# Roy-Shubhajit/FIT-GNN

Hardware: AMD Instinct MI355X
Metric: edges aggregated/sec (GCN fwd+bwd) on coarsened subgraphs (higher is better)
Workload: dtype f32

## Files before the change

fit-gnn_amd/csrc/gemm_f32.hip:

```cpp
#include <algorithm>
#include <cmath>

#include "common.h"
#include "fitgnn_hip.h"

namespace {

typedef float f32x16 __attribute__((ext_vector_type(16)));

constexpr int kBK = 32;
constexpr int kPitch = 36;

template <int WM, int WN, int MI, int NJ, bool AKM, bool BKM>
struct Geo {
    static constexpr int TI = 32 * MI * WM, TJ = 32 * NJ * WN, THREADS = 64 * WM * WN;
    static constexpr int A_DW = AKM ? kBK * TI : TI * kPitch;
    static constexpr int B_DW = BKM ? kBK * TJ : TJ * kPitch;
    static constexpr int STAGE_DW = A_DW + B_DW;
    static constexpr int LDS_BYTES = 2 * STAGE_DW * 4;
    static constexpr int NA = TI * 8 / THREADS, NB = TJ * 8 / THREADS;
    static_assert(LDS_BYTES <= 160 * 1024, "tile does not fit the CU's LDS");
    static_assert(TI * 8 % THREADS == 0 && TJ * 8 % THREADS == 0, "stage not divisible over the threads");
};

template <bool KM, int T, int NV, int THREADS>
__device__ __forceinline__ void load_slab(float4 (&r)[NV], const float *__restrict__ P, long ld, long t0, long lim, long k0, long klim) {
    const int tid = threadIdx.x;
#pragma unroll
    for (int p = 0; p < NV; ++p) {
        const int v = tid + p * THREADS;
        if (!KM) {
            const int row = v >> 3, k4 = v & 7;
            long i = t0 + row;
            i = i < lim ? i : lim - 1;
            const long k = k0 + 4 * k4;
            r[p] = k < klim ? *reinterpret_cast<const float4 *>(P + i * ld + k) : make_float4(0.f, 0.f, 0.f, 0.f);
        } else {
            constexpr int Q = T / 4;
            const int kr = v / Q, c4 = v % Q;
            long i = t0 + 4 * c4;
            i = i + 4 <= lim ? i : lim - 4;
            const long k = k0 + kr;
            r[p] = k < klim ? *reinterpret_cast<const float4 *>(P + k * ld + i) : make_float4(0.f, 0.f, 0.f, 0.f);
        }
    }
}

template <bool KM, int T, int NV, int THREADS>
__device__ __forceinline__ void store_slab(const float4 (&r)[NV], float *lds) {
    const int tid = threadIdx.x;
#pragma unroll
    for (int p = 0; p < NV; ++p) {
        const int v = tid + p * THREADS;
        if (!KM) {
            const int row = v >> 3, k4 = v & 7;
            *reinterpret_cast<float4 *>(lds + row * kPitch + 4 * k4) = r[p];
        } else {
            constexpr int Q = T / 4;
            const int kr = v / Q, c4 = v % Q;
            *reinterpret_cast<float4 *>(lds + kr * T + 4 * c4) = r[p];
        }
    }
}

template <bool KM, int T>
__device__ __forceinline__ void frag(float (&f)[4], const float *lds, int o, int kk, int lane) {
    if (!KM) {
        const float4 v = *reinterpret_cast<const float4 *>(lds + (o + (lane & 31)) * kPitch + 8 * kk + 4 * (lane >> 5));
        f[0] = v.x; f[1] = v.y; f[2] = v.z; f[3] = v.w;
    } else {
        const float *p = lds + (8 * kk + 4 * (lane >> 5)) * T + o + (lane & 31);
#pragma unroll
        for (int s = 0; s < 4; ++s) f[s] = p[s * T];
    }
}

struct StoreEpi {
    const int64_t *rows;
    const float *bias;
    const uint8_t *mask;
    uint64_t seed;
    long row0;
    uint32_t epi;
    float p_drop;
};

template <int WM, int WN, int MI, int NJ, bool AKM, bool BKM, bool EPI>
__global__ __launch_bounds__(64 * WM * WN) void gemm_f32_kernel(const float *__restrict__ A, long lda, const float *__restrict__ B, long ldb,
                                                                   long I, int J, long K, float *__restrict__ C, long ldc, int tiles_i,
                                                                   int tiles_j, int nchunks, long chunk_k, StoreEpi se) {
    using G = Geo<WM, WN, MI, NJ, AKM, BKM>;
    extern __shared__ __attribute__((aligned(16))) float lds_f[];
    const int lane = threadIdx.x & 63, wave = __builtin_amdgcn_readfirstlane(threadIdx.x >> 6);
    const int wm = wave / WN, wn = wave % WN;
    const int xcd = blockIdx.x & 7, slot = blockIdx.x >> 3;
    int ti, tj, chunk = 0;
    if (nchunks > 1) {
        const int ntile = tiles_i * tiles_j;
        const int tile = slot % ntile;
        chunk = xcd + 8 * (slot / ntile);
        ti = tile / tiles_j, tj = tile % tiles_j;
        if (chunk >= nchunks) return;
    } else {
        tj = slot % tiles_j;
        ti = xcd + 8 * (slot / tiles_j);
        if (ti >= tiles_i) return;
    }
    const long i0 = (long)ti * G::TI, j0 = (long)tj * G::TJ;
    const long k_begin = (long)chunk * chunk_k;
    const long k_end = nchunks > 1 ? (k_begin + chunk_k < K ? k_begin + chunk_k : K) : K;
    const int nstage = k_end > k_begin ? (int)((k_end - k_begin + kBK - 1) / kBK) : 0;

    f32x16 acc[MI][NJ];
#pragma unroll
    for (int i = 0; i < MI; ++i)
#pragma unroll
        for (int j = 0; j < NJ; ++j)
#pragma unroll
            for (int r = 0; r < 16; ++r) acc[i][j][r] = 0.f;

    float4 ra[G::NA], rb[G::NB];
    if (nstage > 0) {
        load_slab<AKM, G::TI, G::NA, G::THREADS>(ra, A, lda, i0, I, k_begin, k_end);
        load_slab<BKM, G::TJ, G::NB, G::THREADS>(rb, B, ldb, j0, (long)J, k_begin, k_end);
        store_slab<AKM, G::TI, G::NA, G::THREADS>(ra, lds_f);
        store_slab<BKM, G::TJ, G::NB, G::THREADS>(rb, lds_f + G::A_DW);
    }
    __syncthreads();
    auto read_frags = [&](float (&fa)[MI][4], float (&fb)[NJ][4], const float *sa, const float *sb, int kk) {
#pragma unroll
        for (int i = 0; i < MI; ++i) frag<AKM, G::TI>(fa[i], sa, wm * (32 * MI) + i * 32, kk, lane);
#pragma unroll
        for (int j = 0; j < NJ; ++j) frag<BKM, G::TJ>(fb[j], sb, wn * (32 * NJ) + j * 32, kk, lane);
    };
    auto multiply = [&](const float (&fa)[MI][4], const float (&fb)[NJ][4]) {
#pragma unroll
        for (int st = 0; st < 4; ++st)
#pragma unroll
            for (int i = 0; i < MI; ++i)
#pragma unroll
                for (int j = 0; j < NJ; ++j)
                    acc[i][j] = __builtin_amdgcn_mfma_f32_32x32x2f32(fa[i][st], fb[j][st], acc[i][j], 0, 0, 0);
    };
    constexpr int NKK = kBK / 8;
    auto products = [&](int s) {
        const float *sa = lds_f + (s & 1) * G::STAGE_DW;
        const float *sb = sa + G::A_DW;
#pragma unroll
        for (int kk = 0; kk < NKK; ++kk) {
            float fa[MI][4], fb[NJ][4];
            read_frags(fa, fb, sa, sb, kk);
            multiply(fa, fb);
        }
    };
    for (int s = 0; s < nstage; ++s) {
        const bool more = s + 1 < nstage;
        if (more) {
            const long k0 = k_begin + (long)(s + 1) * kBK;
            load_slab<AKM, G::TI, G::NA, G::THREADS>(ra, A, lda, i0, I, k0, k_end);
            load_slab<BKM, G::TJ, G::NB, G::THREADS>(rb, B, ldb, j0, (long)J, k0, k_end);
        }
        products(s);
        if (more) {
            float *na = lds_f + ((s + 1) & 1) * G::STAGE_DW;
            store_slab<AKM, G::TI, G::NA, G::THREADS>(ra, na);
            store_slab<BKM, G::TJ, G::NB, G::THREADS>(rb, na + G::A_DW);
        }
        __syncthreads();
    }

    float *out = nchunks > 1 ? C + (long)chunk * I * J : C;
    const long ldo = nchunks > 1 ? (long)J : ldc;
    if constexpr (EPI) {
        const uint64_t seed = fitgnn::resolve_seed(se.seed, se.epi);
        const float keep_scale = (se.epi & FITGNN_EPI_DROPOUT) ? 1.0f / (1.0f - se.p_drop) : 1.0f;
        const uint32_t thresh = fitgnn::dropout_threshold(se.p_drop);
#pragma unroll
        for (int i = 0; i < MI; ++i) {
            const long row0 = i0 + wm * (32 * MI) + i * 32 + 4 * (lane >> 5);
            long orow[16];
#pragma unroll
            for (int r = 0; r < 16; ++r) {
                const long row = row0 + (r & 3) + 8 * (r >> 2);
                orow[r] = row < I ? (se.rows ? (long)se.rows[row] : se.row0 + row) : 0;
            }
#pragma unroll
            for (int j = 0; j < NJ; ++j) {
                const long col = j0 + wn * (32 * NJ) + j * 32 + (lane & 31);
                const float bias = ((se.epi & FITGNN_EPI_BIAS) && col < J) ? se.bias[col] : 0.f;
#pragma unroll
                for (int r = 0; r < 16; ++r) {
                    const long row = row0 + (r & 3) + 8 * (r >> 2);
                    if (row < I && col < J)
                        out[row * ldo + col] = fitgnn::finish_elem(acc[i][j][r], bias, se.epi, keep_scale, thresh, seed, se.mask,
                                                                   (uint64_t)orow[r] * (uint64_t)J + (uint64_t)col);
                }
            }
        }
        return;
    }
#pragma unroll
    for (int i = 0; i < MI; ++i) {
#pragma unroll
        for (int j = 0; j < NJ; ++j) {
            const long col = j0 + wn * (32 * NJ) + j * 32 + (lane & 31);
            const long row0 = i0 + wm * (32 * MI) + i * 32 + 4 * (lane >> 5);
#pragma unroll
            for (int r = 0; r < 16; ++r) {
                const long row = row0 + (r & 3) + 8 * (r >> 2);
                if (row < I && col < J) out[row * ldo + col] = acc[i][j][r];
            }
        }
    }
}

template <bool EPI>
__global__ __launch_bounds__(256) void sum_chunks_kernel(const float *__restrict__ partial, int nchunks, long IJ, float *__restrict__ out, int J,
                                                         long ldc, StoreEpi se) {
    const long q = (long)blockIdx.x * blockDim.x + threadIdx.x;
    if (q >= IJ) return;
    float part[8];
#pragma unroll
    for (int u = 0; u < 8; ++u) part[u] = 0.f;
    int c = 0;
    for (; c + 8 <= nchunks; c += 8) {
#pragma unroll
        for (int u = 0; u < 8; ++u) part[u] += partial[(long)(c + u) * IJ + q];
    }
#pragma unroll
    for (int u = 0; u < 8; ++u)
        if (c + u < nchunks) part[u] += partial[(long)(c + u) * IJ + q];
    float acc = part[0];
#pragma unroll
    for (int u = 1; u < 8; ++u) acc += part[u];
    const long row = q / J, col = q % J;
    if constexpr (EPI) {
        const uint64_t seed = fitgnn::resolve_seed(se.seed, se.epi);
        const float keep_scale = (se.epi & FITGNN_EPI_DROPOUT) ? 1.0f / (1.0f - se.p_drop) : 1.0f;
        const long orow = se.rows ? (long)se.rows[row] : se.row0 + row;
        acc = fitgnn::finish_elem(acc, (se.epi & FITGNN_EPI_BIAS) ? se.bias[col] : 0.f, se.epi, keep_scale, fitgnn::dropout_threshold(se.p_drop),
                                  seed, se.mask, (uint64_t)orow * (uint64_t)J + (uint64_t)col);
    }
    out[row * ldc + col] = acc;
}

enum Shape { S256 = 0, S256x128, S64x512, S128, S64x128, S128x64, S64x64 };
struct ShapeDim { int ti, tj, per_cu; };
constexpr ShapeDim kShape[] = {{256, 256, 1}, {256, 128, 1}, {64, 512, 1}, {128, 128, 2}, {64, 128, 2}, {128, 64, 2}, {64, 64, 4}};

struct Plan {
    int shape;
    int tiles_i, tiles_j, nchunks;
    long chunk_k;
    long main_rows;
    int rem_tiles_i, rem_chunks;
    long rem_chunk_k;
};

Plan make_plan(long I, int J, long K, bool akm, bool bkm) {
    Plan p;
    const bool tn = akm && bkm;
    auto tiles_of = [&](int sh) { return ((I + kShape[sh].ti - 1) / kShape[sh].ti) * ((J + kShape[sh].tj - 1) / kShape[sh].tj); };
    if (tn) {
        if (I <= 64) p.shape = S64x512;
        else if (J <= 128 || K < 65536) p.shape = S128;
        else p.shape = S256;
    } else if (J <= 64) {
        p.shape = S128x64;
    } else {
        const int cand[4] = {J <= 128 ? S256x128 : S256, S128, S64x128, S64x64};
        const double eff[4] = {1.0, K <= 256 ? 1.0 : 0.85, 0.94, 0.85};
        double best_cost = 0;
        for (int q = 0; q < 4; ++q) {
            const int sh = cand[q];
            const long t = tiles_of(sh);
            double rounds = (double)((t + 255) / 256);
            if (q == 0 && !akm && t / 256 >= 1 && t % 256 > 0 && t % 256 <= 96 && K >= 8 * 2 * kBK) rounds = (double)(t / 256) + 0.15;
            const double cost = rounds * kShape[sh].ti * kShape[sh].tj / eff[q];
            if (q == 0 || cost < best_cost) { best_cost = cost; p.shape = sh; }
        }
        if (K >= 4096 && tiles_of(S256) <= 512 && J > 128) p.shape = S128;
    }
    const int TI = kShape[p.shape].ti, TJ = kShape[p.shape].tj;
    const double slots = 256.0 * kShape[p.shape].per_cu;
    p.tiles_i = (int)((I + TI - 1) / TI);
    p.tiles_j = (J + TJ - 1) / TJ;
    p.nchunks = 1;
    p.chunk_k = K;
    const double ntile = (double)p.tiles_i * p.tiles_j;
    const double t_tile = 2.0 * TI * TJ * (double)K / (0.45e12 / kShape[p.shape].per_cu);
    const long most = K / (4 * kBK);
    double best = ceil(ntile / slots) * t_tile;
    for (long c = 8; c <= most && c <= 256; c += 8) {
        const double t = ceil(ntile * (double)c / slots) * t_tile / (double)c + (double)(c + 1) * (double)I * (double)J * 4.0 / 3.0e12 + 4e-6;
        if (t < 0.92 * best) { best = t; p.nchunks = (int)c; }
    }
    if (p.nchunks > 1) {
        const long per = (K + p.nchunks - 1) / p.nchunks;
        p.chunk_k = (per + kBK - 1) / kBK * kBK;
    }
    p.main_rows = 0; p.rem_tiles_i = 0; p.rem_chunks = 1; p.rem_chunk_k = K;
    const long T = (long)p.tiles_i * p.tiles_j;
    const long full = T / 256, rem = T % 256;
    if (!akm && kShape[p.shape].per_cu == 1 && p.nchunks == 1 && full >= 1 && rem > 0 && rem <= 96 && K >= 8 * 2 * kBK) {
        const long main_tiles_i = full * 256 / p.tiles_j;
        if (main_tiles_i >= 1 && main_tiles_i < p.tiles_i) {
            p.main_rows = main_tiles_i * TI;
            p.rem_tiles_i = (int)(p.tiles_i - main_tiles_i);
            p.rem_chunks = 8;
            p.rem_chunk_k = ((K + 7) / 8 + kBK - 1) / kBK * kBK;
        }
    }
    return p;
}

template <int WM, int WN, int MI, int NJ, bool AKM, bool BKM, bool EPI>
int launch(const Plan &p, const float *a, long lda, const float *b, long ldb, long I, int J, long K, float *c, long ldc, hipStream_t s,
           const StoreEpi &se) {
    using G = Geo<WM, WN, MI, NJ, AKM, BKM>;
    static std::atomic<uint64_t> lds_done{0};
    if (const int rc = fitgnn_lds_limit_once((const void *)gemm_f32_kernel<WM, WN, MI, NJ, AKM, BKM, EPI>, G::LDS_BYTES, lds_done)) return rc;
    unsigned grid;
    if (p.nchunks > 1) grid = (unsigned)(p.tiles_i * p.tiles_j * ((p.nchunks + 7) / 8 * 8));
    else grid = (unsigned)((p.tiles_i + 7) / 8 * 8 * p.tiles_j);
    hipLaunchKernelGGL((gemm_f32_kernel<WM, WN, MI, NJ, AKM, BKM, EPI>), dim3(grid), dim3(G::THREADS), G::LDS_BYTES, s, a, lda, b, ldb, I, J,
                       K, c, ldc, p.tiles_i, p.tiles_j, p.nchunks, p.chunk_k, se);
    return (int)hipGetLastError();
}

template <bool AKM, bool BKM, bool EPI = false>
int launch_shape(const Plan &p, const float *a, long lda, const float *b, long ldb, long I, int J, long K, float *c, long ldc, hipStream_t s,
                 const StoreEpi &se = StoreEpi{}) {
    if constexpr (AKM && BKM) {
        if (p.shape == S64x512) return launch<1, 4, 2, 4, AKM, BKM, EPI>(p, a, lda, b, ldb, I, J, K, c, ldc, s, se);
    }
    switch (p.shape) {
        case S256x128: return launch<4, 1, 2, 4, AKM, BKM, EPI>(p, a, lda, b, ldb, I, J, K, c, ldc, s, se);
        case S128: return launch<2, 2, 2, 2, AKM, BKM, EPI>(p, a, lda, b, ldb, I, J, K, c, ldc, s, se);
        case S64x128: return launch<2, 2, 1, 2, AKM, BKM, EPI>(p, a, lda, b, ldb, I, J, K, c, ldc, s, se);
        case S128x64: return launch<4, 1, 1, 2, AKM, BKM, EPI>(p, a, lda, b, ldb, I, J, K, c, ldc, s, se);
        case S64x64: return launch<2, 2, 1, 1, AKM, BKM, EPI>(p, a, lda, b, ldb, I, J, K, c, ldc, s, se);
        default: return launch<4, 2, 2, 4, AKM, BKM, EPI>(p, a, lda, b, ldb, I, J, K, c, ldc, s, se);
    }
}

}

extern "C" size_t fitgnn_gemm_exact_workspace_bytes(int64_t I, int32_t J, int64_t K, int32_t a_kmajor, int32_t b_kmajor) {
    if (I <= 0 || J <= 0 || K <= 0) return 0;
    const Plan p = make_plan((long)I, J, (long)K, a_kmajor != 0, b_kmajor != 0);
    if (p.main_rows > 0) return (size_t)p.rem_chunks * (size_t)(I - p.main_rows) * (size_t)J * sizeof(float);
    return p.nchunks > 1 ? (size_t)p.nchunks * (size_t)I * (size_t)J * sizeof(float) : 0;
}

extern "C" int fitgnn_gemm_exact_plan(int64_t I, int32_t J, int64_t K, int32_t a_kmajor, int32_t b_kmajor, int32_t *shape, int32_t *nchunks,
                                      int64_t *main_rows) {
    if (I <= 0 || J <= 0 || K <= 0 || !shape || !nchunks || !main_rows) return FITGNN_E_BADARG;
    const Plan p = make_plan((long)I, J, (long)K, a_kmajor != 0, b_kmajor != 0);
    *shape = p.shape;
    *nchunks = p.nchunks;
    *main_rows = p.main_rows;
    return 0;
}

extern "C" int fitgnn_gemm_exact_f32(const float *a, int64_t lda, int32_t a_kmajor, const float *b, int64_t ldb, int32_t b_kmajor,
                                     int64_t I, int32_t J, int64_t K, float *c, int64_t ldc, void *workspace, void *stream) {
    if (I <= 0 || J <= 0 || K <= 0 || ldc < J) return FITGNN_E_BADARG;
    if (!a || !b || !c) return FITGNN_E_BADARG;
    const int64_t a_inner = a_kmajor ? I : K, b_inner = b_kmajor ? (int64_t)J : K;
    if (a_inner < 4 || b_inner < 4 || (a_inner % 4) != 0 || (b_inner % 4) != 0 || lda < a_inner || ldb < b_inner || (lda % 4) != 0 ||
        (ldb % 4) != 0)
        return FITGNN_E_BADARG;
    if ((((uintptr_t)a | (uintptr_t)b) % 16) != 0) return FITGNN_E_ALIGN;
    if (a_kmajor && !b_kmajor) return FITGNN_E_BADARG;
    const Plan p = make_plan((long)I, J, (long)K, a_kmajor != 0, b_kmajor != 0);
    hipStream_t s = (hipStream_t)stream;
    if (p.main_rows > 0) {
        if (!workspace || ((uintptr_t)workspace % 16) != 0) return FITGNN_E_BADARG;
        Plan pm = p, pr = p;
        pm.tiles_i = (int)(p.main_rows / kShape[p.shape].ti);
        pr.tiles_i = p.rem_tiles_i; pr.nchunks = p.rem_chunks; pr.chunk_k = p.rem_chunk_k;
        const long rem_rows = (long)I - p.main_rows;
        const float *a_rem = a + p.main_rows * (long)lda;
        int rc;
        if (b_kmajor) {
            rc = launch_shape<false, true>(pm, a, (long)lda, b, (long)ldb, p.main_rows, J, (long)K, c, (long)ldc, s);
            if (!rc) rc = launch_shape<false, true>(pr, a_rem, (long)lda, b, (long)ldb, rem_rows, J, (long)K, (float *)workspace, (long)J, s);
        } else {
            rc = launch_shape<false, false>(pm, a, (long)lda, b, (long)ldb, p.main_rows, J, (long)K, c, (long)ldc, s);
            if (!rc) rc = launch_shape<false, false>(pr, a_rem, (long)lda, b, (long)ldb, rem_rows, J, (long)K, (float *)workspace, (long)J, s);
        }
        if (rc) return rc;
        const long IJ = rem_rows * J;
        hipLaunchKernelGGL(sum_chunks_kernel<false>, dim3((unsigned)((IJ + 255) / 256)), dim3(256), 0, s, (const float *)workspace, pr.nchunks,
                           IJ, c + p.main_rows * (long)ldc, J, (long)ldc, StoreEpi{});
        return (int)hipGetLastError();
    }
    float *dst = c;
    long ldd = (long)ldc;
    if (p.nchunks > 1) {
        if (!workspace || ((uintptr_t)workspace % 16) != 0) return FITGNN_E_BADARG;
        dst = (float *)workspace;
    }
    int rc;
    if (a_kmajor) rc = launch_shape<true, true>(p, a, (long)lda, b, (long)ldb, (long)I, J, (long)K, dst, ldd, s);
    else if (b_kmajor) rc = launch_shape<false, true>(p, a, (long)lda, b, (long)ldb, (long)I, J, (long)K, dst, ldd, s);
    else rc = launch_shape<false, false>(p, a, (long)lda, b, (long)ldb, (long)I, J, (long)K, dst, ldd, s);
    if (rc) return rc;
    if (p.nchunks > 1) {
        const long IJ = (long)I * J;
        hipLaunchKernelGGL(sum_chunks_kernel<false>, dim3((unsigned)((IJ + 255) / 256)), dim3(256), 0, s, (const float *)workspace, p.nchunks, IJ, c,
                           J, (long)ldc, StoreEpi{});
        return (int)hipGetLastError();
    }
    return 0;
}

extern "C" int fitgnn_gemm_exact_epi_f32(const float *a, int64_t lda, const float *b, int64_t ldb, int64_t I, int32_t J, int64_t K, float *c,
                                         int64_t ldc, const int64_t *rows, const float *bias, uint32_t epilogue, float p_drop, uint64_t seed,
                                         const uint8_t *mask, void *workspace, void *stream) {
    if (I <= 0 || J <= 0 || K <= 0 || ldc < J) return FITGNN_E_BADARG;
    if (!a || !b || !c) return FITGNN_E_BADARG;
    if (K < 4 || (K % 4) != 0 || lda < K || ldb < K || (lda % 4) != 0 || (ldb % 4) != 0) return FITGNN_E_BADARG;
    if ((((uintptr_t)a | (uintptr_t)b) % 16) != 0) return FITGNN_E_ALIGN;
    if (epilogue & ~(FITGNN_EPI_BIAS | FITGNN_EPI_ELU | FITGNN_EPI_DROPOUT | FITGNN_EPI_SEED_DEVICE)) return FITGNN_E_BADARG;
    if ((epilogue & (FITGNN_EPI_ELU | FITGNN_EPI_DROPOUT)) && (J % 4) != 0) return FITGNN_E_BADARG;
    if ((epilogue & FITGNN_EPI_BIAS) && !bias) return FITGNN_E_BADARG;
    if ((epilogue & FITGNN_EPI_DROPOUT) && !(p_drop >= 0.f && p_drop < 1.f)) return FITGNN_E_BADARG;
    const Plan p = make_plan((long)I, J, (long)K, false, false);
    if (p.nchunks > 1) return FITGNN_E_BADARG;
    hipStream_t s = (hipStream_t)stream;
    StoreEpi se{rows, bias, mask, seed, 0, epilogue, p_drop};
    if (p.main_rows == 0) return launch_shape<false, false, true>(p, a, (long)lda, b, (long)ldb, (long)I, J, (long)K, c, (long)ldc, s, se);
    if (!workspace || ((uintptr_t)workspace % 16) != 0) return FITGNN_E_BADARG;
    Plan pm = p, pr = p;
    pm.tiles_i = (int)(p.main_rows / kShape[p.shape].ti);
    pr.tiles_i = p.rem_tiles_i; pr.nchunks = p.rem_chunks; pr.chunk_k = p.rem_chunk_k;
    const long rem_rows = (long)I - p.main_rows;
    int rc = launch_shape<false, false, true>(pm, a, (long)lda, b, (long)ldb, p.main_rows, J, (long)K, c, (long)ldc, s, se);
    if (!rc) rc = launch_shape<false, false>(pr, a + p.main_rows * (long)lda, (long)lda, b, (long)ldb, rem_rows, J, (long)K, (float *)workspace, (long)J, s);
    if (rc) return rc;
    if (rows) se.rows = rows + p.main_rows;
    se.row0 = p.main_rows;
    const long IJ = rem_rows * J;
    hipLaunchKernelGGL(sum_chunks_kernel<true>, dim3((unsigned)((IJ + 255) / 256)), dim3(256), 0, s, (const float *)workspace, pr.nchunks, IJ,
                       c + p.main_rows * (long)ldc, J, (long)ldc, se);
    return (int)hipGetLastError();
}
```

fit-gnn_amd/csrc/spmm.hip:

```cpp
#include <hip/hip_runtime.h>
#include <stdint.h>

#include <algorithm>

#include "common.h"
#include "fitgnn_hip.h"

namespace {

constexpr int kWaves = 4;
constexpr int kThreads = kWaves * 64;
constexpr int kDefaultWindowRows = 16;
constexpr int kMaxWindowRows = 96;
constexpr int kSmallWindowRows = 16;
constexpr int kLongRow = 16;

template <int VEC> struct Pack;
template <> struct Pack<4> {
    using T = float4;
    static __device__ __forceinline__ T zero() { return make_float4(0.f, 0.f, 0.f, 0.f); }
    static __device__ __forceinline__ void fma(T &a, float v, const T &x) {
        a.x = fmaf(v, x.x, a.x); a.y = fmaf(v, x.y, a.y); a.z = fmaf(v, x.z, a.z); a.w = fmaf(v, x.w, a.w);
    }
    static __device__ __forceinline__ float get(const T &a, int i) { return i == 0 ? a.x : i == 1 ? a.y : i == 2 ? a.z : a.w; }
// ... 164 lines not shown
                    mc[j] = 0; mv[j] = 0.f;
                    if (i < n_meta) { mc[j] = cidx[E0 + i]; mv[j] = val[E0 + i]; }
                }
            }
#pragma unroll
            for (int j = 0; j < B; ++j) {
                const int r = wave + (p0 + j) * kWaves;
                if (r < win_rows) lds[r * 64 + lane] = v[j];
            }
            if (p0 == 0) {
                if ((int)threadIdx.x <= rp_rows) s_rp[threadIdx.x] = rpv;
#pragma unroll
                for (int j = 0; j < MB; ++j) {
                    const int i = threadIdx.x + j * kThreads;
                    if (i < n_meta) { s_col[i] = mc[j]; s_val[i] = mv[j]; }
                }
            }
        }
        for (int i = threadIdx.x + kThreads; i <= rp_rows; i += kThreads) s_rp[i] = rowptr[tile.row_begin + i];
        for (int i = threadIdx.x + MB * kThreads; i < n_meta; i += kThreads) { s_col[i] = cidx[E0 + i]; s_val[i] = val[E0 + i]; }
    }
    __syncthreads();

    const float keep_scale = (epi & FITGNN_EPI_DROPOUT) ? 1.0f / (1.0f - p_drop) : 1.0f;
    const uint32_t thresh = fitgnn::dropout_threshold(p_drop);
    const RowEpilogue rowepi{epi, keep_scale, (epi & FITGNN_EPI_DROPOUT) ? 1.0f - p_drop : 1.0f, thresh, seed, mask, prev};
    float cs[VEC];
#pragma unroll
    for (int i = 0; i < VEC; ++i) cs[i] = 0.f;
    float bv[VEC];
#pragma unroll
    for (int i = 0; i < VEC; ++i) bv[i] = ((epi & FITGNN_EPI_BIAS) && live) ? bias[col0 + i] : 0.f;
    const int slot_off = planned ? 0 : win_begin;
    auto gcol = [&](int c) -> int {
        if (!planned) return c + slot_off;
        if (c < 0) return -(c + 1);
        return listed ? win_cols[win_begin + c] : win_begin + c;
    };
    auto xsrc = [&](int g) -> int64_t { return xrow ? xrow[g] : g; };
    auto gather = [&](int g) -> T {
        const int64_t sr = xsrc(g);
        if (zero_from >= 0 && xrow && sr >= zero_from) return P::zero();
        return *reinterpret_cast<const T *>(Xs + sr * ldx);
    };
    for (int row = tile.row_begin + wave; row < tile.row_end; row += kWaves) {
        const T o_prev = prev_row<VEC>(rowepi, row, col0, H, live);
        const int lr = row - tile.row_begin;
        int e0, e1;
        if (lr < rp_rows) { e0 = s_rp[lr]; e1 = s_rp[lr + 1]; } else { e0 = rowptr[row]; e1 = rowptr[row + 1]; }
        e0 = __builtin_amdgcn_readfirstlane(e0);
        e1 = __builtin_amdgcn_readfirstlane(e1);
        T acc = P::zero();
        for (int base = e0; base < e1; base += 64) {
            const int cnt = min(64, e1 - base);
            int my_c = 0;
            float my_v = 0.f;
            if (lane < cnt) {
                const int i = base + lane - E0;
                if (i < n_meta) { my_c = s_col[i]; my_v = s_val[i]; } else { my_c = cidx[base + lane]; my_v = val[base + lane]; }
            }
            int k = 0;
            if (cnt >= kLongRow) {
                for (; k + 8 <= cnt; k += 8) {
                    T x[8];
                    float w[8];
#pragma unroll
                    for (int u = 0; u < 8; ++u) {
                        const int c = __builtin_amdgcn_readlane(my_c, k + u) - slot_off;
                        w[u] = __int_as_float(__builtin_amdgcn_readlane(__float_as_int(my_v), k + u));
                        x[u] = gather(gcol(c));
                    }
#pragma unroll
                    for (int u = 0; u < 8; ++u) P::fma(acc, w[u], x[u]);
                }
            }
            for (; k < cnt; k += 4) {
                const int k1 = min(k + 1, cnt - 1), k2 = min(k + 2, cnt - 1), k3 = min(k + 3, cnt - 1);
                const int c0 = __builtin_amdgcn_readlane(my_c, k) - slot_off;
                const int c1 = __builtin_amdgcn_readlane(my_c, k1) - slot_off;
                const int c2 = __builtin_amdgcn_readlane(my_c, k2) - slot_off;
                const int c3 = __builtin_amdgcn_readlane(my_c, k3) - slot_off;
                const float w0 = __int_as_float(__builtin_amdgcn_readlane(__float_as_int(my_v), k));
                const float w1 = k + 1 < cnt ? __int_as_float(__builtin_amdgcn_readlane(__float_as_int(my_v), k1)) : 0.f;
                const float w2 = k + 2 < cnt ? __int_as_float(__builtin_amdgcn_readlane(__float_as_int(my_v), k2)) : 0.f;
                const float w3 = k + 3 < cnt ? __int_as_float(__builtin_amdgcn_readlane(__float_as_int(my_v), k3)) : 0.f;
                const bool in0 = (unsigned)c0 < (unsigned)win_rows, in1 = (unsigned)c1 < (unsigned)win_rows;
                const bool in2 = (unsigned)c2 < (unsigned)win_rows, in3 = (unsigned)c3 < (unsigned)win_rows;
                T x0, x1, x2, x3;
                if (in0 && in1 && in2 && in3) {
                    x0 = lds[c0 * 64 + lane]; x1 = lds[c1 * 64 + lane];
                    x2 = lds[c2 * 64 + lane]; x3 = lds[c3 * 64 + lane];
                } else {
                    const int g0 = gcol(c0), g1 = gcol(c1), g2 = gcol(c2), g3 = gcol(c3);
                    if (in0) x0 = lds[c0 * 64 + lane]; else x0 = gather(g0);
                    if (in1) x1 = lds[c1 * 64 + lane]; else x1 = gather(g1);
                    if (in2) x2 = lds[c2 * 64 + lane]; else x2 = gather(g2);
                    if (in3) x3 = lds[c3 * 64 + lane]; else x3 = gather(g3);
                }
                P::fma(acc, w0, x0); P::fma(acc, w1, x1); P::fma(acc, w2, x2); P::fma(acc, w3, x3);
            }
        }
        if (live) finish_row<VEC, true, NOEPI>(acc, row, col0, H, Y, ldy, bv, rowepi, cs, o_prev);
    }
    if (!NOEPI && (epi & FITGNN_EPI_BACKWARD) && col_part)
        write_col_part<VEC>(reinterpret_cast<float *>(lds_raw), cs, col_part, t, H, col0, live);
}


#ifdef FITGNN_SPMM_STAMPS
static __device__ unsigned long long *g_spmm_dbg;
#define SSTAMP(var) const unsigned long long var = __builtin_readcyclecounter()
#define SACC(i, a, b) sdbg[i] += (b) - (a)
#else
#define SSTAMP(var)
#define SACC(i, a, b)
#endif
constexpr int kBlkRows = 16;
constexpr int kBlkLW = 1;
constexpr int kBlkLong = 4 * kBlkLW;
constexpr int kBlkMeta = 128;

template <bool XROW, bool BWD, bool NOEPI = false, bool TWO = false>
__global__ __launch_bounds__(kThreads, BWD ? 4 : TWO ? 6 : XROW ? 7 : 7) void spmm_block_kernel(
    const int32_t *__restrict__ rowptr, const int32_t *__restrict__ col, const float *__restrict__ val,
    const float *__restrict__ X, int64_t ldx, float *__restrict__ Y, int64_t ldy, int32_t H,
    const fitgnn_block_t *__restrict__ blocks, int32_t n_blocks, const int32_t *__restrict__ long_rows, int32_t n_slabs,
    const float *__restrict__ bias, uint32_t epi, float p_drop, uint64_t seed_arg, const uint8_t *__restrict__ mask,
    const int32_t *__restrict__ xrow, const int32_t *__restrict__ xcol, const float *__restrict__ prev, float *__restrict__ col_part,
    int32_t zero_from, const float *__restrict__ Xc2 = nullptr, int64_t ldxc = 0, const int32_t *__restrict__ row_p = nullptr,
    const float *__restrict__ row_w = nullptr, int32_t xc_zero_from = 0) {
    static_assert(!TWO || (XROW && !BWD && NOEPI), "the two-hop form is a plain product over a table");
    constexpr uint32_t kNtOut = TWO ? fitgnn::kNtOutTwoHop : BWD ? 0u : XROW ? fitgnn::kNtOutTable : fitgnn::kNtOutPlain;
    constexpr uint32_t kNtWin = TWO ? fitgnn::kNtWinTwoHop : XROW ? fitgnn::kNtWinTable : fitgnn::kNtWinPlain;
    using P = Pack<4>;
    using T = float4;
    constexpr int kZeroSlot = kBlkRows + kBlkLong;
    const uint64_t seed = fitgnn::resolve_seed(seed_arg, epi);
    __shared__ T s_win[(kBlkRows + kBlkLong + 1) * 64];
    __shared__ int32_t s_rp[kBlkRows + 4];
    __shared__ int32_t s_col[kBlkMeta];
    __shared__ float s_val[kBlkMeta];
    __shared__ int32_t s_long[kBlkLong];
    __shared__ int32_t s_hub_pos;
    const int bid = blockIdx.x;
    const int seq = bid >> 3;
    const int slab = seq % n_slabs;
    const int b = (seq / n_slabs) * 8 + (bid & 7);
    if (b >= n_blocks) return;
#ifdef FITGNN_SPMM_STAMPS
    unsigned long long sdbg[8] = {0, 0, 0, 0, 0, 0, 0, 0};
#endif
    SSTAMP(s_begin);
    const fitgnn_block_t blk = blocks[b];
    if (blk.row_end <= blk.row_begin) return;
    const int lane = threadIdx.x & 63;
    const int wave = __builtin_amdgcn_readfirstlane(threadIdx.x >> 6);
    const int col0 = slab * 256 + lane * 4;
    const bool live = col0 + 4 <= H;
    const float *Xs = X + (live ? col0 : max(H - 4, 0));
    auto src = [&](int r) -> int64_t { return XROW ? (int64_t)xrow[r] : (int64_t)r; };
    auto ecol = [&](int e, int c) -> int { return (TWO || (XROW && xcol)) ? xcol[e] : (XROW ? xrow[c] : c); };
    const int n_long = min(blk.n_long, kBlkLong);
    const float keep_scale = (epi & FITGNN_EPI_DROPOUT) ? 1.0f / (1.0f - p_drop) : 1.0f;
    const uint32_t thresh = fitgnn::dropout_threshold(p_drop);
    const RowEpilogue rowepi{(BWD || TWO) ? (epi | FITGNN_EPI_BACKWARD) : (epi & ~FITGNN_EPI_BACKWARD), keep_scale,
                             (epi & FITGNN_EPI_DROPOUT) ? 1.0f - p_drop : 1.0f, thresh, seed, mask, (BWD || TWO) ? prev : nullptr};
    const int colc2 = live ? col0 : max(H - 4, 0);
    float cs[4];
#pragma unroll
    for (int i = 0; i < 4; ++i) cs[i] = 0.f;
    float bv[4];
#pragma unroll
    for (int i = 0; i < 4; ++i) bv[i] = ((epi & FITGNN_EPI_BIAS) && live) ? bias[col0 + i] : 0.f;

    const bool has_zero = XROW && !TWO && zero_from >= 0;
    auto is_zero_row = [&](int64_t opr) { return has_zero && opr >= (int64_t)zero_from; };
    T pv[4];
    T o_nx[kBlkRows / kWaves];
    int p_rp = 0, p_c = 0, p_cx = 0, p_E0 = 0;
    float p_v = 0.f;
    int xr_next = 0;
    int xp_next = 0, xw_next = 0;
    int sr_pub[4] = {0, 0, 0, 0}, pp_pub[4] = {0, 0, 0, 0};
    float w_pub[4] = {0.f, 0.f, 0.f, 0.f};
    int hub_pos = 0x7fffffff;
    auto fetch_indices = [&](int r0, int r1) {
        if (XROW) {
            const int r = r0 + wave + lane * kWaves;
            xr_next = (lane < 4 && r < r1) ? xrow[r] : 0;
            if (TWO) {
                xp_next = (lane < 4 && r < r1) ? row_p[r] : 0x7fffffff;
                xw_next = (lane < 4 && r < r1) ? __float_as_int(row_w[r]) : 0;
            }
        }
    };
    auto prefetch = [&](int r0, int r1, int E0) {
        const int xr = xr_next;

#pragma unroll
        for (int j = 0; j < 4; ++j) {
            const int r = r0 + wave + j * kWaves;
            pv[j] = P::zero();
            const int64_t sr = XROW ? (int64_t)__builtin_amdgcn_readlane(xr, j) : (int64_t)r;
            if (TWO) {
                const int rr = min(r, r1 - 1);
                const float *rowp = sr >= 0 ? Xs + sr * ldx : prev + (uint64_t)rr * (uint64_t)H + (uint64_t)colc2;
                const int pp = __builtin_amdgcn_readlane(xp_next, j);
                const T a = fitgnn::load4<kNtWin>(rowp);
                pv[j] = r < r1 ? a : P::zero();
                sr_pub[j] = (int)sr;
                pp_pub[j] = pp;
                w_pub[j] = __int_as_float(__builtin_amdgcn_readlane(xw_next, j));
            } else if (r < r1 && !is_zero_row(sr)) {
                pv[j] = fitgnn::load4<kNtWin>(Xs + sr * ldx);
            }
        }
        if (XROW) fetch_indices(r1, min(r1 + kBlkRows, blk.row_end));
        if (BWD) {
#pragma unroll
            for (int j = 0; j < kBlkRows / kWaves; ++j) o_nx[j] = prev_row<4, BWD>(rowepi, min(r0 + wave + j * kWaves, r1 - 1), col0, H, live);
        }
        p_rp = 0;
        if ((int)threadIdx.x <= r1 - r0) p_rp = rowptr[r0 + threadIdx.x];
        p_c = 0; p_cx = 0; p_v = 0.f;
        if ((int)threadIdx.x < kBlkMeta && blk.nnz_end > blk.nnz_begin) {
            const int e = min(E0 + (int)threadIdx.x, blk.nnz_end - 1);
            p_c = col[e];
            p_cx = (TWO || (XROW && xcol)) ? xcol[e] : p_c;
            p_v = val[e];
        }
        p_E0 = E0;
    };
    fetch_indices(blk.row_begin, min(blk.row_begin + kBlkRows, blk.row_end));
    if ((int)threadIdx.x < kBlkLong) s_long[threadIdx.x] = (int)threadIdx.x < n_long ? long_rows[blk.long_off + threadIdx.x] : -1;
    if (XROW && !TWO && (int)threadIdx.x < 64) s_win[kZeroSlot * 64 + threadIdx.x] = P::zero();
    if (TWO && threadIdx.x == 0) s_hub_pos = 0x7fffffff;
    int my_long[kBlkLW], cur[kBlkLW], end[kBlkLW], pos[kBlkLW], lc[kBlkLW], lcx[kBlkLW];
    float lv[kBlkLW];
    T acc_long[kBlkLW];
#pragma unroll
    for (int q = 0; q < kBlkLW; ++q) {
        const int slot = wave + q * kWaves;
        my_long[q] = slot < n_long ? long_rows[blk.long_off + slot] : -1;
        my_long[q] = __builtin_amdgcn_readfirstlane(my_long[q]);
        acc_long[q] = P::zero();
        cur[q] = end[q] = 0;
        pos[q] = 64;
        lc[q] = 0x7fffffff;
        lcx[q] = 0;
        lv[q] = 0.f;
    }
    prefetch(blk.row_begin, min(blk.row_begin + kBlkRows, blk.row_end), blk.nnz_begin);
#pragma unroll
    for (int q = 0; q < kBlkLW; ++q) {
        const int slot = wave + q * kWaves;
        if (my_long[q] >= 0) {
            cur[q] = __builtin_amdgcn_readfirstlane(rowptr[my_long[q]]);
            end[q] = __builtin_amdgcn_readfirstlane(rowptr[my_long[q] + 1]);
            const int64_t lr_src = src(my_long[q]);
            s_win[(kBlkRows + slot) * 64 + lane] = is_zero_row(lr_src) ? P::zero() : *reinterpret_cast<const T *>(Xs + lr_src * ldx);
            if (TWO && slot == 0 && lr_src < (int64_t)xc_zero_from) {
                s_win[kZeroSlot * 64 + lane] = *reinterpret_cast<const T *>(Xc2 + lr_src * ldxc + colc2);
                if (lane == 0) s_hub_pos = (int)lr_src;
            }
        }
    }
    __syncthreads();
    if (TWO) hub_pos = __builtin_amdgcn_readfirstlane(s_hub_pos);
    int lid[kBlkLong];
#pragma unroll
    for (int i = 0; i < kBlkLong; ++i) lid[i] = __builtin_amdgcn_readfirstlane(s_long[i]);

    const int n_pieces = (blk.row_end - blk.row_begin + kBlkRows - 1) / kBlkRows;

    auto gather_long = [&](int q, int bound) {
        while (cur[q] < end[q]) {
            if (pos[q] == 64) {
                const int e = cur[q] + lane;
                lc[q] = e < end[q] ? col[e] : 0x7fffffff;
                lcx[q] = (XROW && xcol && e < end[q]) ? xcol[e] : 0;
                lv[q] = e < end[q] ? val[e] : 0.f;
                pos[q] = 0;
            }
            const unsigned long long in = __ballot(lc[q] < bound) >> pos[q];
            const int n_in = in == 0 ? 0 : (int)__builtin_popcountll(in);
            constexpr int kLongBatch = (TWO || (XROW && !BWD)) ? 4 : 8;
            for (int k = pos[q]; k < pos[q] + n_in; k += kLongBatch) {
                const int last = pos[q] + n_in - 1;
                T x[kLongBatch];
                float w[kLongBatch];
#pragma unroll
                for (int u = 0; u < kLongBatch; ++u) {
                    const int kk = min(k + u, last);
                    const int64_t c = (XROW && xcol) ? (int64_t)__builtin_amdgcn_readlane(lcx[q], kk) : src(__builtin_amdgcn_readlane(lc[q], kk));
                    w[u] = k + u <= last ? __int_as_float(__builtin_amdgcn_readlane(__float_as_int(lv[q]), kk)) : 0.f;
                    x[u] = is_zero_row(c) ? P::zero() : *reinterpret_cast<const T *>(Xs + c * ldx);
                }
#pragma unroll
                for (int u = 0; u < kLongBatch; ++u) P::fma(acc_long[q], w[u], x[u]);
            }
            pos[q] += n_in;
            cur[q] += n_in;
            if (pos[q] < 64) break;
        }
    };
#pragma unroll
    for (int q = 0; q < kBlkLW; ++q)
// ... 962 lines not shown
```

fit-gnn_amd/fitgnn_amd/_lib.py:

```python
import ctypes
import os

_HERE = os.path.dirname(os.path.abspath(__file__))
LIB_PATH = os.path.join(os.path.dirname(_HERE), "lib", "libfitgnn_hip.so")

c_i32, c_i64, c_u32, c_u64, c_f32, c_size = (ctypes.c_int32, ctypes.c_int64, ctypes.c_uint32, ctypes.c_uint64,
                                              ctypes.c_float, ctypes.c_size_t)
ptr = ctypes.c_void_p

EPI_BIAS, EPI_ELU, EPI_DROPOUT, EPI_SEED_DEVICE = 1, 2, 4, 8
SPMM_GATHER = 0x100
MAX_K = 16
MATCH_HEAVY_EDGE, MATCH_ALGEBRAIC_JC = 0, 1
MATCH_SMALL_MAX_NODES, MATCH_SMALL_MAX_NNZ, MATCH_SMALL_MAX_K, MATCH_SMALL_LDS_BUDGET = 128, 1024, 12, 65536
MATCH_DONE, MATCH_TOO_BIG, MATCH_BAD_INPUT = 1, 2, 3
QUALITY_MAX_K = 64

SIGNATURES = {
    "fitgnn_abi_version": (ctypes.c_int, []),
    "fitgnn_error_string": (ctypes.c_char_p, [ctypes.c_int]),
    "fitgnn_stream_copy_f32": (ctypes.c_int, [ptr, ptr, c_i64, ptr]),
    "fitgnn_spmm_default_window_rows": (ctypes.c_int, []),
    "fitgnn_spmm_max_window_rows": (ctypes.c_int, [c_i32]),
    "fitgnn_gcn_norm_csr_f32": (ctypes.c_int, [ptr, ptr, ptr, ptr, ptr, c_i32, ptr]),
    "fitgnn_spmm_csr_f32": (ctypes.c_int, [ptr, ptr, ptr, ptr, c_i64, ptr, c_i64, c_i32, c_i32, ptr, c_i32, ptr, ptr,
                                           ptr, c_i32, c_i32, ptr, c_u32, c_f32, c_u64, ptr, ptr]),
    "fitgnn_spmm_csr_blocks_f32": (ctypes.c_int, [ptr, ptr, ptr, ptr, c_i64, ptr, c_i64, c_i32, c_i32, ptr, c_i32, ptr,
                                                  ptr, ptr, c_i32, ptr, c_u32, c_f32, c_u64, ptr, ptr]),
    "fitgnn_spmm_csr_dz_f32": (ctypes.c_int, [ptr, ptr, ptr, ptr, c_i64, ptr, c_i64, c_i32, c_i32, ptr, c_i32, ptr, ptr,
                                              ptr, c_i32, c_i32, ptr, c_u32, c_f32, c_u64, ptr, ptr, ptr]),
    "fitgnn_spmm_csr_blocks_dz_f32": (ctypes.c_int, [ptr, ptr, ptr, ptr, c_i64, ptr, c_i64, c_i32, c_i32, ptr, c_i32, ptr,
                                                     ptr, ptr, c_i32, ptr, c_u32, c_f32, c_u64, ptr, ptr, ptr]),
    "fitgnn_lanczos_parts": (c_i32, [c_i32]),
    "fitgnn_lanczos_spmv_f64": (ctypes.c_int, [ptr, ptr, ptr, ptr, ptr, c_i32, ctypes.c_double, ctypes.c_double, ptr]),
    "fitgnn_lanczos_project_f64": (ctypes.c_int, [ptr, c_i64, c_i32, ptr, c_i32, ptr, ptr, ptr]),
    "fitgnn_lanczos_reduce_f64": (ctypes.c_int, [ptr, c_i32, c_i32, ptr, ptr]),
    "fitgnn_lanczos_finish_f64": (ctypes.c_int, [ptr, c_i64, c_i32, ptr, c_i32, ptr, ptr, ptr, ptr, c_i32, ptr]),
    "fitgnn_lanczos_rotate_f64": (ctypes.c_int, [ptr, c_i64, c_i32, ptr, c_i32, ptr, c_i64, c_i32, ptr]),
    "fitgnn_spmm_csr_stream_f32": (ctypes.c_int, [ptr, ptr, ptr, c_i64, ptr, c_i64, ptr, c_i64, c_i32, c_i32, ptr, c_i32, ptr, c_i32, ptr, ptr,
                                                  ptr, c_u32, c_f32, c_u64, ptr, ptr]),
    "fitgnn_spmm_csr_stream_dz_f32": (ctypes.c_int, [ptr, ptr, ptr, c_i64, ptr, c_i64, ptr, c_i64, c_i32, c_i32, ptr, c_i32, ptr, c_i32, ptr, ptr,
                                                     ptr, c_u32, c_f32, c_u64, ptr, ptr, ptr]),
    "fitgnn_spmm_rows_compact_parts": (c_i32, [c_i32]),
    "fitgnn_spmm_rows_compact_f32": (ctypes.c_int, [ptr, ptr, ptr, c_i64, ptr, c_i64, c_i32, ptr, c_i64, c_i32, c_i32, ptr]),
    "fitgnn_spmm_rows_compact_dz_f32": (ctypes.c_int, [ptr, ptr, ptr, c_i64, ptr, c_i64, c_i32, ptr, c_i64, c_i32, c_i32, ptr, c_u32, c_f32,
                                                       c_u64, ptr, ptr, ptr]),
    "fitgnn_two_hop_rows_f32": (ctypes.c_int, [ptr, ptr, ptr, ptr, c_i64, c_i32, ptr, c_i32, ptr, c_i32, c_u32, c_f32, c_u64, ptr, ptr, c_i64, ptr]),
    "fitgnn_spmm_two_hop_blocks_f32": (ctypes.c_int, [ptr, ptr, ptr, ptr, c_i64, ptr, c_i64, c_i32, c_i32, ptr, c_i32, ptr, ptr, ptr, ptr, ptr, c_i64,
                                                      c_i32, ptr, ptr, c_u32, c_f32, c_u64, ptr, ptr, ptr]),
    "fitgnn_segment_sum_f32": (ctypes.c_int, [ptr, ptr, c_i32, ptr, c_i64, c_i32, ptr, c_i64, ptr]),
    "fitgnn_segment_max_f32": (ctypes.c_int, [ptr, ptr, c_i32, ptr, c_i64, c_i32, ptr, ptr, ptr]),
    "fitgnn_segment_max_bwd_f32": (ctypes.c_int, [ptr, ptr, c_i32, c_i32, ptr, c_i64, ptr]),
    "fitgnn_segment_expand_f32": (ctypes.c_int, [ptr, ptr, ptr, c_i64, c_i32, ptr, ptr]),
    "fitgnn_make_tiles_host": (ctypes.c_int, [ptr, c_i64, c_i32, ptr, c_i64, ptr]),
    "fitgnn_split_blocks_host": (ctypes.c_int, [ptr, c_i64, ptr, c_i32, c_i64, c_i32, ptr, c_i64, ptr, ptr, ptr, ptr, c_i64, ptr]),
    "fitgnn_plan_tiles_host": (ctypes.c_int, [ptr, ptr, c_i32, c_i32, ptr, c_i32, c_i32, c_i32, ptr, ptr, ptr, ptr, ptr]),
    "fitgnn_epilogue_bwd_workspace_bytes": (c_size, [c_i32, c_i32]),
    "fitgnn_epilogue_bwd_f32": (ctypes.c_int, [ptr, ptr, ptr, c_i32, c_i32, c_u32, c_f32, c_u64, ptr, ptr, ptr, c_size, ptr]),
    "fitgnn_head_max_classes": (ctypes.c_int, []),
    "fitgnn_head_max_classes_wide": (ctypes.c_int, []),
    "fitgnn_epilogue_bwd_head_supported": (ctypes.c_int, [c_i32, c_i32, c_i32]),
    "fitgnn_epilogue_bwd_head_workspace_bytes": (c_size, [c_i32, c_i32, c_i32]),
    "fitgnn_epilogue_bwd_head_f32": (ctypes.c_int, [ptr, ptr, c_i32, ptr, ptr, c_i32, c_i32, c_u32, c_f32, c_u64, ptr, ptr, ptr,
                                                   ptr, c_size, ptr]),
    "fitgnn_epilogue_bwd_head_rows_f32": (ctypes.c_int, [ptr, ptr, c_i32, ptr, ptr, c_i32, c_i32, ptr, c_i32, c_u32, c_f32, c_u64, ptr,
                                                        ptr, ptr, ptr, c_size, ptr]),
    "fitgnn_epilogue_bwd_rows_f32": (ctypes.c_int, [ptr, ptr, ptr, c_i32, c_i32, ptr, c_i32, c_u32, c_f32, c_u64, ptr, ptr, ptr, c_size, ptr]),
    "fitgnn_spmm_epilogue_bwd_supported": (ctypes.c_int, [c_i32, c_i32, c_i32]),
    "fitgnn_spmm_epilogue_bwd_workspace_bytes": (c_size, [c_i32, c_i32, c_i32]),
    "fitgnn_spmm_epilogue_bwd_f32": (ctypes.c_int, [ptr, ptr, ptr, ptr, c_i32, c_i32, ptr, ptr, ptr, c_i32, ptr, ptr, c_i32, c_i32,
                                                   c_u32, c_f32, c_u64, ptr, ptr, ptr, ptr, c_size, ptr]),
    "fitgnn_gat_scores_f32": (ctypes.c_int, [ptr, c_i64, c_i32, c_i32, ptr, ptr, ptr, ptr, ptr]),
    "fitgnn_gat_edge_softmax_f32": (ctypes.c_int, [ptr, ptr, ptr, ptr, c_f32, c_i32, ptr, ptr]),
    "fitgnn_sddmm_csr_f32": (ctypes.c_int, [ptr, ptr, ptr, c_i64, ptr, c_i64, c_i32, c_i32, ptr, ptr]),
    "fitgnn_sddmm_csr_rows_f32": (ctypes.c_int, [ptr, ptr, ptr, c_i64, ptr, c_i64, ptr, c_i32, c_i32, ptr, ptr]),
    "fitgnn_gat_softmax_bwd_rows_f32": (ctypes.c_int, [ptr, ptr, ptr, ptr, ptr, ptr, c_f32, ptr, c_i32, ptr, ptr, ptr]),
    "fitgnn_gat_softmax_bwd_f32": (ctypes.c_int, [ptr, ptr, ptr, ptr, ptr, ptr, c_f32, c_i32, ptr, ptr, ptr]),
    "fitgnn_l1_loss_f32": (ctypes.c_int, [ptr, ptr, c_i32, c_f32, ptr, ptr, ptr]),
    "fitgnn_softmax_nll_workspace_bytes": (c_size, [c_i32]),
    "fitgnn_softmax_nll_f32": (ctypes.c_int, [ptr, c_i64, c_i32, c_i32, ptr, ptr, c_i32, c_f32, ptr, ptr, ptr, c_size, ptr]),
    "fitgnn_adam_step_f32": (ctypes.c_int, [ptr, ptr, ptr, ptr, c_i64, c_f32, c_f32, c_f32, c_f32, c_f32, ptr, ptr]),
    "fitgnn_sum_leading_f32": (ctypes.c_int, [ptr, c_i32, c_i64, ptr, ptr]),
    "fitgnn_gemm_atb_workspace_bytes": (c_size, [c_i64, c_i32, c_i32]),
    "fitgnn_gemm_atb_f32": (ctypes.c_int, [ptr, c_i64, ptr, c_i64, c_i64, c_i32, c_i32, ptr, ptr, ptr]),
    "fitgnn_gemm_nt_f32": (ctypes.c_int, [ptr, c_i64, ptr, c_i64, c_i64, c_i32, c_i32, ptr, c_i64, ptr]),
    "fitgnn_gemm_exact_workspace_bytes": (c_size, [c_i64, c_i32, c_i64, c_i32, c_i32]),
    "fitgnn_gemm_exact_f32": (ctypes.c_int, [ptr, c_i64, c_i32, ptr, c_i64, c_i32, c_i64, c_i32, c_i64, ptr, c_i64, ptr, ptr]),
    "fitgnn_gemm_exact_plan": (ctypes.c_int, [c_i64, c_i32, c_i64, c_i32, c_i32, ptr, ptr, ptr]),
    "fitgnn_gemm_exact_epi_f32": (ctypes.c_int, [ptr, c_i64, ptr, c_i64, c_i64, c_i32, c_i64, ptr, c_i64, ptr, ptr, c_u32, c_f32, c_u64, ptr, ptr,
                                                 ptr]),
    "fitgnn_gemm_nt_presplit_bytes": (c_size, [c_i32, c_i32]),
    "fitgnn_gemm_nt_presplit_f32": (ctypes.c_int, [ptr, c_i64, c_i64, c_i32, c_i32, c_i32, ptr, ptr]),
    "fitgnn_gemm_nt_pre_f32": (ctypes.c_int, [ptr, c_i64, ptr, c_i64, c_i32, c_i32, ptr, c_i64, ptr]),
    "fitgnn_gemm_nt_epilogue_bwd_workspace_bytes": (c_size, [c_i64, c_i32]),
    "fitgnn_gemm_nt_epilogue_bwd_f32": (ctypes.c_int, [ptr, c_i64, ptr, c_i64, c_i64, c_i32, c_i32, ptr, ptr, ctypes.c_uint32, c_f32,
                                                       ctypes.c_uint64, ptr, ptr, ptr, c_size, ptr]),
    "fitgnn_colsum_partials_f32": (ctypes.c_int, [ptr, c_i32, c_i32, ptr, ptr]),
    "fitgnn_head_rows_lds_bytes": (c_size, [c_i32, c_i32]),
    "fitgnn_head_rows_f32": (ctypes.c_int, [ptr, c_i64, ptr, c_i32, ptr, ptr, c_i32, c_i32, ptr, c_i64, c_i32, ptr]),
    "fitgnn_epilogue_fwd_rows_f32": (ctypes.c_int, [ptr, c_i64, ptr, c_i32, c_i32, ptr, c_u32, c_f32, c_u64, ptr, ptr]),
    "fitgnn_dense_narrow_k_lds_bytes": (c_size, [c_i32, c_i32]),
    "fitgnn_dense_narrow_k_f32": (ctypes.c_int, [ptr, c_i64, ptr, c_i64, c_i32, c_i32, c_i32, ptr, c_u32, c_f32, c_u64, ptr, ptr, c_i64, ptr]),
    "fitgnn_narrow_atb_workspace_bytes": (c_size, [c_i32, c_i32, c_i32]),
    "fitgnn_narrow_atb_f32": (ctypes.c_int, [ptr, c_i64, ptr, c_u32, c_f32, c_u64, ptr, ptr, c_i64, c_i32, c_i32, c_i32, ptr, ptr, ptr, c_size,
                                             ptr]),
    "fitgnn_adam_step_acc_f32": (ctypes.c_int, [ptr, ptr, ptr, ptr, ptr, c_i64, c_f32, c_f32, c_f32, c_f32, c_f32, ptr, ptr, c_i32, c_u64, ptr]),
    "fitgnn_pool_head_supported": (ctypes.c_int, [c_i32, c_i32]),
    "fitgnn_pool_head_f32": (ctypes.c_int, [ptr, ptr, c_i32, ptr, c_i64, c_i32, ptr, ptr, ptr, c_i32, ptr, ptr, ptr]),
    "fitgnn_pool_head_bwd_f32": (ctypes.c_int, [ptr, ptr, c_i32, ptr, ptr, ptr, c_i64, c_i32, c_i32, ptr, ptr, ptr, ptr]),
    "fitgnn_colsum_narrow_workspace_bytes": (c_size, [c_i32, c_i32]),
    "fitgnn_colsum_narrow_f32": (ctypes.c_int, [ptr, c_i64, c_i32, c_i32, ptr, ptr, c_size, ptr]),
    "fitgnn_spmm_narrow_f32": (ctypes.c_int, [ptr, ptr, ptr, ptr, ptr, c_i32, c_i32, c_f32, ptr, c_f32, ptr, c_f32, ptr]),
    "fitgnn_spmm_narrow_padded_f32": (ctypes.c_int, [ptr, ptr, ptr, ptr, ptr, c_i32, c_i32, c_f32, ptr, c_f32, ptr, c_f32, ptr]),
    "fitgnn_appnp_unit_rows": (ctypes.c_int, [c_i32]),
    "fitgnn_appnp_unit_entries": (ctypes.c_int, []),
    "fitgnn_appnp_block_rows": (ctypes.c_int, []),
    "fitgnn_appnp_block_entries": (ctypes.c_int, []),
    "fitgnn_appnp_blocks_f32": (ctypes.c_int, [ptr, ptr, ptr, ptr, c_i32, c_i32, c_i32, ptr, ptr, ptr, ptr, c_i32, c_i32, c_f32, c_i32, ptr]),
    "fitgnn_appnp_lds_bytes": (ctypes.c_int64, [c_i32, c_i32, c_i32]),
    "fitgnn_appnp_lds_max_bytes": (ctypes.c_int, []),
    "fitgnn_appnp_lds_items_per_thread": (ctypes.c_int, []),
    "fitgnn_appnp_lds_f32": (ctypes.c_int, [ptr, ptr, ptr, ptr, c_i32, c_i32, c_i32, ptr, ptr, c_i32, c_i32, c_f32, c_i32, c_i32, c_i32, ptr]),
    "fitgnn_gather_rows_padded_f32": (ctypes.c_int, [ptr, c_i64, c_i32, ptr, c_i64, ptr, c_i32, ptr]),
    "fitgnn_appnp_units_f32": (ctypes.c_int, [ptr, ptr, ptr, ptr, c_i32, c_i32, c_i32, ptr, ptr, c_i32, c_i32, c_f32, c_i32, ptr]),
    "fitgnn_gcn_query_gather_f32": (ctypes.c_int, [ptr, ptr, ptr, ptr, c_i64, ptr, ptr, ptr, c_i32, c_i32, ptr, c_i64, ptr]),
    "fitgnn_sage_query_gather_f32": (ctypes.c_int, [ptr, ptr, ptr, ptr, c_i64, ptr, ptr, ptr, c_i32, c_i32, ptr, c_i64, ptr]),
    "fitgnn_gat_query_gather_f32": (ctypes.c_int, [ptr, ptr, ptr, c_i64, ptr, ptr, ptr, ptr, c_f32, ptr, ptr, c_f32, ptr, c_i32, c_i32, ptr,
                                                   c_i64, ptr]),
    "fitgnn_gcn_query_tail_lds_bytes": (c_size, [c_i32, c_i32]),
    "fitgnn_gcn_query_tail_f32": (ctypes.c_int, [ptr, c_i64, c_i32, ptr, ptr, ptr, ptr, c_i32, c_i32, c_i32, ptr, c_i64, c_i32, ptr]),
    "fitgnn_gcn_graph_query_hops_lds_bytes": (c_size, [c_i32, c_i32]),
    "fitgnn_gcn_graph_query_hops_f32": (ctypes.c_int, [ptr, ptr, ptr, ptr, c_i64, ptr, ptr, ptr, ptr, ptr, c_i32, c_i32, c_i32, ptr, c_i64, ptr]),
    "fitgnn_gcn_graph_query_tail_lds_bytes": (c_size, [c_i32, c_i32]),
    "fitgnn_gcn_graph_query_tail_f32": (ctypes.c_int, [ptr, c_i64, ptr, c_i32, ptr, ptr, ptr, ptr, c_i32, c_i32, c_i32, c_i32, c_i32, ptr, c_i64,
                                                       ptr]),
    "fitgnn_gin_query_hops_f32": (ctypes.c_int, [ptr, ptr, ptr, ptr, c_i64, ptr, ptr, ptr, ptr, ptr, ptr, ptr, c_i32, c_i32, c_i32, ptr, c_i64,
                                                 ptr]),
    "fitgnn_gin_query_tail_lds_bytes": (c_size, [c_i32, c_i32, c_i32]),
    "fitgnn_gin_query_tail_f32": (ctypes.c_int, [ptr, c_i64, c_i32, ptr, ptr, ptr, ptr, ptr, ptr, c_i32, c_i32, c_i32, c_i32, ptr, c_i64, c_i32,
                                                 ptr]),
    "fitgnn_gin_graph_query_hops_lds_bytes": (c_size, [c_i32, c_i32, c_i32]),
    "fitgnn_gin_graph_query_hops_f32": (ctypes.c_int, [ptr, ptr, ptr, ptr, c_i64, ptr, ptr, ptr, ptr, ptr, ptr, ptr, ptr, ptr, c_i32, c_i32, c_i32,
                                                       c_i32, ptr, c_i64, ptr]),
    "fitgnn_gin_graph_query_tail_lds_bytes": (c_size, [c_i32, c_i32, c_i32]),
    "fitgnn_gin_graph_query_tail_f32": (ctypes.c_int, [ptr, c_i64, ptr, c_i32, ptr, ptr, ptr, ptr, ptr, ptr, c_i32, c_i32, c_i32, c_i32, c_i32,
                                                       c_i32, ptr, c_i64, ptr]),
    "fitgnn_gat_graph_query_hops_lds_bytes": (c_size, [c_i32, c_i32]),
    "fitgnn_gat_graph_query_hops_f32": (ctypes.c_int, [ptr, ptr, ptr, c_i64, ptr, ptr, ptr, ptr, c_f32, ptr, ptr, c_f32, ptr, ptr, ptr, c_i32,
                                                       c_i32, c_i32, ptr, c_i64, ptr]),
    "fitgnn_sage_graph_query_hops_lds_bytes": (c_size, [c_i32, c_i32]),
    "fitgnn_sage_graph_query_hops_f32": (ctypes.c_int, [ptr, ptr, ptr, ptr, c_i64, ptr, ptr, ptr, ptr, ptr, c_i32, c_i32, c_i32, ptr, c_i64, ptr]),
    "fitgnn_csr_row_sum_f32": (ctypes.c_int, [ptr, ptr, c_i32, ptr, ptr]),
    "fitgnn_induced_edges_count": (ctypes.c_int, [ptr, ptr, ptr, ptr, ptr, ptr, c_i64, ptr, ptr]),
    "fitgnn_induced_edges_fill": (ctypes.c_int, [ptr, ptr, ptr, ptr, ptr, ptr, ptr, c_i64, ptr, ptr, ptr, ptr]),
    "fitgnn_batch_offsets": (ctypes.c_int, [ptr, ptr, c_i32, ptr, ptr, ptr, ptr, ptr, ptr, ptr, ptr, ptr]),
    "fitgnn_batch_gather": (ctypes.c_int, [c_i32, ptr, ptr, ptr, ptr, ptr, ptr, ptr, ptr, ptr, ptr, ptr, ptr, ptr, c_i32, ptr, c_i32, c_i32,
                                           c_i32, c_i32, c_i32, c_i32, ptr, ptr, ptr, ptr, ptr, ptr, ptr, ptr, ptr, c_i32, ptr, ptr, ptr, ptr, ptr,
                                           c_i32, ptr]),
    "fitgnn_closed_neighbourhoods": (ctypes.c_int, [ptr, ptr, c_i32, ptr, ptr, ptr]),
    "fitgnn_variation_costs_f64": (ctypes.c_int, [ptr, ptr, ptr, ptr, ptr, c_i32, c_i64, ptr, ptr, ptr, c_i32, ptr, ptr]),
    "fitgnn_variation_costs_batch_f64": (ctypes.c_int, [ptr, ptr, ptr, ptr, ptr, c_i32, c_i64, ptr, ptr, ptr, ptr, c_i32, ptr, ptr]),
    "fitgnn_greedy_select_workspace_bytes": (c_size, [c_i32, c_i64]),
    "fitgnn_greedy_select": (ctypes.c_int, [ptr, ptr, ptr, ptr, ptr, c_i32, c_i64, c_i32, ptr, ptr, ptr, c_i64, ptr, ptr,
                                            ptr, ptr, c_size, ptr]),
    "fitgnn_greedy_select_batch_workspace_bytes": (c_size, [c_i32, c_i64, c_i32]),
    "fitgnn_greedy_select_batch": (ctypes.c_int, [ptr, ptr, ptr, ptr, ptr, c_i32, c_i64, c_i32, ptr, ptr, ptr, c_i32, ptr, ptr,
                                                  c_i64, ptr, ptr, ptr, ptr, ptr, ptr, c_size, ptr]),
    "fitgnn_build_assignment_workspace_bytes": (c_size, [c_i32]),
    "fitgnn_build_assignment": (ctypes.c_int, [c_i32, ptr, ptr, ptr, ptr, ptr, ptr, ptr, c_size, ptr]),
    "fitgnn_compose_levels": (ctypes.c_int, [c_i32, ptr, ptr, ptr, ptr, ptr]),
    "fitgnn_lift_adjacency_workspace_bytes": (c_size, [c_i32, c_i64, c_i32]),
    "fitgnn_lift_adjacency": (ctypes.c_int, [c_i32, ptr, ptr, ptr, ptr, ptr, c_i32, ptr, ptr, ptr, ptr, ptr, c_size, ptr]),
    "fitgnn_edge_list": (ctypes.c_int, [ptr, ptr, ptr, c_i32, ptr, ptr, ptr, ptr, c_i64, ptr, ptr]),
    "fitgnn_heavy_edge_proximity_workspace_bytes": (c_size, [c_i32]),
    "fitgnn_heavy_edge_proximity": (ctypes.c_int, [ptr, ptr, ptr, c_i32, ptr, ptr, ptr, c_i64, ptr, ptr, c_size, ptr]),
    "fitgnn_jc_proximity": (ctypes.c_int, [ptr, ptr, c_i64, ptr, c_i32, c_i64, ptr, ptr]),
    "fitgnn_affinity_proximity_workspace_bytes": (c_size, [c_i32, c_i64]),
    "fitgnn_affinity_proximity": (ctypes.c_int, [c_i32, ptr, ptr, c_i64, ptr, c_i32, c_i64, ptr, ptr, c_size, ptr]),
    "fitgnn_edge_variation_costs_f64": (ctypes.c_int, [ptr, ptr, c_i64, ptr, ptr, c_i32, c_i64, ptr, ptr]),
    "fitgnn_jacobi_vectors_workspace_bytes": (c_size, [c_i32, c_i32]),
    "fitgnn_jacobi_vectors_f64": (ctypes.c_int, [ptr, ptr, ptr, ptr, c_i32, ptr, c_i32, c_i32, ptr, ptr, c_size, ptr]),
    "fitgnn_gauss_seidel_vectors_f64": (ctypes.c_int, [ptr, ptr, ptr, ptr, c_i32, c_i32, ptr, ptr, c_i32, ptr, ptr]),
    "fitgnn_greedy_matching_workspace_bytes": (c_size, [c_i32, c_i64, c_i32]),
    "fitgnn_greedy_matching": (ctypes.c_int, [ptr, ptr, ptr, c_i32, ptr, ptr, ptr, c_i64, ptr, c_i32, ptr, ptr, c_i64, ptr, ptr, ptr,
                                              ptr, ptr, ptr, c_size, ptr]),
    "fitgnn_match_small_lds_bytes": (c_size, [c_i32, c_i32, c_i32, c_i32]),
    "fitgnn_match_small": (ctypes.c_int, [c_i32, ptr, ptr, ptr, ptr, c_i32, c_i32, ctypes.c_double, c_i32, c_i32, ctypes.c_double, ptr,
                                          c_i64, ptr, c_i32, c_i32, ptr, ptr, ptr, ptr, ptr, ptr, ptr, ptr, ptr, ptr]),
    "fitgnn_pool_rows_workspace_bytes": (c_size, [c_i32, c_i32]),
    "fitgnn_pool_rows_f32": (ctypes.c_int, [ptr, ptr, c_i32, c_i32, ptr, c_i64, c_i32, ptr, c_i64, ptr, ptr, c_size, ptr]),
    "fitgnn_coarse_laplacian_workspace_bytes": (c_size, [c_i32, c_i64, c_i32]),
    "fitgnn_coarse_laplacian": (ctypes.c_int, [c_i32, ptr, ptr, ptr, c_i64, ptr, ptr, ptr, c_i32, ptr, ptr, ptr, ptr, ptr, c_size, ptr]),
    "fitgnn_project_lift_workspace_bytes": (c_size, [c_i32, c_i32]),
    "fitgnn_project_lift_f64": (ctypes.c_int, [ptr, ptr, c_i32, c_i32, ptr, c_i64, c_i32, ptr, c_i64, ptr, c_i64, ptr, c_size, ptr]),
    "fitgnn_laplacian_gram_workspace_bytes": (c_size, [c_i32, c_i32, c_i32]),
    "fitgnn_laplacian_gram_f64": (ctypes.c_int, [ptr, ptr, ptr, ptr, c_i32, ptr, c_i64, c_i32, ptr, c_i64, c_i32, ptr, c_i64, ptr, c_size,
                                                 ptr]),
    "fitgnn_cross_atb_workspace_bytes": (c_size, [c_i32, c_i32, c_i32]),
    "fitgnn_cross_atb_f64": (ctypes.c_int, [ptr, c_i64, c_i32, ptr, c_i64, c_i32, c_i32, ptr, c_i64, ptr, c_size, ptr]),
}

_lib = None


class FitgnnError(RuntimeError):
    pass


def lib():
    global _lib
    if _lib is None:
        if not os.path.exists(LIB_PATH):
            raise FitgnnError(f"{LIB_PATH} not found: build the HIP extension first "
                              "(python -c 'import __graft_entry__ as g; g.build()'); there is no CPU fallback")
        import torch

        L = ctypes.CDLL(LIB_PATH)
        for name, (res, args) in SIGNATURES.items():
            fn = getattr(L, name)
            fn.restype = res
            fn.argtypes = args
        if L.fitgnn_abi_version() != 1:
            raise FitgnnError("libfitgnn_hip.so ABI version mismatch")
        _lib = L
    return _lib


def check(rc, what=""):
    if rc != 0:
        msg = lib().fitgnn_error_string(int(rc)).decode()
        raise FitgnnError(f"{what}: {msg} (code {rc})")


def dptr(t):
    return None if t is None else ctypes.c_void_p(t.data_ptr())


def stream_ptr(device=None):
    import torch

    return ctypes.c_void_p(torch.cuda.current_stream(device).cuda_stream)


# ... 5 lines not shown
```

fit-gnn_amd/fitgnn_amd/ops.py:

```python
import ctypes

import os

import torch

from . import _lib
from ._lib import EPI_BIAS, EPI_DROPOUT, EPI_ELU


class OpConfig:
    __slots__ = ("gemm_precision", "atb_kernel", "nt_kernel", "nt_presplit", "fuse_dx_epilogue", "fold_backward",
                 "dedup_gather", "pad_table_min_k", "split_large_blocks", "compact_head_backward", "last_layer_on_loss_rows",
                 "compact_rows_kernel", "stream_kernel", "two_hop_backward", "narrow_input_first", "fused_pool_head", "fused_gemm_epilogue", "pooled_rows_last_layer", "rows_kernel_min_rows", "appnp_in_lds", "appnp_blocks", "appnp_sliced", "grad_sink", "profile", "profile_gemm",
                 "profile_fused", "seed_bank")

    def __init__(self, gemm_precision="exact", atb_kernel=True, nt_kernel=True, nt_presplit=True, fuse_dx_epilogue=True,
                 fold_backward=False, dedup_gather=True, pad_table_min_k=0, split_large_blocks=True, compact_head_backward=True,
                 last_layer_on_loss_rows=True, compact_rows_kernel=True, stream_kernel=False, two_hop_backward=True, narrow_input_first=True, fused_pool_head=True, fused_gemm_epilogue=True, pooled_rows_last_layer=True, rows_kernel_min_rows=32768, appnp_in_lds=True, appnp_blocks=True, appnp_sliced=True, grad_sink=None,
                 profile=None, profile_gemm=None, profile_fused=None, seed_bank=None):
        if gemm_precision not in ("exact", "high", "highest"):
            raise ValueError(f"gemm_precision {gemm_precision!r}: 'exact', 'high' or 'highest'")
        self.gemm_precision, self.atb_kernel, self.nt_kernel, self.nt_presplit = gemm_precision, atb_kernel, nt_kernel, nt_presplit
        self.fuse_dx_epilogue, self.fold_backward, self.dedup_gather = fuse_dx_epilogue, fold_backward, dedup_gather
        self.pad_table_min_k, self.split_large_blocks = pad_table_min_k, split_large_blocks
        self.compact_head_backward, self.last_layer_on_loss_rows = compact_head_backward, last_layer_on_loss_rows
        self.compact_rows_kernel, self.stream_kernel, self.two_hop_backward = compact_rows_kernel, stream_kernel, two_hop_backward
        self.narrow_input_first, self.fused_pool_head, self.grad_sink = narrow_input_first, fused_pool_head, grad_sink
        self.fused_gemm_epilogue = fused_gemm_epilogue
        self.pooled_rows_last_layer, self.rows_kernel_min_rows = pooled_rows_last_layer, int(rows_kernel_min_rows)
        self.appnp_in_lds, self.appnp_blocks, self.appnp_sliced = appnp_in_lds, appnp_blocks, appnp_sliced
        self.profile, self.profile_gemm, self.profile_fused, self.seed_bank = profile, profile_gemm, profile_fused, seed_bank

    def replace(self, **kw):
        cur = {k: getattr(self, k) for k in self.__slots__}
        cur.update(kw)
        return OpConfig(**cur)


DEFAULT = OpConfig()


def _addresses(*params):
    return tuple(None if t is None else t.data_ptr() for t in params)


class _GradSink:
    __slots__ = ("_sink", "_slices")

    def __init__(self, grad_sink):
        self._sink, self._slices = grad_sink, []

    def slice(self, ptr):
        if self._sink is None or ptr is None:
            return None
        s = self._sink.view(ptr)
        if s is not None:
            self._slices.append(s)
        return s

    def buffer(self, ptr, shape, device):
        s = self.slice(ptr)
        return s if s is not None else torch.empty(shape, dtype=torch.float32, device=device)

    def result(self, grad):
        return None if any(grad is s for s in self._slices) else grad


def mm(a, b):
    return torch.mm(a, b)


def _rows_16b(t):
    return (t.is_cuda and t.dtype == torch.float32 and t.dim() == 2 and t.shape[0] >= 1 and t.shape[1] >= 4 and t.shape[1] % 4 == 0
            and t.stride(1) == 1 and t.stride(0) % 4 == 0 and t.stride(0) >= t.shape[1] and t.data_ptr() % 16 == 0)


def _exact(cfg, a, b):
    return cfg.gemm_precision == "exact" and _rows_16b(a) and _rows_16b(b)


def gemm_exact(a, b, form, cfg=DEFAULT, out=None):
    L = _lib.lib()
    if form == "nt":
        (I, K), J, akm, bkm = a.shape, b.shape[0], 0, 0
        assert b.shape[1] == K
    elif form == "nn":
        (I, K), J, akm, bkm = a.shape, b.shape[1], 0, 1
        assert b.shape[0] == K
    elif form == "tn":
        (K, I), J, akm, bkm = a.shape, b.shape[1], 1, 1
        assert b.shape[0] == K
    else:
        raise ValueError(form)
    if out is None:
        out = torch.empty((I, J), dtype=torch.float32, device=a.device)
    else:
        assert out.shape == (I, J) and out.dtype == torch.float32 and out.stride(1) == 1 and out.is_cuda
    wb = int(L.fitgnn_gemm_exact_workspace_bytes(I, J, K, akm, bkm))
    ws = torch.empty(wb // 4, dtype=torch.float32, device=a.device) if wb else None
    ev = _gemm_events(cfg, "gemm_f32_kernel[%s]" % form, 2.0 * I * J * K)
    rc = L.fitgnn_gemm_exact_f32(_lib.dptr(a), a.stride(0), akm, _lib.dptr(b), b.stride(0), bkm, I, J, K, _lib.dptr(out), out.stride(0),
                                 _lib.dptr(ws), _lib.stream_ptr(a.device))
    _gemm_done(cfg, ev)
    _lib.check(rc, "fitgnn_gemm_exact_f32")
    return out


def gemm_exact_epi(a, b, rows, bias, epilogue, p=0.0, seed=0, mask=None, cfg=DEFAULT):
    L = _lib.lib()
    (I, K), J = a.shape, b.shape[0]
    assert b.shape[1] == K
    shape, nchunks, main_rows = ctypes.c_int32(), ctypes.c_int32(), ctypes.c_int64()
    _lib.check(L.fitgnn_gemm_exact_plan(I, J, K, 0, 0, ctypes.byref(shape), ctypes.byref(nchunks), ctypes.byref(main_rows)),
               "fitgnn_gemm_exact_plan")
    if nchunks.value > 1:
        return None
    _lib.require_cuda(a, b, rows, bias, mask)
    seed, epilogue = _seed_arg(seed, epilogue)
    if rows is not None:
        rows = (rows if rows.dtype == torch.int64 else rows.long()).contiguous()
    out = torch.empty((I, J), dtype=torch.float32, device=a.device)
    wb = int(L.fitgnn_gemm_exact_workspace_bytes(I, J, K, 0, 0))
    ws = torch.empty(wb // 4, dtype=torch.float32, device=a.device) if wb else None
    ev = _gemm_events(cfg, "gemm_f32_kernel[nt+epi]", 2.0 * I * J * K)
    rc = L.fitgnn_gemm_exact_epi_f32(_lib.dptr(a), a.stride(0), _lib.dptr(b), b.stride(0), I, J, K, _lib.dptr(out), out.stride(0),
                                     _lib.dptr(rows), _lib.dptr(None if bias is None else _f32c(bias)), epilogue, float(p), seed,
                                     _lib.dptr(mask), _lib.dptr(ws), _lib.stream_ptr(a.device))
    _gemm_done(cfg, ev)
    _lib.check(rc, "fitgnn_gemm_exact_epi_f32")
    return out


def padded_weight(W, Kp):
    Wp = torch.zeros((W.shape[0], Kp), dtype=torch.float32, device=W.device)
    Wp[:, : W.shape[1]] = W
    return Wp


def _full_grid(R, N):
    return ((R + 255) // 256) * ((N + 255) // 256) >= 128


def _nt_ok(a, b, cfg):
    if not (cfg.nt_kernel and cfg.gemm_precision == "high" and a.is_cuda and a.dtype == torch.float32 and b.dtype == torch.float32
            and a.dim() == 2 and b.dim() == 2 and a.stride(1) == 1 and a.shape[1] % 32 == 0 and a.shape[0] >= 1024
            and b.shape[0] >= 64 and a.stride(0) % 4 == 0 and a.data_ptr() % 16 == 0):
        return False
    if cfg.nt_presplit and _full_grid(a.shape[0], b.shape[0]):
        return True
    return b.stride(1) == 1 and b.stride(0) % 4 == 0 and b.data_ptr() % 16 == 0


def mm_xwt(x, W, cfg=DEFAULT):
    if _exact(cfg, x, W):
        return gemm_exact(x, W, "nt", cfg)
    if _nt_ok(x, W, cfg):
        return gemm_nt(x, W, cfg)
    return mm(x, W.t())


def _wt_operand(a, W, cfg):
    if cfg.nt_presplit and cfg.nt_kernel and _full_grid(a.shape[0], W.shape[1]):
        return W.t()
    return W.t().contiguous()


def mm_by_transposed(a, W, cfg=DEFAULT, out=None):
    if _exact(cfg, a, W):
        return gemm_exact(a, W, "nn", cfg, out=out)
    if out is not None:
        out.copy_(mm_by_transposed(a, W, cfg))
        return out
    if a.is_cuda and W.dim() == 2 and W.shape[0] >= 64 and W.shape[1] >= 64:
        Wt = _wt_operand(a, W, cfg)
        if _nt_ok(a, Wt, cfg):
            return gemm_nt(a, Wt, cfg)
        return mm(a, W.t().contiguous().t())
    return mm(a, W)


def _atb_ok(t):
    return (t.is_cuda and t.dtype == torch.float32 and t.dim() == 2 and t.stride(1) == 1 and t.stride(0) % 4 == 0
            and t.shape[1] % 4 == 0 and t.shape[1] >= 4 and t.data_ptr() % 16 == 0)


class _timed:
    __slots__ = ("cfg", "kind", "ev")

    def __init__(self, cfg, kind):
        self.cfg, self.kind, self.ev = cfg, kind, None

    def __enter__(self):
        if self.cfg is not None and self.cfg.profile is not None:
            self.ev = (torch.cuda.Event(enable_timing=True), torch.cuda.Event(enable_timing=True))
            self.ev[0].record()
        return self

    def __exit__(self, *exc):
        if self.ev is not None:
            self.ev[1].record()
            self.cfg.profile.append((self.ev[0], self.ev[1], self.kind))
        return False


def _gemm_events(cfg, name, flops):
    if cfg.profile_gemm is None:
        return None
    ev = (torch.cuda.Event(enable_timing=True), torch.cuda.Event(enable_timing=True), name, flops)
    ev[0].record()
    return ev


def _gemm_done(cfg, ev):
    if ev is not None:
        ev[1].record()
        cfg.profile_gemm.append(ev)


def gemm_atb(a, b, cfg=DEFAULT):
    L = _lib.lib()
    R, M, N = a.shape[0], a.shape[1], b.shape[1]
    ws = torch.empty(int(L.fitgnn_gemm_atb_workspace_bytes(R, M, N)) // 4, dtype=torch.float32, device=a.device)
    out = torch.empty((M, N), dtype=torch.float32, device=a.device)
    ev = _gemm_events(cfg, "gemm_atb_kernel+atb_reduce_kernel", 6.0 * R * M * N)
    rc = L.fitgnn_gemm_atb_f32(_lib.dptr(a), a.stride(0), _lib.dptr(b), b.stride(0), R, M, N, _lib.dptr(out), _lib.dptr(ws),
                               _lib.stream_ptr(a.device))
    _gemm_done(cfg, ev)
    _lib.check(rc, "fitgnn_gemm_atb_f32")
    return out


def _presplit(b, K_pad=None):
    L = _lib.lib()
    N, K = b.shape
    Kp = K if K_pad is None else int(K_pad)
    img = torch.empty(int(L.fitgnn_gemm_nt_presplit_bytes(N, Kp)), dtype=torch.uint8, device=b.device)
    _lib.check(L.fitgnn_gemm_nt_presplit_f32(_lib.dptr(b), b.stride(0), b.stride(1), N, Kp, K, _lib.dptr(img),
                                             _lib.stream_ptr(b.device)), "fitgnn_gemm_nt_presplit_f32")
    return img


def padded_table(x):
    pad = getattr(x, "_fitgnn_pad", None)
    if pad is None or pad[0] != x._version:
        Kp = (x.shape[1] + 31) // 32 * 32
        xp = torch.zeros((x.shape[0], Kp), dtype=torch.float32, device=x.device)
        xp[:, : x.shape[1]] = x
        x._fitgnn_pad = pad = (x._version, xp)
    return pad[1]


def gemm_nt_padded_k(a_pad, b, cfg=DEFAULT):
    L = _lib.lib()
    R, Kp, N = a_pad.shape[0], a_pad.shape[1], b.shape[0]
    out = torch.empty((R, N), dtype=torch.float32, device=a_pad.device)
    img = _presplit(b, K_pad=Kp)
    ev = _gemm_events(cfg, "gemm_nt_kernel<4,false,true>", 6.0 * R * N * Kp)
    rc = L.fitgnn_gemm_nt_pre_f32(_lib.dptr(a_pad), a_pad.stride(0), _lib.dptr(img), R, N, Kp, _lib.dptr(out), N,
                                  _lib.stream_ptr(a_pad.device))
    _gemm_done(cfg, ev)
    _lib.check(rc, "fitgnn_gemm_nt_pre_f32")
    return out


def _padded_table_path(Xt, W, cfg):
    return (cfg.nt_kernel and cfg.atb_kernel and cfg.nt_presplit and cfg.gemm_precision == "high" and Xt.is_cuda
            and Xt.dtype == torch.float32 and Xt.shape[1] % 32 != 0 and Xt.shape[1] >= cfg.pad_table_min_k and not Xt.requires_grad
            and W.shape[0] % 4 == 0 and W.shape[0] >= 64 and Xt.shape[0] >= 1024)


def gemm_nt(a, b, cfg=DEFAULT):
    L = _lib.lib()
    R, K, N = a.shape[0], a.shape[1], b.shape[0]
    out = torch.empty((R, N), dtype=torch.float32, device=a.device)
    if cfg.nt_presplit and _full_grid(R, N):
        img = _presplit(b)
        ev = _gemm_events(cfg, "gemm_nt_kernel<4,false,true>", 6.0 * R * N * K)
        rc = L.fitgnn_gemm_nt_pre_f32(_lib.dptr(a), a.stride(0), _lib.dptr(img), R, N, K, _lib.dptr(out), N, _lib.stream_ptr(a.device))
        _gemm_done(cfg, ev)
        _lib.check(rc, "fitgnn_gemm_nt_pre_f32")
        return out
    b = b.contiguous()
    _lib.check(L.fitgnn_gemm_nt_f32(_lib.dptr(a), a.stride(0), _lib.dptr(b), b.stride(0), R, N, K, _lib.dptr(out), N,
                                    _lib.stream_ptr(a.device)), "fitgnn_gemm_nt_f32")
    return out


def gemm_nt_epilogue_bwd(a, b, out, epilogue, p=0.0, seed=0, mask=None, want_db=True, cfg=DEFAULT):
    _lib.require_cuda(a, b, out, mask)
    L = _lib.lib()
    R, K, N = a.shape[0], a.shape[1], b.shape[0]
    seed, epilogue = _seed_arg(seed, epilogue)
    dZ = torch.empty((R, N), dtype=torch.float32, device=a.device)
    db = torch.empty(N, dtype=torch.float32, device=a.device) if want_db else None
    wb = int(L.fitgnn_gemm_nt_epilogue_bwd_workspace_bytes(R, N))
    work = torch.empty(max(wb, 4), dtype=torch.uint8, device=a.device)
    if cfg.nt_presplit and _full_grid(R, N):
        b_arg, ldb = _presplit(b), 0
    else:
        b_arg = b.contiguous()
        ldb = b_arg.stride(0)
    ev = _gemm_events(cfg, "gemm_nt_kernel<4,true,%s>" % ("true" if ldb == 0 else "false"), 6.0 * R * N * K)
    rc = L.fitgnn_gemm_nt_epilogue_bwd_f32(_lib.dptr(a), a.stride(0), _lib.dptr(b_arg), ldb, R, N, K, _lib.dptr(out),
                                           _lib.dptr(dZ), epilogue, float(p), seed, _lib.dptr(mask), _lib.dptr(db),
                                           _lib.dptr(work), wb, _lib.stream_ptr(a.device))
    _gemm_done(cfg, ev)
    _lib.check(rc, "fitgnn_gemm_nt_epilogue_bwd_f32")
    return dZ, db


def head_weight_grad_rows(dy_c, out_c, cfg=DEFAULT):
    C = dy_c.shape[1]
    if cfg.gemm_precision == "exact" and dy_c.is_cuda and _rows_16b(out_c):
        Cp = (C + 3) // 4 * 4
        if Cp != C or not _rows_16b(dy_c):
            pad = torch.zeros((dy_c.shape[0], Cp), dtype=torch.float32, device=dy_c.device)
            pad[:, :C] = dy_c
            dy_c = pad
        return gemm_exact(dy_c, out_c, "tn", cfg)[:C].contiguous()
    if dy_c.is_cuda and C < 64 and cfg.atb_kernel and cfg.gemm_precision == "high" and dy_c.shape[0] >= 256 and _atb_ok(out_c):
        pad = torch.zeros((dy_c.shape[0], 64), dtype=torch.float32, device=dy_c.device)
        pad[:, :C] = dy_c
        return gemm_atb(pad, out_c, cfg)[:C].contiguous()
    return mm_at_b(dy_c, out_c, cfg)


def mm_at_b(a, b, cfg=DEFAULT, out=None):
    R = a.shape[0]
    if out is not None:
        if _exact(cfg, a, b):
            return gemm_exact(a, b, "tn", cfg, out=out)
        out.copy_(mm_at_b(a, b, cfg))
        return out
    if _exact(cfg, a, b):
        return gemm_exact(a, b, "tn", cfg)
    if (cfg.gemm_precision == "high" and cfg.atb_kernel and R >= 256 and min(a.shape[1], b.shape[1]) >= 64 and _atb_ok(a)
            and _atb_ok(b)):
        return gemm_atb(a, b, cfg)
    B = R // 1408
    if B < 4:
        return mm(a.t(), b)
    Kc = R // B
    main = B * Kc
    part = torch.bmm(a[:main].view(B, Kc, a.shape[1]).transpose(1, 2), b[:main].view(B, Kc, b.shape[1]))
    W = part.shape[1] * part.shape[2]
    if part.is_cuda and W % 4 == 0:
        L = _lib.lib()
        st = _lib.stream_ptr(part.device)
        G = 64
        if B >= 8 * G and W <= 16384:
            Bg = B // G
            flat = part.view(B, W)
            stage = torch.empty((G + B - Bg * G, W), dtype=torch.float32, device=part.device)
            _lib.check(L.fitgnn_sum_leading_f32(_lib.dptr(flat), Bg, G * W, _lib.dptr(stage), st), "fitgnn_sum_leading_f32")
            if B > Bg * G:
                stage[G:].copy_(flat[Bg * G:])
            part, B = stage, int(stage.shape[0])
            out = torch.empty((a.shape[1], b.shape[1]), dtype=torch.float32, device=part.device)
        else:
            out = torch.empty(part.shape[1:], dtype=torch.float32, device=part.device)
        _lib.check(L.fitgnn_sum_leading_f32(_lib.dptr(part), B, W, _lib.dptr(out), st), "fitgnn_sum_leading_f32")
    else:
        out = part.sum(0)
    if main < R:
        out = out + torch.mm(a[main:].t(), b[main:])
    return out


class Linear(torch.autograd.Function):

    @staticmethod
    def forward(ctx, x, W, cfg):
        ctx.save_for_backward(x, W)
        ctx.cfg = cfg
        return mm_xwt(x, W, cfg)

    @staticmethod
    def backward(ctx, dh):
        x, W = ctx.saved_tensors
        dx = mm_by_transposed(dh, W, ctx.cfg) if ctx.needs_input_grad[0] else None
        dW = mm_at_b(dh, x, ctx.cfg) if ctx.needs_input_grad[1] else None
        return dx, dW, None


def colsum_narrow(x, out=None):
    if not (x.is_cuda and x.dim() == 2 and x.shape[1] <= 64 and x.dtype == torch.float32 and x.stride(1) == 1):
        return x.t().contiguous().sum(1) if (x.dim() == 2 and x.shape[0] > 4 * x.shape[1]) else x.sum(0)
    L = _lib.lib()
    n, C = x.shape
    if out is None:
        out = torch.empty(C, dtype=torch.float32, device=x.device)
    wb = int(L.fitgnn_colsum_narrow_workspace_bytes(n, C))
    work = torch.empty(max(wb, 4), dtype=torch.uint8, device=x.device)
    _lib.check(L.fitgnn_colsum_narrow_f32(_lib.dptr(x), x.stride(0), n, C, _lib.dptr(out), _lib.dptr(work), wb,
                                          _lib.stream_ptr(x.device)), "fitgnn_colsum_narrow_f32")
    return out


class BiasAdd(torch.autograd.Function):

    @staticmethod
    def forward(ctx, y, b):
        return y + b

    @staticmethod
    def backward(ctx, g):
        return g, (colsum_narrow(g if g.stride(1) == 1 else g.contiguous()) if ctx.needs_input_grad[1] else None)


class SmallLinear(torch.autograd.Function):

    @staticmethod
    def forward(ctx, x, W, b, cfg):
        ctx.save_for_backward(x, W)
        ctx.cfg = cfg
        y = torch.mm(x, W.t())
        return y if b is None else y + b

    @staticmethod
    def backward(ctx, dy):
        x, W = ctx.saved_tensors
        dx = torch.mm(dy, W) if ctx.needs_input_grad[0] else None
        dW = mm_at_b(_f32c(dy), _f32c(x), ctx.cfg) if ctx.needs_input_grad[1] else None
        db = colsum_narrow(dy) if ctx.needs_input_grad[2] else None
        return dx, dW, db, None


def softmax_nll_raw(z, idx, labels, scale):
    _lib.require_cuda(z, idx, labels)
    L = _lib.lib()
    if z.dtype != torch.float32 or z.stride(1) != 1 or z.stride(0) < z.shape[1]:
        z = _f32c(z)
    n_rows, C = z.shape
    ldz = int(z.stride(0))
    n = int(idx.numel())
    idx, labels = idx.long().contiguous(), labels.long().contiguous()
    loss = torch.empty(1, dtype=torch.float32, device=z.device)
    dz = torch.empty((n_rows, ldz), dtype=torch.float32, device=z.device)
    wb = int(L.fitgnn_softmax_nll_workspace_bytes(n))
    work = torch.empty(wb, dtype=torch.uint8, device=z.device)
    _lib.check(L.fitgnn_softmax_nll_f32(_lib.dptr(z), ldz, n_rows, C, _lib.dptr(idx), _lib.dptr(labels), n, float(scale),
                                        _lib.dptr(loss), _lib.dptr(dz), _lib.dptr(work), wb, _lib.stream_ptr(z.device)),
               "fitgnn_softmax_nll_f32")
    return loss, (dz if ldz == C else dz[:, :C])


class SoftmaxNLL(torch.autograd.Function):

    @staticmethod
    def forward(ctx, z, idx, labels, scale):
        loss, dz = softmax_nll_raw(z, idx, labels, scale)
        ctx.save_for_backward(dz)
        return loss[0]

    @staticmethod
    def backward(ctx, g):
        (dz,) = ctx.saved_tensors
        return dz * g, None, None, None


def l1_loss_raw(out, tgt, scale, loss_out=None):
    _lib.require_cuda(out, tgt)
    o, t = _f32c(out).reshape(-1), _f32c(tgt).reshape(-1)
    assert o.numel() == t.numel()
    loss = loss_out if loss_out is not None else torch.empty(1, dtype=torch.float32, device=o.device)
    grad = torch.empty_like(o)
    _lib.check(_lib.lib().fitgnn_l1_loss_f32(_lib.dptr(o), _lib.dptr(t), int(o.numel()), float(scale), _lib.dptr(loss), _lib.dptr(grad),
                                             _lib.stream_ptr(o.device)), "fitgnn_l1_loss_f32")
    return loss, grad.view(out.shape)


class L1Loss(torch.autograd.Function):

    @staticmethod
    def forward(ctx, out, tgt, scale):
        _lib.require_cuda(out, tgt)
        o, t = _f32c(out).reshape(-1), _f32c(tgt).reshape(-1)
        assert o.numel() == t.numel()
        loss = torch.empty(1, dtype=torch.float32, device=o.device)
        grad = torch.empty_like(o)
# ... 177 lines not shown
    L = _lib.lib()
    _lib.require_cuda(Xc, xrow, bias, mask)
    H, dev = Xc.shape[1], Xc.device
    xcol = _entry_rows(side, xrow) if xrow is not None else None
    Y = torch.empty((g.n, H), dtype=torch.float32, device=dev)
    st = _lib.stream_ptr(dev)
    n_seg, n_ranges = int(g.seg.numel()) - 1, int(g.range_seg.numel()) - 1
    seed_v, epi_v = _seed_arg(seed, epilogue)
    ev = None
    if cfg.profile is not None:
        ev = (torch.cuda.Event(enable_timing=True), torch.cuda.Event(enable_timing=True))
        ev[0].record()
    db = None
    if dz is None:
        _lib.check(L.fitgnn_spmm_csr_stream_f32(_lib.dptr(side.rowptr), _lib.dptr(side.col), _lib.dptr(side.val), int(side.col.numel()),
                                                _lib.dptr(Xc), Xc.stride(0), _lib.dptr(Y), Y.stride(0), g.n, H, _lib.dptr(g.seg), n_seg,
                                                _lib.dptr(g.range_seg), n_ranges, _lib.dptr(xrow), _lib.dptr(xcol), _lib.dptr(bias), epi_v,
                                                float(p), seed_v, _lib.dptr(mask), st), "fitgnn_spmm_csr_stream_f32")
    else:
        prev, want_db = dz
        part = torch.empty((n_ranges, H), dtype=torch.float32, device=dev) if want_db else None
        _lib.check(L.fitgnn_spmm_csr_stream_dz_f32(_lib.dptr(side.rowptr), _lib.dptr(side.col), _lib.dptr(side.val), int(side.col.numel()),
                                                   _lib.dptr(Xc), Xc.stride(0), _lib.dptr(Y), Y.stride(0), g.n, H, _lib.dptr(g.seg), n_seg,
                                                   _lib.dptr(g.range_seg), n_ranges, _lib.dptr(xrow), _lib.dptr(xcol), _lib.dptr(prev), epi_v,
                                                   float(p), seed_v, _lib.dptr(mask), _lib.dptr(part), st), "fitgnn_spmm_csr_stream_dz_f32")
        if want_db:
            db = torch.empty(H, dtype=torch.float32, device=dev)
            _lib.check(L.fitgnn_colsum_partials_f32(_lib.dptr(part), n_ranges, H, _lib.dptr(db), st), "fitgnn_colsum_partials_f32")
    if ev is not None:
        ev[1].record()
        cfg.profile.append((ev[0], ev[1], kind or ("dz" if dz is not None else ("tile" if xrow is None else "table"))))
    return Y if dz is None else (Y, db)


def _spmm_rows_compact(g, side, Xc, xrow, zero_from, cfg, kind, dz=None, val=None):
    L = _lib.lib()
    _lib.require_cuda(Xc, xrow, val)
    val = side.val if val is None else val
    H, dev = Xc.shape[1], Xc.device
    xcol = _entry_rows(side, xrow)
    Y = torch.empty((g.n, H), dtype=torch.float32, device=dev)
    st = _lib.stream_ptr(dev)
    ev = None
    if cfg.profile is not None:
        ev = (torch.cuda.Event(enable_timing=True), torch.cuda.Event(enable_timing=True))
        ev[0].record()
    db = None
    if dz is None:
        _lib.check(L.fitgnn_spmm_rows_compact_f32(_lib.dptr(side.rowptr), _lib.dptr(xcol), _lib.dptr(val), int(side.col.numel()), _lib.dptr(Xc),
                                                  Xc.stride(0), int(zero_from), _lib.dptr(Y), Y.stride(0), g.n, H, st), "fitgnn_spmm_rows_compact_f32")
    else:
        prev, epilogue, p, seed, mask, want_db = dz
        seed_v, epi_v = _seed_arg(seed, epilogue & ~_lib.SPMM_GATHER)
        n_part = int(L.fitgnn_spmm_rows_compact_parts(g.n))
        part = torch.empty((n_part, H), dtype=torch.float32, device=dev) if want_db else None
        _lib.check(L.fitgnn_spmm_rows_compact_dz_f32(_lib.dptr(side.rowptr), _lib.dptr(xcol), _lib.dptr(val), int(side.col.numel()),
                                                     _lib.dptr(Xc), Xc.stride(0), int(zero_from), _lib.dptr(Y), Y.stride(0), g.n, H, _lib.dptr(prev),
                                                     epi_v, float(p), seed_v, _lib.dptr(mask), _lib.dptr(part), st),
                   "fitgnn_spmm_rows_compact_dz_f32")
        if want_db:
            db = torch.empty(H, dtype=torch.float32, device=dev)
            _lib.check(L.fitgnn_colsum_partials_f32(_lib.dptr(part), n_part, H, _lib.dptr(db), st), "fitgnn_colsum_partials_f32")
    if ev is not None:
        ev[1].record()
        cfg.profile.append((ev[0], ev[1], kind or ("compact" if dz is None else "compact_dz")))
    return Y if dz is None else (Y, db)


def two_hop_supported(g, link, Xc, prev, cfg):
    return (cfg.two_hop_backward and link is not None and link.g is g and Xc.shape[1] % 4 == 0 and prev.is_contiguous()
            and prev.shape[1] == Xc.shape[1] and g.t.blocks is not None and cfg.split_large_blocks)


NO_ROW = 0x7fffffff


BLOCK_PIECE_ROWS = 16
BLOCK_CARRIED = 4


def _two_hop_block_index(g, rows, pos):
    cache = getattr(g, "_two_hop_blk", None)
    if not _same_index(cache, rows):
        side, dev, R, n_sel = g.t, rows.device, g.n, int(rows.numel())
        col = side.col.long()
        counts = (side.rowptr[1:] - side.rowptr[:-1]).long()
        ar = torch.arange(R, device=dev)
        row_e = torch.repeat_interleave(ar, counts)
        blk = side.blocks.long()
        rb, cnt = blk[:, 0], blk[:, 1] - blk[:, 0]
        nb = int(blk.shape[0])
        in_rows = torch.repeat_interleave(rb, cnt) + (torch.arange(int(cnt.sum()), device=dev) - torch.repeat_interleave(torch.cumsum(cnt, 0) - cnt, cnt))
        block_of = torch.full((R,), -1, dtype=torch.int64, device=dev)
        block_of[in_rows] = torch.repeat_interleave(torch.arange(nb, device=dev), cnt)
        piece_of = torch.zeros(R, dtype=torch.int64, device=dev)
        piece_of[in_rows] = (in_rows - torch.repeat_interleave(rb, cnt)) // BLOCK_PIECE_ROWS
        carried = torch.zeros(R, dtype=torch.bool, device=dev)
        long_rows = side.long_rows.long()
        for k in range(BLOCK_CARRIED):
            sel = blk[:, 5] > k
            if bool(sel.any()):
                carried[long_rows[blk[sel, 4] + k]] = True
        pc = pos.long().index_select(0, col)
        loss_e = pc < n_sel
        b_r, b_c = block_of.index_select(0, row_e), block_of.index_select(0, col)
        served = (b_r >= 0) & (b_r == b_c) & ((piece_of.index_select(0, row_e) == piece_of.index_select(0, col)) | carried.index_select(0, col)
                                              | carried.index_select(0, row_e))
        n_loss_cols = torch.zeros(R, dtype=torch.int64, device=dev).index_add_(0, row_e, loss_e.long())
        in_zt = (block_of < 0) | carried | (n_loss_cols >= 2)
        in_zt[col[~served]] = True
        in_zt[rows.long()] = False
        other = torch.nonzero(in_zt).flatten()
        zrow = torch.full((R,), -1, dtype=torch.int64, device=dev)
        zrow[rows.long()] = torch.arange(n_sel, device=dev)
        zrow[other] = n_sel + torch.arange(other.numel(), device=dev)
        zc = zrow.index_select(0, col)
        zcol = torch.where(zc >= 0, zc, torch.full_like(zc, NO_ROW)).to(torch.int32).contiguous()
        assert bool((served | (zc >= 0)).all()), "an entry the kernel gathers has no table row"
        row_p = torch.full((R,), NO_ROW, dtype=torch.int32, device=dev)
        row_w = torch.zeros(R, dtype=torch.float32, device=dev)
        row_p[row_e[loss_e]] = pc[loss_e].to(torch.int32)
        row_w[row_e[loss_e]] = side.val[loss_e]
        tile_zt = zrow[block_of < 0]
        cache = (rows, rows._version, dict(zcol=zcol, zrow=zrow.to(torch.int32).contiguous(), zt_rows=torch.cat([rows.long(), other]).contiguous(),
                                           row_p=row_p, row_w=row_w, tile_zt=tile_zt.contiguous()))
        g._two_hop_blk = cache
    return cache[2]


def spmm_two_hop_blocks(g, Xc, prev, rows, pos, link, cfg=DEFAULT, profile_kind=None):
    L = _lib.lib()
    side = g.t
    Xc, prev = _f32c(Xc), _f32c(prev)
    _lib.require_cuda(Xc, prev, rows, pos, link.mask)
    H, dev = Xc.shape[1], Xc.device
    n_sel = int(rows.numel())
    ix = _two_hop_block_index(g, rows, pos)
    n_zt = int(ix["zt_rows"].numel())
    seed_v, epi_v = _seed_arg(link.seed, link.epi)
    st = _lib.stream_ptr(dev)
    ev = None
    if cfg.profile is not None:
        ev = (torch.cuda.Event(enable_timing=True), torch.cuda.Event(enable_timing=True))
        ev[0].record()
    ZT = torch.empty((max(n_zt, 1), H), dtype=torch.float32, device=dev)
    _lib.check(L.fitgnn_two_hop_rows_f32(_lib.dptr(side.rowptr), _lib.dptr(ix["zcol"]), _lib.dptr(side.val), _lib.dptr(Xc), Xc.stride(0), n_sel,
                                         _lib.dptr(ix["zt_rows"]), n_zt, _lib.dptr(prev), H, epi_v, float(link.p), seed_v, _lib.dptr(link.mask),
                                         _lib.dptr(ZT), ZT.stride(0), st), "fitgnn_two_hop_rows_f32")
    Y = torch.empty((g.n, H), dtype=torch.float32, device=dev)
    quiet = cfg if cfg.profile is None else cfg.replace(profile=None)
    if side.small_tiles.shape[0]:
        spmm_raw(side.rowptr, side.col, side.val, side.small_tiles, ZT, g.n, window_rows=g.window_rows, out=Y, cfg=quiet, xrow=ix["zrow"])
    n_blocks = int(side.blocks.shape[0])
    part = torch.zeros((n_blocks + 1, H), dtype=torch.float32, device=dev) if link.want_db else None
    _lib.check(L.fitgnn_spmm_two_hop_blocks_f32(_lib.dptr(side.rowptr), _lib.dptr(side.col), _lib.dptr(side.val), _lib.dptr(ZT), ZT.stride(0),
                                                _lib.dptr(Y), Y.stride(0), g.n, H, _lib.dptr(side.blocks), n_blocks, _lib.dptr(side.long_rows),
                                                _lib.dptr(ix["zrow"]), _lib.dptr(ix["zcol"]), _lib.dptr(prev), _lib.dptr(Xc), Xc.stride(0), n_sel,
                                                _lib.dptr(ix["row_p"]), _lib.dptr(ix["row_w"]), epi_v, float(link.p), seed_v, _lib.dptr(link.mask),
                                                _lib.dptr(part), st), "fitgnn_spmm_two_hop_blocks_f32")
    db = None
    if link.want_db:
        if ix["tile_zt"].numel():
            torch.sum(ZT.index_select(0, ix["tile_zt"]), 0, out=part[n_blocks])
        db = _fold_partials(part, dev, st)
    if ev is not None:
        ev[1].record()
        cfg.profile.append((ev[0], ev[1], profile_kind or "two_hop"))
    return Y, db


def _fold_partials(part, dev, st):
    L = _lib.lib()
    n_part, H = int(part.shape[0]), int(part.shape[1])
    if n_part > 8192:
        G = 1024
        per = n_part // G
        head = part[: G * per].view(G, per, H).sum(1)
        part = torch.cat([head, part[G * per:]]) if n_part > G * per else head
        n_part = int(part.shape[0])
    db = torch.empty(H, dtype=torch.float32, device=dev)
    _lib.check(L.fitgnn_colsum_partials_f32(_lib.dptr(part.contiguous()), n_part, H, _lib.dptr(db), st), "fitgnn_colsum_partials_f32")
    return db


def spmm_graph_dz(g, X, prev, epilogue, p=0.0, seed=0, mask=None, want_db=True, transposed=True, xrow=None, cfg=DEFAULT, profile_kind=None,
                  zero_from=-1):
    side = g.t if transposed else g.f
    Xc, prev = _f32c(X), _f32c(prev)
    _lib.require_cuda(Xc, prev, mask, xrow)
    L = _lib.lib()
    H = Xc.shape[1]
    if xrow is not None and zero_from >= 0 and cfg.compact_rows_kernel and H % 4 == 0 and g.n >= cfg.rows_kernel_min_rows:
        return _spmm_rows_compact(g, side, Xc, xrow, zero_from, cfg, profile_kind, dz=(prev, epilogue, p, seed, mask, want_db))
    if (side.blocks is not None and cfg.split_large_blocks and cfg.stream_kernel and g.seg is not None and zero_from < 0 and H % 4 == 0
            and Xc.stride(0) % 4 == 0):
        return _spmm_stream(g, side, Xc, xrow, cfg, profile_kind, epilogue=epilogue & ~_lib.SPMM_GATHER, p=p, seed=seed, mask=mask,
                            dz=(prev, want_db))
    dev = Xc.device
    seed_v, epi_v = _seed_arg(seed, epilogue & ~_lib.SPMM_GATHER)
    split = side.blocks is not None and cfg.split_large_blocks
    tiles = side.small_tiles if split else side.tiles
    n_tiles = int(tiles.shape[0])
    n_blocks = int(side.blocks.shape[0]) if split else 0
    Y = torch.empty((g.n, H), dtype=torch.float32, device=dev)
    part = (_scratch((n_tiles, H), dev) if n_blocks == 0 else torch.zeros((n_tiles + n_blocks, H), dtype=torch.float32, device=dev)) if want_db else None
    st = _lib.stream_ptr(dev)
    ev = None
    if cfg.profile is not None:
        ev = (torch.cuda.Event(enable_timing=True), torch.cuda.Event(enable_timing=True))
        ev[0].record()
    if n_tiles:
        _lib.check(L.fitgnn_spmm_csr_dz_f32(_lib.dptr(side.rowptr), _lib.dptr(side.col), _lib.dptr(side.val), _lib.dptr(Xc), Xc.stride(0),
                                            _lib.dptr(Y), Y.stride(0), g.n, H, _lib.dptr(tiles), n_tiles,
                                            _lib.dptr(None if split else side.lcol), _lib.dptr(None if split else side.win_cols),
                                            _lib.dptr(xrow), int(zero_from), int(g.window_rows), _lib.dptr(prev), epi_v, float(p), seed_v,
                                            _lib.dptr(mask), _lib.dptr(part), st), "fitgnn_spmm_csr_dz_f32")
    if n_blocks:
        xcol = None
        if xrow is not None:
            xcol = _entry_rows(side, xrow)
        _lib.check(L.fitgnn_spmm_csr_blocks_dz_f32(_lib.dptr(side.rowptr), _lib.dptr(side.col), _lib.dptr(side.val), _lib.dptr(Xc), Xc.stride(0),
                                                   _lib.dptr(Y), Y.stride(0), g.n, H, _lib.dptr(side.blocks), n_blocks, _lib.dptr(side.long_rows),
                                                   _lib.dptr(xrow), _lib.dptr(xcol), int(zero_from), _lib.dptr(prev), epi_v, float(p), seed_v, _lib.dptr(mask),
                                                   _lib.dptr(None if part is None else part[n_tiles:]), st), "fitgnn_spmm_csr_blocks_dz_f32")
    if ev is not None:
        ev[1].record()
        cfg.profile.append((ev[0], ev[1], profile_kind or "dz"))
    db = None
    if want_db:
        n_part = n_tiles + n_blocks
        if n_part > 8192:
            G = 1024
            per = n_part // G
            head = part[: G * per].view(G, per, H).sum(1)
            part2 = torch.cat([head, part[G * per:]]) if n_part > G * per else head
            db = torch.empty(H, dtype=torch.float32, device=dev)
            _lib.check(L.fitgnn_colsum_partials_f32(_lib.dptr(part2), int(part2.shape[0]), H, _lib.dptr(db), st), "fitgnn_colsum_partials_f32")
        else:
            db = torch.empty(H, dtype=torch.float32, device=dev)
            _lib.check(L.fitgnn_colsum_partials_f32(_lib.dptr(part), n_part, H, _lib.dptr(db), st), "fitgnn_colsum_partials_f32")
    return Y, db


def epilogue_bwd_head_raw(dy, Wl, out, epilogue, p=0.0, seed=0, mask=None, want_db=True, want_dWl=True):
    _lib.require_cuda(dy, Wl, out, mask)
    L = _lib.lib()
    dy, Wl, out = _f32c(dy), _f32c(Wl), _f32c(out)
    n, H = out.shape
    C = Wl.shape[0]
    seed, epilogue = _seed_arg(seed, epilogue)
    dZ = torch.empty_like(out)
    db = torch.empty(H, dtype=torch.float32, device=out.device) if want_db else None
    dWl = torch.empty((C, H), dtype=torch.float32, device=out.device) if want_dWl else None
    wb = int(L.fitgnn_epilogue_bwd_head_workspace_bytes(n, H, C))
    work = torch.empty(max(wb, 4), dtype=torch.uint8, device=out.device)
    rc = L.fitgnn_epilogue_bwd_head_f32(_lib.dptr(dy), _lib.dptr(Wl), C, _lib.dptr(out), _lib.dptr(dZ), n, H, epilogue, float(p),
                                        seed, _lib.dptr(mask), _lib.dptr(db), _lib.dptr(dWl),
                                        _lib.dptr(work), wb, _lib.stream_ptr(out.device))
    _lib.check(rc, "fitgnn_epilogue_bwd_head_f32")
    return dZ, db, dWl


ZERO_ROWS = 256


def epilogue_bwd_head_rows_raw(dy, Wl, out, rows, epilogue, p=0.0, seed=0, mask=None, want_db=True, want_dWl=True, inputs_compact=False,
                               zero_rows=ZERO_ROWS, db_out=None, dWl_out=None):
    _lib.require_cuda(dy, Wl, out, mask, rows)
    L = _lib.lib()
    dy, Wl, out = _f32c(dy), _f32c(Wl), _f32c(out)
    rows = (rows if rows.dtype == torch.int64 else rows.long()).contiguous()
    n_sel, H = int(rows.numel()), out.shape[1]
    C = Wl.shape[0]
    seed, epilogue = _seed_arg(seed, epilogue)
    dZc = torch.empty((n_sel + zero_rows, H), dtype=torch.float32, device=out.device)
    if zero_rows:
        dZc[n_sel:].zero_()
    db = (db_out if db_out is not None else torch.empty(H, dtype=torch.float32, device=out.device)) if want_db else None
    dWl = (dWl_out if dWl_out is not None else torch.empty((C, H), dtype=torch.float32, device=out.device)) if want_dWl else None
    wb = int(L.fitgnn_epilogue_bwd_head_workspace_bytes(n_sel, H, C))
    work = torch.empty(max(wb, 4), dtype=torch.uint8, device=out.device)
    rc = L.fitgnn_epilogue_bwd_head_rows_f32(_lib.dptr(dy), _lib.dptr(Wl), C, _lib.dptr(out), _lib.dptr(rows), n_sel, 1 if inputs_compact else 0,
                                             _lib.dptr(dZc), H, epilogue, float(p), seed, _lib.dptr(mask), _lib.dptr(db), _lib.dptr(dWl),
                                             _lib.dptr(work), wb, _lib.stream_ptr(out.device))
    _lib.check(rc, "fitgnn_epilogue_bwd_head_rows_f32")
    return dZc, db, dWl


def epilogue_fwd_rows_(z, rows, bias, epilogue, p=0.0, seed=0, mask=None):
    _lib.require_cuda(z, rows, bias, mask)
    seed, epilogue = _seed_arg(seed, epilogue)
    rows = (rows if rows.dtype == torch.int64 else rows.long()).contiguous()
    _lib.check(_lib.lib().fitgnn_epilogue_fwd_rows_f32(_lib.dptr(z), z.stride(0), _lib.dptr(rows), z.shape[0], z.shape[1],
                                                       _lib.dptr(None if bias is None else _f32c(bias)), epilogue, float(p), seed,
                                                       _lib.dptr(mask), _lib.stream_ptr(z.device)), "fitgnn_epilogue_fwd_rows_f32")
    return z


def _compact_positions(g, rows):
    cache = getattr(g, "_compact_pos", None)
    if not _same_index(cache, rows):
        pos = int(rows.numel()) + torch.arange(g.n, dtype=torch.int32, device=rows.device) % ZERO_ROWS
        pos[rows.long()] = torch.arange(rows.numel(), dtype=torch.int32, device=rows.device)
        cache = (rows, rows._version, pos)
        g._compact_pos = cache
    return cache[2]


def head_rows_supported(out, Wl):
    H, C = out.shape[1], Wl.shape[0]
    return (out.is_cuda and out.dtype == torch.float32 and Wl.dtype == torch.float32 and H % 4 == 0 and out.stride(1) == 1
            and out.stride(0) % 4 == 0 and _lib.lib().fitgnn_head_rows_lds_bytes(H, C) <= 160 * 1024)


def head_rows(out, rows, Wl, bl, n_total=None):
    _lib.require_cuda(out, rows, Wl, bl)
    compact = n_total is not None
    R, H = (int(n_total) if compact else out.shape[0]), out.shape[1]
    C = Wl.shape[0]
    Wl = _f32c(Wl)
    y = torch.zeros((R, C), dtype=torch.float32, device=out.device)
    rows = rows if rows.dtype == torch.int64 else rows.long()
    _lib.check(_lib.lib().fitgnn_head_rows_f32(_lib.dptr(out), out.stride(0), _lib.dptr(rows.contiguous()), rows.numel(), _lib.dptr(Wl),
                                               _lib.dptr(None if bl is None else _f32c(bl)), C, H, _lib.dptr(y), C, 1 if compact else 0,
                                               _lib.stream_ptr(out.device)), "fitgnn_head_rows_f32")
    return y


_LDS_BYTES = 160 * 1024


def _fits_lds(nbytes):
    return 0 < nbytes <= _LDS_BYTES


def _lds_rows(lds_bytes, H):
    per_row = int(lds_bytes(1, int(H)))
    return _LDS_BYTES // per_row if per_row > 0 else 0


def _f32_on_gpu(params):
    return all(p is None or (p.is_cuda and p.dtype == torch.float32 and p.is_contiguous()) for p in params)


def gcn_query_gather(rowptr, col, val, T, rows, xrow=None, b0=None, out=None):
    _lib.require_cuda(rowptr, col, val, T, rows, xrow, b0)
    Q, H = int(rows.numel()), int(T.shape[1])
    G = out if out is not None else torch.empty((Q, H), dtype=torch.float32, device=T.device)
    _lib.check(_lib.lib().fitgnn_gcn_query_gather_f32(_lib.dptr(rowptr), _lib.dptr(col), _lib.dptr(val), _lib.dptr(T), T.stride(0),
                                                      _lib.dptr(xrow), _lib.dptr(b0), _lib.dptr(rows), Q, H, _lib.dptr(G), G.stride(0),
                                                      _lib.stream_ptr(T.device)), "fitgnn_gcn_query_gather_f32")
    return G


def gcn_query_tail(G, W1, b1, Wl, bl, log_softmax=False, out=None):
    _lib.require_cuda(G, W1, b1, Wl, bl)
    Q, H = int(G.shape[0]), int(G.shape[1])
    H2, C = int(W1.shape[0]), int(Wl.shape[0])
# ... 543 lines not shown
        if aggregated:
            return _f32c(dOut), db
        return spmm_graph(g, _f32c(dOut), transposed=True, cfg=cfg), db
    plain = not (cfg.fold_backward and getattr(g, "fold_ok", False))
    dH, db, _ = layer_backward(g, out, ep.bwd, ep.p, ep.seed, mask, has_bias, dOut=dOut, cfg=cfg, db_out=db_out if plain else None)
    return dH, db


class FusedGCNLayer(torch.autograd.Function):

    @staticmethod
    def forward(ctx, X, W, b, g, p, training, seed, mask, link_in, link_out, cfg):
        X = _f32c(X)
        Hm = mm_xwt(X, W, cfg)
        ep = _Epilogue(b is not None, p, training, seed, mask)
        out = spmm_graph(g, Hm, bias=b, epilogue=ep.fwd, p=ep.p, seed=ep.seed, mask=ep.mask, cfg=cfg)
        ctx.save_for_backward(X, W, out, ep.mask)
        ctx.g, ctx.ep, ctx.has_bias, ctx.cfg = g, ep, b is not None, cfg
        ctx.link_in, ctx.link_out = link_in, link_out
        ctx.ptrs = _addresses(W, b)
        if link_out is not None:
            link_out.record(ep.drop, ep.p, ep.seed, ep.mask, b is not None, g=g)
        return out

    @staticmethod
    def backward(ctx, dOut):
        X, W, out, mask = ctx.saved_tensors
        cfg = ctx.cfg
        sink, (pW, pb) = _GradSink(cfg.grad_sink), ctx.ptrs
        sb = sink.slice(pb) if (ctx.has_bias and ctx.needs_input_grad[2]) else None
        dH, db = _producer_backward(cfg, ctx.link_out, ctx.g, out, ctx.ep, mask, ctx.has_bias, dOut, db_out=sb)
        dW = sink.result(mm_at_b(dH, X, cfg, out=sink.slice(pW))) if ctx.needs_input_grad[1] else None
        dX = _dx_through_link(cfg, ctx.link_in, dH, W, X) if ctx.needs_input_grad[0] else None
        return dX, dW, (sink.result(db) if ctx.has_bias else None), None, None, None, None, None, None, None, None


def narrow_input_supported(x, W, cfg=DEFAULT):
    if not (cfg.narrow_input_first and x.is_cuda and x.dim() == 2 and not x.requires_grad and x.shape[0] > 0):
        return False
    K, H = int(x.shape[1]), int(W.shape[0])
    L = _lib.lib()
    return K < H and bool(L.fitgnn_dense_narrow_k_lds_bytes(K, H)) and bool(L.fitgnn_narrow_atb_workspace_bytes(int(x.shape[0]), K, H))


def aggregated_input(g, x, cfg=DEFAULT):
    cache = getattr(g, "_agg_input", None)
    if cache is None or cache[0] is not x or cache[1] != x._version:
        with torch.no_grad():
            ax = spmm_graph(g, _f32c(x), cfg=cfg.replace(profile=None) if cfg.profile is not None else cfg)
        cache = (x, x._version, ax)
        g._agg_input = cache
    return cache[2]


class FusedGCNLayerAggregatedInput(torch.autograd.Function):

    @staticmethod
    def forward(ctx, AX, W, b, p, training, seed, mask, link_out, cfg):
        L = _lib.lib()
        n, K = AX.shape
        H = int(W.shape[0])
        Wc = _f32c(W)
        ep = _Epilogue(b is not None, p, training, seed, mask)
        out = torch.empty((n, H), dtype=torch.float32, device=AX.device)
        seed_v, epi_v = _seed_arg(ep.seed, ep.fwd)
        rc = L.fitgnn_dense_narrow_k_f32(_lib.dptr(AX), AX.stride(0), _lib.dptr(Wc), Wc.stride(0), n, K, H, _lib.dptr(b), epi_v,
                                         float(ep.p), seed_v, _lib.dptr(ep.mask), _lib.dptr(out), out.stride(0),
                                         _lib.stream_ptr(AX.device))
        _lib.check(rc, "fitgnn_dense_narrow_k_f32")
        ctx.save_for_backward(AX, out, ep.mask)
        ctx.ep, ctx.has_bias, ctx.cfg, ctx.link_out, ctx.H = ep, b is not None, cfg, link_out, H
        ctx.ptrs = _addresses(W, b)
        if link_out is not None:
            link_out.record(ep.drop, ep.p, ep.seed, ep.mask, b is not None, g=None)
        return out

    @staticmethod
    def backward(ctx, dOut):
        AX, out, mask = ctx.saved_tensors
        L = _lib.lib()
        n, K = AX.shape
        H = ctx.H
        dOut = _f32c(dOut)
        ep, link = ctx.ep, ctx.link_out
        prev, epi = out, ep.bwd
        if link is not None and link.take() is not None:
            prev, epi = None, 0
        seed_v, epi_v = _seed_arg(ep.seed, epi)
        sink, (pW, pb) = _GradSink(ctx.cfg.grad_sink), ctx.ptrs
        want_dW, want_db = ctx.needs_input_grad[1], ctx.has_bias and ctx.needs_input_grad[2]
        dW = sink.buffer(pW if want_dW else None, (H, K), dOut.device)
        db = sink.buffer(pb if want_db else None, H, dOut.device)
        wb = int(L.fitgnn_narrow_atb_workspace_bytes(n, K, H))
        work = torch.empty(wb // 4, dtype=torch.float32, device=dOut.device)
        rc = L.fitgnn_narrow_atb_f32(_lib.dptr(dOut), dOut.stride(0), _lib.dptr(prev), epi_v, float(ep.p), seed_v,
                                     _lib.dptr(mask), _lib.dptr(AX), AX.stride(0), n, K, H, _lib.dptr(dW), _lib.dptr(db), _lib.dptr(work), wb,
                                     _lib.stream_ptr(dOut.device))
        _lib.check(rc, "fitgnn_narrow_atb_f32")
        return None, (sink.result(dW) if want_dW else None), (sink.result(db) if want_db else None), None, None, None, None, None, None


class FusedGCNLayerHead(torch.autograd.Function):

    @staticmethod
    def forward(ctx, X, W, b, Wl, bl, g, p, training, seed, mask, link_in, cfg, loss_rows=None):
        X = _f32c(X)
        ctx.link_in, ctx.cfg, ctx.loss_rows = link_in, cfg, loss_rows
        Hm = mm_xwt(X, W, cfg)
        ep = _Epilogue(b is not None, p, training, seed, mask)
        out = spmm_graph(g, Hm, bias=b, epilogue=ep.fwd, p=ep.p, seed=ep.seed, mask=ep.mask, cfg=cfg)
        if loss_rows is not None and head_rows_supported(out, Wl):
            y = head_rows(out, loss_rows, Wl, bl)
        else:
            y = torch.mm(out, Wl.t())
            if bl is not None:
                y = y + bl
        ctx.save_for_backward(X, W, Wl, out, ep.mask)
        ctx.g, ctx.ep, ctx.has_bias, ctx.has_bl = g, ep, b is not None, bl is not None
        return y

    @staticmethod
    def backward(ctx, dy):
        X, W, Wl, out, mask = ctx.saved_tensors
        dy = _f32c(dy)
        cfg, ep = ctx.cfg, ctx.ep
        dH, db, dWl = layer_backward(ctx.g, out, ep.bwd, ep.p, ep.seed, mask, ctx.has_bias, dy=dy, Wl=Wl, want_dWl=ctx.needs_input_grad[3],
                                     cfg=cfg, loss_rows=ctx.loss_rows)
        dy_l = dy if ctx.loss_rows is None else dy.index_select(0, ctx.loss_rows)
        dbl = colsum_narrow(dy_l) if ctx.has_bl and ctx.needs_input_grad[4] else None
        dW = mm_at_b(dH, X, cfg) if ctx.needs_input_grad[1] else None
        dX = _dx_through_link(cfg, ctx.link_in, dH, W, X) if ctx.needs_input_grad[0] else None
        return dX, dW, (db if ctx.has_bias else None), dWl, dbl, None, None, None, None, None, None, None, None


def _arange_rows(g, n, device):
    cache = getattr(g, "_arange_rows", None)
    if cache is None or cache.numel() != n or cache.device != device:
        cache = torch.arange(n, dtype=torch.int64, device=device)
        g._arange_rows = cache
    return cache


def _dense_rows(AHc, W, b, rows, ep, cfg):
    if cfg.fused_gemm_epilogue and _exact(cfg, AHc, W) and W.shape[0] % 4 == 0:
        outc = gemm_exact_epi(AHc, W, rows, b, ep.fwd, p=ep.p, seed=ep.seed, mask=ep.mask, cfg=cfg)
        if outc is not None:
            return outc
    outc = mm_xwt(AHc, W, cfg)
    if not outc.is_contiguous():
        outc = outc.contiguous()
    return epilogue_fwd_rows_(outc, rows, b, ep.fwd, p=ep.p, seed=ep.seed, mask=ep.mask)


def _head_rows_fwd(outc, Wl, bl, rows, n_total, compact_out, g, cfg):
    if _exact(cfg, outc, Wl) and Wl.shape[0] >= 16:
        y = gemm_exact_epi(outc, Wl, None, bl, EPI_BIAS, cfg=cfg) if (cfg.fused_gemm_epilogue and bl is not None) else None
        if y is None:
            y = gemm_exact(outc, Wl, "nt", cfg)
            if bl is not None:
                y = y + bl
        if not compact_out:
            y = torch.zeros((n_total, y.shape[1]), dtype=torch.float32, device=y.device).index_copy_(0, rows, y)
        return y
    if compact_out:
        return head_rows(outc, _arange_rows(g, rows.numel(), rows.device), Wl, bl, n_total=rows.numel())
    return head_rows(outc, rows, Wl, bl, n_total=n_total)


def _head_rows_bwd(dy, rows, compact_out, outc, Wl, ep, mask, has_bias, want_dWl, want_dbl, cfg, sink, pb=None, pWl=None, pbl=None):
    H, C = outc.shape[1], Wl.shape[0]
    dy_c = _f32c(dy) if compact_out else _f32c(dy).index_select(0, rows)
    inside = want_dWl and bool(_lib.lib().fitgnn_epilogue_bwd_head_supported(H, C, 1))
    dZc, db, dWl = epilogue_bwd_head_rows_raw(dy_c, Wl, outc, rows, ep.bwd, p=ep.p, seed=ep.seed, mask=mask, want_db=has_bias,
                                              want_dWl=inside, inputs_compact=True, zero_rows=0, db_out=sink.slice(pb),
                                              dWl_out=sink.slice(pWl) if inside else None)
    if want_dWl and not inside:
        dWl = head_weight_grad_rows(dy_c, outc, cfg)
    dbl = colsum_narrow(dy_c, out=sink.slice(pbl)) if want_dbl else None
    return dZc, sink.result(db), sink.result(dWl), sink.result(dbl)


def _rows_adjoint(g, dZc, W, rows, link, Xprev, cfg, zero_tail, two_hop=False):
    n, K = dZc.shape[0], W.shape[1]
    dAH = torch.empty((n + ZERO_ROWS, K), dtype=torch.float32, device=dZc.device)
    if zero_tail:
        dAH[n:].zero_()
    mm_by_transposed(dZc, W, cfg, out=dAH[:n])
    if two_hop and Xprev is not None and two_hop_supported(g, link, dAH, Xprev, cfg):
        dX, db_prev = spmm_two_hop_blocks(g, dAH, Xprev, rows, _compact_positions(g, rows), link, cfg=cfg)
        link.hand_back(db_prev, aggregated=True)
    elif Xprev is not None:
        dX, db_prev = spmm_graph_dz(g, dAH, Xprev, link.epi, p=link.p, seed=link.seed, mask=link.mask, want_db=link.want_db,
                                    xrow=_compact_positions(g, rows), cfg=cfg, profile_kind="compact_dz", zero_from=n)
        link.hand_back(db_prev)
    else:
        dX = spmm_graph(g, dAH, transposed=True, cfg=cfg, xrow=_compact_positions(g, rows), profile_kind="compact", zero_from=n)
    return dX


class FusedGCNLastLayerRows(torch.autograd.Function):

    @staticmethod
    def forward(ctx, X, W, b, Wl, bl, g, p, training, seed, mask, rows, cfg, link_in=None, compact_out=False, fwd_sub=None):
        X = _f32c(X)
        rows = rows if rows.dtype == torch.int64 else rows.long()
        ctx.link_in, ctx.compact_out = link_in, bool(compact_out)
        if fwd_sub is not None:
            f = fwd_sub.f
            AHc = spmm_raw(f.rowptr, f.col, f.val, f.tiles, X, fwd_sub.m, window_rows=fwd_sub.window_rows, cfg=cfg, profile_kind="rows_fwd")
        else:
            AH = spmm_graph(g, X, cfg=cfg)
            AHc = AH.index_select(0, rows)
            del AH
        ep = _Epilogue(b is not None, p, training, seed, mask)
        outc = _dense_rows(AHc, W, b, rows, ep, cfg)
        y = _head_rows_fwd(outc, Wl, bl, rows, g.n, compact_out, g, cfg)
        keep_x = link_in is not None and cfg.fuse_dx_epilogue and X.shape[1] % 4 == 0
        ctx.save_for_backward(W, Wl, AHc, outc, rows, ep.mask, X if keep_x else None)
        ctx.g, ctx.ep, ctx.has_bias, ctx.has_bl, ctx.cfg = g, ep, b is not None, bl is not None, cfg
        ctx.ptrs = _addresses(W, b, Wl, bl)
        return y

    @staticmethod
    def backward(ctx, dy):
        W, Wl, AHc, outc, rows, mask, Xprev = ctx.saved_tensors
        cfg = ctx.cfg
        sink, (pW, pb, pWl, pbl) = _GradSink(cfg.grad_sink), ctx.ptrs
        dZc, db, dWl, dbl = _head_rows_bwd(dy, rows, ctx.compact_out, outc, Wl, ctx.ep, mask, ctx.has_bias, ctx.needs_input_grad[3],
                                           ctx.has_bl and ctx.needs_input_grad[4], cfg, sink, pb=pb if ctx.needs_input_grad[2] else None,
                                           pWl=pWl, pbl=pbl)
        dW = sink.result(mm_at_b(dZc, AHc, cfg, out=sink.slice(pW))) if ctx.needs_input_grad[1] else None
        dX = _rows_adjoint(ctx.g, dZc, W, rows, ctx.link_in, Xprev, cfg, zero_tail=True, two_hop=True) if ctx.needs_input_grad[0] else None
        return dX, dW, (db if ctx.has_bias else None), dWl, dbl, None, None, None, None, None, None, None, None, None, None


class FusedGCNLayerRows(torch.autograd.Function):

    @staticmethod
    def forward(ctx, X, W, b, g, p, training, seed, mask, rows, cfg, link_in=None):
        X = _f32c(X)
        rows = rows if rows.dtype == torch.int64 else rows.long()
        AHc = spmm_graph(g, X, cfg=cfg).index_select(0, rows)
        ep = _Epilogue(b is not None, p, training, seed, mask)
        outc = _dense_rows(AHc, W, b, rows, ep, cfg)
        keep_x = link_in is not None and cfg.fuse_dx_epilogue and X.shape[1] % 4 == 0
        ctx.save_for_backward(W, AHc, outc, rows, ep.mask, X if keep_x else None)
        ctx.g, ctx.ep, ctx.has_bias, ctx.cfg, ctx.link_in = g, ep, b is not None, cfg, link_in
        ctx.ptrs = _addresses(W, b)
        return outc

    @staticmethod
    def backward(ctx, dOutc):
        W, AHc, outc, rows, mask, Xprev = ctx.saved_tensors
        cfg, ep = ctx.cfg, ctx.ep
        sink, (pW, pb) = _GradSink(cfg.grad_sink), ctx.ptrs
        sb = sink.slice(pb) if (ctx.has_bias and ctx.needs_input_grad[2]) else None
        dZc, db = epilogue_bwd_rows_raw(dOutc, outc, rows, ep.bwd, p=ep.p, seed=ep.seed, mask=mask, want_db=ctx.has_bias, db_out=sb)
        dW = sink.result(mm_at_b(dZc, AHc, cfg, out=sink.slice(pW))) if ctx.needs_input_grad[1] else None
        dX = _rows_adjoint(ctx.g, dZc, W, rows, ctx.link_in, Xprev, cfg, zero_tail=False) if ctx.needs_input_grad[0] else None
        return dX, dW, (sink.result(db) if ctx.has_bias else None), None, None, None, None, None, None, None, None


class FusedGCNLayerDedup(torch.autograd.Function):

    @staticmethod
    def forward(ctx, Xt, W, b, g, ridx, p, training, seed, mask, link_out, cfg):
        Xt = _f32c(Xt)
        ctx.link_out, ctx.cfg = link_out, cfg
        ctx.wide = _padded_table_path(Xt, W, cfg)
        ctx.exact_pad = (cfg.gemm_precision == "exact" and Xt.is_cuda and Xt.shape[1] % 4 != 0 and not Xt.requires_grad
                         and W.shape[0] % 4 == 0)
        if ctx.exact_pad:
            Xp = padded_table(Xt)
            Ht = gemm_exact(Xp, padded_weight(W, Xp.shape[1]), "nt", cfg)
        else:
            Ht = gemm_nt_padded_k(padded_table(Xt), W, cfg) if ctx.wide else mm_xwt(Xt, W, cfg)
        ep = _Epilogue(b is not None, p, training, seed, mask)
        out = spmm_graph(g, Ht, bias=b, epilogue=ep.fwd | (_lib.SPMM_GATHER if cfg.dedup_gather else 0), p=ep.p, seed=ep.seed, mask=ep.mask,
                         xrow=ridx.index, cfg=cfg)
        ctx.save_for_backward(Xt, W, out, ep.mask)
        ctx.g, ctx.ridx, ctx.ep, ctx.has_bias = g, ridx, ep, b is not None
        ctx.ptrs = _addresses(W)
        if link_out is not None:
            link_out.record(ep.drop, ep.p, ep.seed, ep.mask, b is not None, g=g)
        return out

    @staticmethod
    def backward(ctx, dOut):
        Xt, W, out, mask = ctx.saved_tensors
        g, ridx = ctx.g, ctx.ridx
        cfg = ctx.cfg
        dH, db = _producer_backward(cfg, ctx.link_out, g, out, ctx.ep, mask, ctx.has_bias, dOut)
        dHt = segment_sum(ridx.seg_off, ridx.members, dH, ridx.n_table)
        if ctx.exact_pad and ctx.needs_input_grad[1]:
            dW = gemm_exact(_f32c(dHt), padded_table(Xt), "tn", cfg)[:, : Xt.shape[1]]
        elif ctx.wide and ctx.needs_input_grad[1]:
            dW = gemm_atb(_f32c(dHt), padded_table(Xt), cfg)[:, : Xt.shape[1]]
        elif ctx.needs_input_grad[1]:
            sink, (pW,) = _GradSink(cfg.grad_sink), ctx.ptrs
            dW = sink.result(mm_at_b(dHt, Xt, cfg, out=sink.slice(pW)))
        else:
            dW = None
        dXt = mm(dHt, W) if ctx.needs_input_grad[0] else None
        return dXt, dW, (db if ctx.has_bias else None), None, None, None, None, None, None, None, None


class GATAggregate(torch.autograd.Function):

    @staticmethod
    def forward(ctx, h, att_src, att_dst, bias, g, slope, act, p, training, seed, mask, cfg, ridx=None, link_out=None):
        L = _lib.lib()
        h = _f32c(h)
        nh, C = h.shape
        n = g.n
        dev = h.device
        st = _lib.stream_ptr(dev)
        a_src = torch.empty(nh, dtype=torch.float32, device=dev)
        a_dst = torch.empty(nh, dtype=torch.float32, device=dev)
        att_src, att_dst = _f32c(att_src.reshape(-1)), _f32c(att_dst.reshape(-1))
        with _timed(cfg, "gat_scores"):
            _lib.check(L.fitgnn_gat_scores_f32(_lib.dptr(h), C, nh, C, _lib.dptr(att_src), _lib.dptr(att_dst), _lib.dptr(a_src),
                                               _lib.dptr(a_dst), st), "gat_scores")
            if ridx is not None:
                a_src, a_dst = a_src.index_select(0, ridx.index.long()), a_dst.index_select(0, ridx.index.long())
        alpha = torch.empty(g.nnz, dtype=torch.float32, device=dev)
        with _timed(cfg, "gat_edge_softmax"):
            _lib.check(L.fitgnn_gat_edge_softmax_f32(_lib.dptr(g.f.rowptr), _lib.dptr(g.f.col), _lib.dptr(a_src), _lib.dptr(a_dst),
                                                     float(slope), n, _lib.dptr(alpha), st), "gat_edge_softmax")
        ep = _Epilogue(bias is not None, p, training, seed, mask, act=act)
        out = spmm_graph(g, h, val=alpha, bias=bias, epilogue=ep.fwd, p=ep.p, seed=ep.seed, mask=ep.mask, cfg=cfg,
                         profile_kind="gat_aggregate", xrow=None if ridx is None else ridx.index)
        ctx.save_for_backward(h, att_src, att_dst, a_src, a_dst, alpha, out if act else None, ep.mask)
        ctx.g, ctx.slope, ctx.has_bias, ctx.cfg, ctx.ridx = g, slope, bias is not None, cfg, ridx
        ctx.act, ctx.ep = bool(act), ep
        ctx.link_out = link_out if act else None
        if ctx.link_out is not None:
            link_out.record(ep.drop, ep.p, ep.seed, ep.mask, bias is not None, g=None)
        return out

    @staticmethod
    def backward(ctx, dOut):
        h, att_src, att_dst, a_src, a_dst, alpha, out, mask = ctx.saved_tensors
        g, L = ctx.g, _lib.lib()
        dOut = _f32c(dOut)
        db_fused = None
        cfg, ep = ctx.cfg, ctx.ep
        taken = ctx.link_out.take() if ctx.link_out is not None else None
        if taken is not None:
            db_fused = taken[0]
        elif ctx.act:
            with _timed(cfg, "gat_epilogue_bwd"):
                dOut, db_fused = epilogue_bwd_raw(dOut, out, ep.bwd, p=ep.p, seed=ep.seed, mask=mask, want_db=ctx.has_bias)
        C = h.shape[1]
        n = g.n
        ridx = ctx.ridx
        dev = h.device
        st = _lib.stream_ptr(dev)
        dalpha = torch.empty_like(alpha)
        ecol = g.f.col if ridx is None else _entry_rows(g.f, ridx.index)
        with _timed(cfg, "gat_sddmm"):
            _lib.check(L.fitgnn_sddmm_csr_f32(_lib.dptr(g.f.rowptr), _lib.dptr(ecol), _lib.dptr(dOut), C, _lib.dptr(h), C, n, C,
                                              _lib.dptr(dalpha), st), "sddmm")
        ds = torch.empty_like(alpha)
        da_dst = torch.empty(n, dtype=torch.float32, device=dev)
        with _timed(cfg, "gat_softmax_bwd"):
            _lib.check(L.fitgnn_gat_softmax_bwd_f32(_lib.dptr(g.f.rowptr), _lib.dptr(g.f.col), _lib.dptr(a_src), _lib.dptr(a_dst),
                                                    _lib.dptr(alpha), _lib.dptr(dalpha), float(ctx.slope), n, _lib.dptr(ds),
                                                    _lib.dptr(da_dst), st), "gat_softmax_bwd")
        with _timed(cfg, "gat_transpose_edges"):
            ds_t = ds[g._perm_t].contiguous()
            da_src = torch.empty(n, dtype=torch.float32, device=dev)
            _lib.check(L.fitgnn_csr_row_sum_f32(_lib.dptr(g.t.rowptr), _lib.dptr(ds_t), n, _lib.dptr(da_src), st), "csr_row_sum")
            alpha_t = alpha[g._perm_t].contiguous()
        dh = spmm_graph(g, dOut, transposed=True, val=alpha_t, cfg=ctx.cfg, profile_kind="gat_aggregate_t")
        with _timed(cfg, "gat_rank1"):
            da = torch.stack([da_src, da_dst], dim=1)
            if ridx is not None:
                dh = segment_sum(ridx.seg_off, ridx.members, dh, ridx.n_table)
                da = segment_sum(ridx.seg_off, ridx.members, da, ridx.n_table)
            dh.addmm_(da, torch.stack([att_src, att_dst], dim=0))
        datt = mm_at_b(da, h, ctx.cfg) if (ctx.needs_input_grad[1] or ctx.needs_input_grad[2]) else None
        datt_src = datt[0] if ctx.needs_input_grad[1] else None
        datt_dst = datt[1] if ctx.needs_input_grad[2] else None
        if ctx.act:
            db = db_fused if ctx.has_bias else None
        else:
            db = dOut.sum(0) if ctx.has_bias and ctx.needs_input_grad[3] else None
        return dh, datt_src, datt_dst, db, None, None, None, None, None, None, None, None, None, None


def _gat_rank2_csr(g, rows, pos):
    cache = getattr(g, "_gat_rank2", None)
    if not _same_index(cache, rows):
        side, dev, R, n = g.t, rows.device, g.n, int(rows.numel())
        rp = side.rowptr.long()
        ar = torch.arange(R + 1, device=dev)
        rp_aug = rp + 2 * ar
        cnt = (rp[1:] - rp[:-1])
        row_e = torch.repeat_interleave(ar[:-1], cnt)
        main = torch.arange(int(rp[-1]), device=dev) + 2 * row_e
        ext = rp_aug[1:] - 2
        posz = pos.long()
        posz = torch.where(posz >= n, posz + 2, posz)
        xcol_aug = torch.empty(int(rp_aug[-1]), dtype=torch.int32, device=dev)
        xcol_aug[main] = posz.index_select(0, side.col.long()).to(torch.int32)
        xcol_aug[ext] = n
        xcol_aug[ext + 1] = n + 1
        cache = (rows, rows._version, (rp_aug.to(torch.int32).contiguous(), xcol_aug, main, ext))
        g._gat_rank2 = cache
    return cache[2]

# ... 432 lines not shown
```

include/fitgnn_hip.h:

```cpp
#ifndef FITGNN_HIP_H
#define FITGNN_HIP_H

#include <stddef.h>
#include <stdint.h>

#ifdef __cplusplus
extern "C" {
#endif

#define FITGNN_ABI_VERSION 1
#define FITGNN_MAX_K 16

#define FITGNN_E_BADARG (-1)
#define FITGNN_E_WORKSPACE (-2)
#define FITGNN_E_ALIGN (-3)

int fitgnn_abi_version(void);
const char *fitgnn_error_string(int code);

int fitgnn_stream_copy_f32(const float *src, float *dst, int64_t n, void *stream);


typedef struct fitgnn_tile {
    int32_t row_begin, row_end;
    int32_t win_begin;
    int32_t win_rows;
    int32_t nnz_begin, nnz_end;
    int32_t reserved[2];
} fitgnn_tile_t;

int fitgnn_plan_tiles_host(const int32_t *rowptr, const int32_t *col, int32_t n_rows, int32_t n_cols,
                           const int64_t *block_ptr, int32_t n_blocks, int32_t max_rows, int32_t max_window,
                           fitgnn_tile_t *tiles, int32_t *n_tiles, int32_t *win_cols, int32_t *n_win, int32_t *lcol);

int fitgnn_make_tiles_host(const int64_t *ptr, int64_t n_blocks, int32_t max_rows, int32_t *tiles4, int64_t capacity, int64_t *n_tiles);
int fitgnn_split_blocks_host(const int64_t *ptr, int64_t n_blocks, const int32_t *rowptr, int32_t cap, int64_t limit, int32_t long_row,
                             int32_t *tiles4, int64_t tiles_capacity, int64_t *n_tiles, int32_t *blocks8, int64_t *n_large,
                             int32_t *long_rows, int64_t long_capacity, int64_t *n_long);

typedef struct fitgnn_block {
    int32_t row_begin, row_end;
    int32_t nnz_begin, nnz_end;
    int32_t long_off, n_long;
    int32_t reserved[2];
} fitgnn_block_t;

int fitgnn_spmm_csr_blocks_f32(const int32_t *rowptr, const int32_t *col, const float *val, const float *X, int64_t ldx,
                               float *Y, int64_t ldy, int32_t n_rows, int32_t H, const fitgnn_block_t *blocks,
                               int32_t n_blocks, const int32_t *long_rows, const int32_t *xrow, const int32_t *xcol,
                               int32_t xrow_zero_from, const float *bias, uint32_t epilogue, float p_drop, uint64_t seed,
                               const uint8_t *mask, void *stream);

int fitgnn_spmm_csr_dz_f32(const int32_t *rowptr, const int32_t *col, const float *val, const float *X, int64_t ldx, float *Y,
                           int64_t ldy, int32_t n_rows, int32_t H, const fitgnn_tile_t *tiles, int32_t n_tiles, const int32_t *lcol,
                           const int32_t *win_cols, const int32_t *xrow, int32_t xrow_zero_from, int32_t window_rows, const float *prev,
                           uint32_t epilogue, float p_drop, uint64_t seed, const uint8_t *mask, float *col_part, void *stream);
int fitgnn_spmm_csr_blocks_dz_f32(const int32_t *rowptr, const int32_t *col, const float *val, const float *X, int64_t ldx, float *Y,
                                  int64_t ldy, int32_t n_rows, int32_t H, const fitgnn_block_t *blocks, int32_t n_blocks,
                                  const int32_t *long_rows, const int32_t *xrow, const int32_t *xcol, int32_t xrow_zero_from,
                                  const float *prev, uint32_t epilogue, float p_drop, uint64_t seed, const uint8_t *mask,
                                  float *col_part, void *stream);

int32_t fitgnn_lanczos_parts(int32_t n);
int fitgnn_lanczos_spmv_f64(const int32_t *rowptr, const int32_t *col, const double *val, const double *x, double *y, int32_t n,
                            double alpha, double beta, void *stream);
int fitgnn_lanczos_project_f64(const double *V, int64_t ldv, int32_t ncol, double *w, int32_t n, const double *h_in, double *part_out,
                               void *stream);
int fitgnn_lanczos_reduce_f64(const double *part, int32_t n_part, int32_t ncol1, double *out, void *stream);
int fitgnn_lanczos_finish_f64(double *V, int64_t ldv, int32_t j, const double *w, int32_t n, const double *ha, const double *hb,
                              const double *hc, double *H, int32_t ldh, void *stream);
int fitgnn_lanczos_rotate_f64(const double *V, int64_t ldv, int32_t m, const double *S, int32_t nk, double *out, int64_t ldo, int32_t n,
                              void *stream);

int fitgnn_spmm_csr_stream_f32(const int32_t *rowptr, const int32_t *col, const float *val, int64_t nnz, const float *X, int64_t ldx,
                               float *Y, int64_t ldy, int32_t n_rows, int32_t H, const int32_t *seg_ptr, int32_t n_seg,
                               const int32_t *range_seg, int32_t n_ranges, const int32_t *xrow, const int32_t *xcol, const float *bias,
                               uint32_t epilogue, float p_drop, uint64_t seed, const uint8_t *mask, void *stream);
int fitgnn_spmm_csr_stream_dz_f32(const int32_t *rowptr, const int32_t *col, const float *val, int64_t nnz, const float *X, int64_t ldx,
                                  float *Y, int64_t ldy, int32_t n_rows, int32_t H, const int32_t *seg_ptr, int32_t n_seg,
                                  const int32_t *range_seg, int32_t n_ranges, const int32_t *xrow, const int32_t *xcol, const float *prev,
                                  uint32_t epilogue, float p_drop, uint64_t seed, const uint8_t *mask, float *col_part, void *stream);

int32_t fitgnn_spmm_rows_compact_parts(int32_t n_rows);
int fitgnn_spmm_rows_compact_f32(const int32_t *rowptr, const int32_t *xcol, const float *val, int64_t nnz, const float *X, int64_t ldx,
                                 int32_t zero_from, float *Y, int64_t ldy, int32_t n_rows, int32_t H, void *stream);
int fitgnn_spmm_rows_compact_dz_f32(const int32_t *rowptr, const int32_t *xcol, const float *val, int64_t nnz, const float *X, int64_t ldx,
                                    int32_t zero_from, float *Y, int64_t ldy, int32_t n_rows, int32_t H, const float *prev,
                                    uint32_t epilogue, float p_drop, uint64_t seed, const uint8_t *mask, float *col_part, void *stream);

int fitgnn_two_hop_rows_f32(const int32_t *rowptr, const int32_t *zcol, const float *val, const float *Xc, int64_t ldx, int32_t zero_from,
                            const int64_t *zt_rows, int32_t n_zt, const float *prev, int32_t H, uint32_t epilogue, float p_drop,
                            uint64_t seed, const uint8_t *mask, float *ZT, int64_t ldz, void *stream);
int fitgnn_spmm_two_hop_blocks_f32(const int32_t *rowptr, const int32_t *col, const float *val, const float *ZT, int64_t ldz, float *Y,
                                   int64_t ldy, int32_t n_rows, int32_t H, const fitgnn_block_t *blocks, int32_t n_blocks,
                                   const int32_t *long_rows, const int32_t *zrow, const int32_t *zcol, const float *prev, const float *Xc,
                                   int64_t ldx, int32_t zero_from, const int32_t *row_p, const float *row_w, uint32_t epilogue,
                                   float p_drop, uint64_t seed, const uint8_t *mask, float *col_part, void *stream);


int fitgnn_spmm_default_window_rows(void);
int fitgnn_spmm_max_window_rows(int32_t H);

int fitgnn_gcn_norm_csr_f32(const int32_t *rowptr, const int32_t *col, const float *w, float *val, float *dinv,
                            int32_t n_rows, void *stream);

#define FITGNN_EPI_BIAS 1u
#define FITGNN_EPI_ELU 2u
#define FITGNN_EPI_DROPOUT 4u
#define FITGNN_EPI_SEED_DEVICE 8u
#define FITGNN_EPI_BACKWARD 0x10u
#define FITGNN_SPMM_GATHER 0x100u

int fitgnn_spmm_csr_f32(const int32_t *rowptr, const int32_t *col, const float *val, const float *X, int64_t ldx,
                        float *Y, int64_t ldy, int32_t n_rows, int32_t H, const fitgnn_tile_t *tiles,
                        int32_t n_tiles, const int32_t *lcol, const int32_t *win_cols, const int32_t *xrow,
                        int32_t xrow_zero_from, int32_t window_rows, const float *bias, uint32_t epilogue, float p_drop,
                        uint64_t seed, const uint8_t *mask, void *stream);

int fitgnn_segment_sum_f32(const int32_t *seg_off, const int32_t *members, int32_t n_seg, const float *X, int64_t ldx,
                           int32_t F, float *out, int64_t ldo, void *stream);

int fitgnn_segment_max_f32(const int32_t *seg_off, const int32_t *members, int32_t n_seg, const float *X, int64_t ldx, int32_t F,
                           float *out, int32_t *arg, void *stream);
int fitgnn_segment_max_bwd_f32(const float *g, const int32_t *arg, int32_t n_seg, int32_t F, float *dst, int64_t ldd, void *stream);
int fitgnn_segment_expand_f32(const float *src, const int32_t *seg_of_row, const float *scale, int64_t n_rows, int32_t F, float *dst,
                              void *stream);

int fitgnn_pool_head_supported(int32_t F, int32_t C);
int fitgnn_pool_head_f32(const int32_t *seg_off, const int32_t *members, int32_t n_seg, const float *X, int64_t ldx, int32_t F,
                         const float *inv_cnt, const float *W, const float *b, int32_t C, float *pooled, float *y, void *stream);
int fitgnn_pool_head_bwd_f32(const float *dy, const float *W, int32_t C, const float *pooled, const int32_t *seg_of_row,
                             const float *inv_cnt, int64_t n_rows, int32_t n_seg, int32_t F, float *dx, float *dW, float *db,
                             void *stream);

int fitgnn_sum_leading_f32(const float *part, int32_t B, int64_t W, float *out, void *stream);

size_t fitgnn_gemm_atb_workspace_bytes(int64_t R, int32_t M, int32_t N);
int fitgnn_gemm_atb_f32(const float *a, int64_t lda, const float *b, int64_t ldb, int64_t R, int32_t M, int32_t N,
                        float *out, void *workspace, void *stream);

int fitgnn_gemm_nt_f32(const float *a, int64_t lda, const float *b, int64_t ldb, int64_t R, int32_t N, int32_t K,
                       float *c, int64_t ldc, void *stream);

size_t fitgnn_gemm_exact_workspace_bytes(int64_t I, int32_t J, int64_t K, int32_t a_kmajor, int32_t b_kmajor);
int fitgnn_gemm_exact_f32(const float *a, int64_t lda, int32_t a_kmajor, const float *b, int64_t ldb, int32_t b_kmajor,
                          int64_t I, int32_t J, int64_t K, float *c, int64_t ldc, void *workspace, void *stream);
int fitgnn_gemm_exact_plan(int64_t I, int32_t J, int64_t K, int32_t a_kmajor, int32_t b_kmajor, int32_t *shape, int32_t *nchunks,
                           int64_t *main_rows);
int fitgnn_gemm_exact_epi_f32(const float *a, int64_t lda, const float *b, int64_t ldb, int64_t I, int32_t J, int64_t K, float *c,
                              int64_t ldc, const int64_t *rows, const float *bias, uint32_t epilogue, float p_drop, uint64_t seed,
                              const uint8_t *mask, void *workspace, void *stream);

size_t fitgnn_gemm_nt_presplit_bytes(int32_t N, int32_t K);
int fitgnn_gemm_nt_presplit_f32(const float *b, int64_t stride_n, int64_t stride_k, int32_t N, int32_t K, int32_t K_valid,
                                void *image, void *stream);
int fitgnn_gemm_nt_pre_f32(const float *a, int64_t lda, const void *b_image, int64_t R, int32_t N, int32_t K, float *c,
                           int64_t ldc, void *stream);

size_t fitgnn_gemm_nt_epilogue_bwd_workspace_bytes(int64_t R, int32_t N);
int fitgnn_gemm_nt_epilogue_bwd_f32(const float *a, int64_t lda, const float *b, int64_t ldb, int64_t R, int32_t N, int32_t K,
                                    const float *out, float *dZ, uint32_t epilogue, float p_drop, uint64_t seed,
                                    const uint8_t *mask, float *db, void *work, size_t work_bytes, void *stream);

size_t fitgnn_head_rows_lds_bytes(int32_t H, int32_t C);
int fitgnn_head_rows_f32(const float *out, int64_t ldo, const int64_t *rows, int32_t n_rows, const float *Wl, const float *bl,
                         int32_t C, int32_t H, float *y, int64_t ldy, int32_t out_compact, void *stream);

size_t fitgnn_colsum_narrow_workspace_bytes(int32_t n_rows, int32_t C);
int fitgnn_colsum_narrow_f32(const float *x, int64_t ldx, int32_t n_rows, int32_t C, float *out, void *work, size_t work_bytes,
                             void *stream);

int fitgnn_colsum_partials_f32(const float *partial, int32_t n_chunks, int32_t H, float *out, void *stream);

int fitgnn_l1_loss_f32(const float *out, const float *tgt, int32_t n, float scale, float *loss, float *grad, void *stream);

size_t fitgnn_softmax_nll_workspace_bytes(int32_t n);
int fitgnn_softmax_nll_f32(const float *z, int64_t ldz, int32_t n_rows, int32_t C, const int64_t *idx,
                           const int64_t *labels, int32_t n, float scale, float *loss, float *dz, void *work,
                           size_t work_bytes, void *stream);

int fitgnn_adam_step_f32(float *param, const float *grad, float *exp_avg, float *exp_avg_sq, int64_t n, float lr,
                         float beta1, float beta2, float eps, float weight_decay, float *step, void *stream);

int fitgnn_adam_step_acc_f32(float *param, float *grad_acc, float *grad_new, float *exp_avg, float *exp_avg_sq, int64_t n, float lr,
                             float beta1, float beta2, float eps, float weight_decay, float *state, uint64_t *seeds, int32_t n_seeds,
                             uint64_t seed_stride, void *stream);

size_t fitgnn_epilogue_bwd_workspace_bytes(int32_t n_rows, int32_t H);
int fitgnn_epilogue_bwd_f32(const float *dOut, const float *out, float *dZ, int32_t n_rows, int32_t H,
                            uint32_t epilogue, float p_drop, uint64_t seed, const uint8_t *mask, float *db,
                            void *work, size_t work_bytes, void *stream);

int fitgnn_head_max_classes(void);
int fitgnn_head_max_classes_wide(void);
int fitgnn_epilogue_bwd_head_supported(int32_t H, int32_t C, int32_t with_dWl);
size_t fitgnn_epilogue_bwd_head_workspace_bytes(int32_t n_rows, int32_t H, int32_t C);
int fitgnn_epilogue_bwd_head_f32(const float *dy, const float *Wl, int32_t C, const float *out, float *dZ,
                                 int32_t n_rows, int32_t H, uint32_t epilogue, float p_drop, uint64_t seed,
                                 const uint8_t *mask, float *db, float *dWl, void *work, size_t work_bytes, void *stream);

int fitgnn_epilogue_bwd_head_rows_f32(const float *dy, const float *Wl, int32_t C, const float *out, const int64_t *rows,
                                      int32_t n_sel, int32_t inputs_compact, float *dZc, int32_t H, uint32_t epilogue, float p_drop,
                                      uint64_t seed, const uint8_t *mask, float *db, float *dWl, void *work, size_t work_bytes,
                                      void *stream);

int fitgnn_epilogue_bwd_rows_f32(const float *dOut, const float *out, const int64_t *rows, int32_t n_sel, int32_t inputs_compact, float *dZc,
                                 int32_t H, uint32_t epilogue, float p_drop, uint64_t seed, const uint8_t *mask, float *db, void *work,
                                 size_t work_bytes, void *stream);

int fitgnn_epilogue_fwd_rows_f32(float *z, int64_t ldz, const int64_t *rows, int32_t n, int32_t H, const float *bias,
                                 uint32_t epilogue, float p_drop, uint64_t seed, const uint8_t *mask, void *stream);

size_t fitgnn_dense_narrow_k_lds_bytes(int32_t K, int32_t H);
int fitgnn_dense_narrow_k_f32(const float *a, int64_t lda, const float *W, int64_t ldw, int32_t n, int32_t K, int32_t H,
                              const float *bias, uint32_t epilogue, float p_drop, uint64_t seed, const uint8_t *mask, float *out,
                              int64_t ldo, void *stream);

size_t fitgnn_narrow_atb_workspace_bytes(int32_t n, int32_t K, int32_t H);
int fitgnn_narrow_atb_f32(const float *d, int64_t ldd, const float *prev, uint32_t epilogue, float p_drop, uint64_t seed,
                          const uint8_t *mask, const float *a, int64_t lda, int32_t n, int32_t K, int32_t H, float *dW, float *db,
                          void *work, size_t work_bytes, void *stream);

int fitgnn_spmm_epilogue_bwd_supported(int32_t H, int32_t C, int32_t window_rows);
size_t fitgnn_spmm_epilogue_bwd_workspace_bytes(int32_t n_tiles, int32_t H, int32_t C);
int fitgnn_spmm_epilogue_bwd_f32(const int32_t *rowptr, const int32_t *col, const float *val, const fitgnn_tile_t *tiles,
                                 int32_t n_tiles, int32_t window_rows, const float *dOut, const float *dy, const float *Wl,
                                 int32_t C, const float *out, float *dH, int32_t n_rows, int32_t H, uint32_t epilogue,
                                 float p_drop, uint64_t seed, const uint8_t *mask, float *db, float *dWl, void *work,
                                 size_t work_bytes, void *stream);

int fitgnn_gat_scores_f32(const float *h, int64_t ldh, int32_t n, int32_t C, const float *att_src, const float *att_dst,
                          float *a_src, float *a_dst, void *stream);
int fitgnn_gat_edge_softmax_f32(const int32_t *rowptr, const int32_t *col, const float *a_src, const float *a_dst,
                                float negative_slope, int32_t n, float *alpha, void *stream);
int fitgnn_sddmm_csr_f32(const int32_t *rowptr, const int32_t *col, const float *dOut, int64_t ldo, const float *h,
                         int64_t ldh, int32_t n, int32_t C, float *dalpha, void *stream);
int fitgnn_gat_softmax_bwd_f32(const int32_t *rowptr, const int32_t *col, const float *a_src, const float *a_dst,
                               const float *alpha, const float *dalpha, float negative_slope, int32_t n, float *ds,
                               float *da_dst, void *stream);
int fitgnn_sddmm_csr_rows_f32(const int32_t *rowptr, const int32_t *col, const float *dOut_c, int64_t ldo, const float *h, int64_t ldh,
                              const int64_t *sel, int32_t n_sel, int32_t C, float *dalpha, void *stream);
int fitgnn_gat_softmax_bwd_rows_f32(const int32_t *rowptr, const int32_t *col, const float *a_src, const float *a_dst,
                                    const float *alpha, const float *dalpha, float negative_slope, const int64_t *sel, int32_t n_sel,
                                    float *ds, float *da_dst, void *stream);
int fitgnn_csr_row_sum_f32(const int32_t *rowptr, const float *v, int32_t n, float *y, void *stream);

int fitgnn_spmm_narrow_f32(const int32_t *rowptr, const int32_t *col, const float *val, const float *X, float *Y,
                           int32_t n_rows, int32_t H, float beta, const float *Z0, float gamma, float *ACC, float delta,
                           void *stream);
int fitgnn_spmm_narrow_padded_f32(const int32_t *rowptr, const int32_t *col, const float *val, const float *X, float *Y,
                                  int32_t n_rows, int32_t h4, float beta, const float *Z0, float gamma, float *ACC, float delta,
                                  void *stream);

int fitgnn_gather_rows_padded_f32(const float *src, int64_t lds, int32_t H, const int32_t *index, int64_t n_rows, float *dst, int32_t h4,
                                  void *stream);

int fitgnn_appnp_unit_rows(int32_t h4);
int fitgnn_appnp_unit_entries(void);
int fitgnn_appnp_units_f32(const int32_t *rowptr, const int32_t *col, const float *val, const int32_t *units, int32_t n_units, int32_t max_rows,
                           int32_t max_entries, const float *X, float *Y, int32_t h4, int32_t K, float alpha, int32_t backward, void *stream);

int fitgnn_appnp_block_rows(void);
int fitgnn_appnp_block_entries(void);
int fitgnn_appnp_blocks_f32(const int32_t *rowptr, const int32_t *col, const float *val, const int32_t *blocks, int32_t n_blocks, int32_t max_rows,
                            int32_t max_entries, const float *X, float *Y, float *T1, float *T2, int32_t h4, int32_t K, float alpha,
                            int32_t backward, void *stream);

int64_t fitgnn_appnp_lds_bytes(int32_t max_rows, int32_t max_entries, int32_t slice);
int fitgnn_appnp_lds_max_bytes(void);
int fitgnn_appnp_lds_items_per_thread(void);
int fitgnn_appnp_lds_f32(const int32_t *rowptr, const int32_t *col, const float *val, const int32_t *ranges, int32_t n_ranges, int32_t max_rows,
                         int32_t max_entries, const float *X, float *Y, int32_t h4, int32_t K, float alpha, int32_t backward, int32_t threads,
                         int32_t slice, void *stream);


int fitgnn_gcn_query_gather_f32(const int32_t *rowptr, const int32_t *col, const float *val, const float *T, int64_t ldt,
                                const int32_t *xrow, const float *b0, const int64_t *rows, int32_t Q, int32_t H, float *G, int64_t ldg,
                                void *stream);

int fitgnn_gat_query_gather_f32(const int32_t *rowptr, const int32_t *col, const float *T, int64_t ldt, const int32_t *xrow,
                                const float *a_src0, const float *a_dst0, const float *b0, float slope0, const float *u_src,
                                const float *u_dst, float slope1, const int64_t *rows, int32_t Q, int32_t H, float *G, int64_t ldg,
                                void *stream);

int fitgnn_sage_query_gather_f32(const int32_t *rowptr, const int32_t *col, const float *val, const float *T, int64_t ldt,
                                 const int32_t *xrow, const float *b0, const int64_t *rows, int32_t Q, int32_t H, float *G,
                                 int64_t ldg, void *stream);

size_t fitgnn_gcn_query_tail_lds_bytes(int32_t H2, int32_t C);
int fitgnn_gcn_query_tail_f32(const float *G, int64_t ldg, int32_t Q, const float *W1, const float *b1, const float *Wl, const float *bl,
                              int32_t H, int32_t H2, int32_t C, float *out, int64_t ldo, int32_t log_softmax, void *stream);

size_t fitgnn_gcn_graph_query_hops_lds_bytes(int32_t max_rows, int32_t H);
int fitgnn_gcn_graph_query_hops_f32(const int32_t *rowptr, const int32_t *col, const float *val, const float *T, int64_t ldt,
                                    const int32_t *xrow, const float *b0, const int64_t *seg, const int64_t *prow, const int64_t *pptr,
                                    int32_t Q, int32_t H, int32_t max_rows, float *G, int64_t ldg, void *stream);

size_t fitgnn_gcn_graph_query_tail_lds_bytes(int32_t H2, int32_t C);
int fitgnn_gcn_graph_query_tail_f32(const float *G, int64_t ldg, const int64_t *pptr, int32_t Q, const float *W1, const float *b1,
                                    const float *Wl, const float *bl, int32_t H, int32_t H2, int32_t C, int32_t pool, int32_t softmax,
                                    float *out, int64_t ldo, void *stream);

int fitgnn_gin_query_hops_f32(const int32_t *rowptr, const int32_t *col, const float *val, const float *T, int64_t ldt,
                              const int32_t *xrow, const float *b0a, const float *eps0, const float *W0b, const float *b0b,
// ... 166 lines not shown
```

Before: 3.619 billion.

## Fuse row gathers into exact GEMM operand loads and vectorize epilogue stores

Adds row-index lists to the exact f32 GEMM so A rows (forward) and B k-rows (dW backward) are gathered inside the slab loads. This removes the separate index_select copies of the aggregated features in the row-selected GCN layers. It also adds an LDS-staged epilogue that writes float4 groups with bias, ELU and dropout applied, and replaces some zero-filled partial buffers with uninitialized scratch plus an explicit zero of the tail row. The cost is extra index loads and new template instantiations, and gathered rows may hurt load coalescing.

```diff
diff --git a/fit-gnn_amd/csrc/gemm_f32.hip b/fit-gnn_amd/csrc/gemm_f32.hip
--- a/fit-gnn_amd/csrc/gemm_f32.hip
+++ b/fit-gnn_amd/csrc/gemm_f32.hip
@@ -46,6 +46,55 @@
     }
 }
 
+struct RowLists {
+    const int64_t *a_rows, *b_rows;
+};
+
+template <int NV, int THREADS>
+__device__ __forceinline__ void slab_row_offsets(long (&ro)[NV], const int64_t *__restrict__ list, long ld, long t0, long lim) {
+    const int tid = threadIdx.x;
+#pragma unroll
+    for (int p = 0; p < NV; ++p) {
+        long i = t0 + ((tid + p * THREADS) >> 3);
+        i = i < lim ? i : lim - 1;
+        ro[p] = (list ? (long)list[i] : i) * ld;
+    }
+}
+
+template <int NV, int THREADS>
+__device__ __forceinline__ void load_slab_rows(float4 (&r)[NV], const float *__restrict__ P, const long (&ro)[NV], long k0, long klim) {
+    const int tid = threadIdx.x;
+#pragma unroll
+    for (int p = 0; p < NV; ++p) {
+        const long k = k0 + 4 * ((tid + p * THREADS) & 7);
+        r[p] = k < klim ? *reinterpret_cast<const float4 *>(P + ro[p] + k) : make_float4(0.f, 0.f, 0.f, 0.f);
+    }
+}
+
+template <int T, int NV, int THREADS>
+__device__ __forceinline__ void slab_k_rows(long (&kx)[NV], const int64_t *__restrict__ list, long k0, long klim) {
+    constexpr int Q = T / 4;
+#pragma unroll
+    for (int p = 0; p < NV; ++p) {
+        long k;
+        if constexpr (Q % 64 == 0) k = k0 + (__builtin_amdgcn_readfirstlane((int)(threadIdx.x >> 6)) * 64 + p * THREADS) / Q;
+        else k = k0 + ((int)threadIdx.x + p * THREADS) / Q;
+        kx[p] = k < klim ? (list ? (long)list[k] : k) : -1;
+    }
+}
+
+template <int T, int NV, int THREADS>
+__device__ __forceinline__ void load_slab_k_rows(float4 (&r)[NV], const float *__restrict__ P, long ld, long t0, long lim, const long (&kx)[NV]) {
+    constexpr int Q = T / 4;
+    const int tid = threadIdx.x;
+#pragma unroll
+    for (int p = 0; p < NV; ++p) {
+        long i = t0 + 4 * ((tid + p * THREADS) % Q);
+        i = i + 4 <= lim ? i : lim - 4;
+        r[p] = kx[p] >= 0 ? *reinterpret_cast<const float4 *>(P + kx[p] * ld + i) : make_float4(0.f, 0.f, 0.f, 0.f);
+    }
+}
+
 template <bool KM, int T, int NV, int THREADS>
 __device__ __forceinline__ void store_slab(const float4 (&r)[NV], float *lds) {
     const int tid = threadIdx.x;
@@ -83,12 +132,30 @@
     long row0;
     uint32_t epi;
     float p_drop;
+    int vec;
 };
 
-template <int WM, int WN, int MI, int NJ, bool AKM, bool BKM, bool EPI>
-__global__ __launch_bounds__(64 * WM * WN) void gemm_f32_kernel(const float *__restrict__ A, long lda, const float *__restrict__ B, long ldb,
-                                                                   long I, int J, long K, float *__restrict__ C, long ldc, int tiles_i,
-                                                                   int tiles_j, int nchunks, long chunk_k, StoreEpi se) {
+__device__ __forceinline__ float4 finish_group(float4 x, const float (&bias)[4], uint32_t epi, float keep_scale, uint32_t thresh, uint64_t seed,
+                                               const uint8_t *__restrict__ mask, uint64_t idx) {
+    float y[4] = {x.x, x.y, x.z, x.w};
+    uint64_t bits = 0;
+    if ((epi & 4u) && !mask) bits = fitgnn::dropout_bits(seed, idx >> 2);
+#pragma unroll
+    for (int q = 0; q < 4; ++q) {
+        y[q] = y[q] + ((epi & 1u) ? bias[q] : 0.f);
+        if (epi & 2u) y[q] = y[q] > 0.f ? y[q] : __expf(y[q]) - 1.0f;
+        if (epi & 4u) {
+            const bool keep = mask ? (mask[idx + q] != 0) : fitgnn::dropout_keep(bits, q, thresh);
+            y[q] = keep ? y[q] * keep_scale : 0.f;
+        }
+    }
+    return make_float4(y[0], y[1], y[2], y[3]);
+}
+
+template <int WM, int WN, int MI, int NJ, bool AKM, bool BKM, bool EPI, bool IDX>
+__device__ __forceinline__ void gemm_f32_tile(const float *__restrict__ A, long lda, const float *__restrict__ B, long ldb, long I, int J, long K,
+                                              float *__restrict__ C, long ldc, int tiles_i, int tiles_j, int nchunks, long chunk_k,
+                                              const StoreEpi &se, const RowLists &rl) {
     using G = Geo<WM, WN, MI, NJ, AKM, BKM>;
     extern __shared__ __attribute__((aligned(16))) float lds_f[];
     const int lane = threadIdx.x & 63, wave = __builtin_amdgcn_readfirstlane(threadIdx.x >> 6);
@@ -120,9 +187,25 @@
             for (int r = 0; r < 16; ++r) acc[i][j][r] = 0.f;
 
     float4 ra[G::NA], rb[G::NB];
+    constexpr bool AIDX = IDX && !AKM, BIDX = IDX && BKM;
+    long a_ro[AIDX ? G::NA : 1], b_kx[BIDX ? G::NB : 1];
+    auto load_a = [&](long k0) {
+        if constexpr (AIDX) load_slab_rows<G::NA, G::THREADS>(ra, A, a_ro, k0, k_end);
+        else load_slab<AKM, G::TI, G::NA, G::THREADS>(ra, A, lda, i0, I, k0, k_end);
+    };
+    auto load_b = [&](long k0) {
+        if constexpr (BIDX) {
+            load_slab_k_rows<G::TJ, G::NB, G::THREADS>(rb, B, ldb, j0, (long)J, b_kx);
+        } else {
+            load_slab<BKM, G::TJ, G::NB, G::THREADS>(rb, B, ldb, j0, (long)J, k0, k_end);
+        }
+    };
     if (nstage > 0) {
-        load_slab<AKM, G::TI, G::NA, G::THREADS>(ra, A, lda, i0, I, k_begin, k_end);
-        load_slab<BKM, G::TJ, G::NB, G::THREADS>(rb, B, ldb, j0, (long)J, k_begin, k_end);
+        if constexpr (AIDX) slab_row_offsets<G::NA, G::THREADS>(a_ro, rl.a_rows, lda, i0, I);
+        if constexpr (BIDX) slab_k_rows<G::TJ, G::NB, G::THREADS>(b_kx, rl.b_rows, k_begin, k_end);
+        load_a(k_begin);
+        load_b(k_begin);
+        if constexpr (BIDX) slab_k_rows<G::TJ, G::NB, G::THREADS>(b_kx, rl.b_rows, k_begin + kBK, k_end);
         store_slab<AKM, G::TI, G::NA, G::THREADS>(ra, lds_f);
         store_slab<BKM, G::TJ, G::NB, G::THREADS>(rb, lds_f + G::A_DW);
     }
@@ -151,14 +234,17 @@
             float fa[MI][4], fb[NJ][4];
             read_frags(fa, fb, sa, sb, kk);
             multiply(fa, fb);
+            if constexpr (BIDX) {
+                if (kk == 0) slab_k_rows<G::TJ, G::NB, G::THREADS>(b_kx, rl.b_rows, k_begin + (long)(s + 2) * kBK, k_end);
+            }
         }
     };
     for (int s = 0; s < nstage; ++s) {
         const bool more = s + 1 < nstage;
         if (more) {
             const long k0 = k_begin + (long)(s + 1) * kBK;
-            load_slab<AKM, G::TI, G::NA, G::THREADS>(ra, A, lda, i0, I, k0, k_end);
-            load_slab<BKM, G::TJ, G::NB, G::THREADS>(rb, B, ldb, j0, (long)J, k0, k_end);
+            load_a(k0);
+            load_b(k0);
         }
         products(s);
         if (more) {
@@ -175,6 +261,45 @@
         const uint64_t seed = fitgnn::resolve_seed(se.seed, se.epi);
         const float keep_scale = (se.epi & FITGNN_EPI_DROPOUT) ? 1.0f / (1.0f - se.p_drop) : 1.0f;
         const uint32_t thresh = fitgnn::dropout_threshold(se.p_drop);
+        if (se.vec) {
+            constexpr int W = 32 * NJ, P = W + 8, RPP = 256 / W, NP = 32 / RPP;
+            static_assert(WM * WN * 32 * P * 4 <= G::LDS_BYTES, "the store regions fit the operand LDS");
+            float *reg = lds_f + wave * (32 * P);
+            const int c4 = lane % (W / 4), rsub = lane / (W / 4);
+            const long col = j0 + wn * W + 4 * c4;
+            const bool col_ok = col < J;
+            float bv[4];
+#pragma unroll
+            for (int q = 0; q < 4; ++q) bv[q] = ((se.epi & FITGNN_EPI_BIAS) && col_ok) ? se.bias[col + q] : 0.f;
+#pragma unroll
+            for (int q = 0; q < 4; ++q) asm volatile("" ::"v"(bv[q]));
+#pragma unroll
+            for (int i = 0; i < MI; ++i) {
+                const long rbase = i0 + wm * (32 * MI) + i * 32;
+                long orow[NP];
+#pragma unroll
+                for (int ps = 0; ps < NP; ++ps) {
+                    const long row = rbase + ps * RPP + rsub;
+                    orow[ps] = row < I ? (se.rows ? (long)se.rows[row] : se.row0 + row) : 0;
+                }
+#pragma unroll
+                for (int j = 0; j < NJ; ++j)
+#pragma unroll
+                    for (int r = 0; r < 16; ++r) reg[((r & 3) + 8 * (r >> 2) + 4 * (lane >> 5)) * P + j * 32 + (lane & 31)] = acc[i][j][r];
+#pragma unroll
+                for (int ps = 0; ps < NP; ++ps) asm volatile("" ::"v"(orow[ps]));
+#pragma unroll
+                for (int ps = 0; ps < NP; ++ps) {
+                    const int rr = ps * RPP + rsub;
+                    const long row = rbase + rr;
+                    const float4 x = *reinterpret_cast<const float4 *>(reg + rr * P + 4 * c4);
+                    if (row < I && col_ok)
+                        *reinterpret_cast<float4 *>(out + row * ldo + col) =
+                            finish_group(x, bv, se.epi, keep_scale, thresh, seed, se.mask, (uint64_t)orow[ps] * (uint64_t)J + (uint64_t)col);
+                }
+            }
+            return;
+        }
 #pragma unroll
         for (int i = 0; i < MI; ++i) {
             const long row0 = i0 + wm * (32 * MI) + i * 32 + 4 * (lane >> 5);
@@ -185,9 +310,12 @@
                 orow[r] = row < I ? (se.rows ? (long)se.rows[row] : se.row0 + row) : 0;
             }
 #pragma unroll
+            for (int r = 0; r < 16; ++r) asm volatile("" ::"v"(orow[r]));
+#pragma unroll
             for (int j = 0; j < NJ; ++j) {
                 const long col = j0 + wn * (32 * NJ) + j * 32 + (lane & 31);
                 const float bias = ((se.epi & FITGNN_EPI_BIAS) && col < J) ? se.bias[col] : 0.f;
+                asm volatile("" ::"v"(bias));
 #pragma unroll
                 for (int r = 0; r < 16; ++r) {
                     const long row = row0 + (r & 3) + 8 * (r >> 2);
@@ -212,6 +340,20 @@
             }
         }
     }
+}
+
+template <int WM, int WN, int MI, int NJ, bool AKM, bool BKM, bool EPI>
+__global__ __launch_bounds__(64 * WM * WN) void gemm_f32_kernel(const float *__restrict__ A, long lda, const float *__restrict__ B, long ldb,
+                                                                   long I, int J, long K, float *__restrict__ C, long ldc, int tiles_i,
+                                                                   int tiles_j, int nchunks, long chunk_k, StoreEpi se) {
+    gemm_f32_tile<WM, WN, MI, NJ, AKM, BKM, EPI, false>(A, lda, B, ldb, I, J, K, C, ldc, tiles_i, tiles_j, nchunks, chunk_k, se,
+                                                        RowLists{nullptr, nullptr});
+}
+template <int WM, int WN, int MI, int NJ, bool AKM, bool BKM, bool EPI, int LISTS>
+__global__ __launch_bounds__(64 * WM * WN) void gemm_f32_kernel_rows(const float *__restrict__ A, long lda, const float *__restrict__ B, long ldb,
+                                                                     long I, int J, long K, float *__restrict__ C, long ldc, int tiles_i,
+                                                                     int tiles_j, int nchunks, long chunk_k, StoreEpi se, RowLists rl) {
+    gemm_f32_tile<WM, WN, MI, NJ, AKM, BKM, EPI, true>(A, lda, B, ldb, I, J, K, C, ldc, tiles_i, tiles_j, nchunks, chunk_k, se, rl);
 }
 
 template <bool EPI>
@@ -314,34 +456,49 @@
     return p;
 }
 
-template <int WM, int WN, int MI, int NJ, bool AKM, bool BKM, bool EPI>
+template <int WM, int WN, int MI, int NJ, bool AKM, bool BKM, bool EPI, bool IDX>
 int launch(const Plan &p, const float *a, long lda, const float *b, long ldb, long I, int J, long K, float *c, long ldc, hipStream_t s,
-           const StoreEpi &se) {
+           const StoreEpi &se, const RowLists &rl) {
     using G = Geo<WM, WN, MI, NJ, AKM, BKM>;
     static std::atomic<uint64_t> lds_done{0};
-    if (const int rc = fitgnn_lds_limit_once((const void *)gemm_f32_kernel<WM, WN, MI, NJ, AKM, BKM, EPI>, G::LDS_BYTES, lds_done)) return rc;
+    if constexpr (!IDX) {
+        if (const int rc = fitgnn_lds_limit_once((const void *)gemm_f32_kernel<WM, WN, MI, NJ, AKM, BKM, EPI>, G::LDS_BYTES, lds_done)) return rc;
+    } else {
+        if (const int rc = fitgnn_lds_limit_once((const void *)gemm_f32_kernel_rows<WM, WN, MI, NJ, AKM, BKM, EPI, 1>, G::LDS_BYTES, lds_done)) return rc;
+    }
     unsigned grid;
     if (p.nchunks > 1) grid = (unsigned)(p.tiles_i * p.tiles_j * ((p.nchunks + 7) / 8 * 8));
     else grid = (unsigned)((p.tiles_i + 7) / 8 * 8 * p.tiles_j);
-    hipLaunchKernelGGL((gemm_f32_kernel<WM, WN, MI, NJ, AKM, BKM, EPI>), dim3(grid), dim3(G::THREADS), G::LDS_BYTES, s, a, lda, b, ldb, I, J,
-                       K, c, ldc, p.tiles_i, p.tiles_j, p.nchunks, p.chunk_k, se);
+    if constexpr (!IDX)
+        hipLaunchKernelGGL((gemm_f32_kernel<WM, WN, MI, NJ, AKM, BKM, EPI>), dim3(grid), dim3(G::THREADS), G::LDS_BYTES, s, a, lda, b, ldb, I, J, K, c,
+                           ldc, p.tiles_i, p.tiles_j, p.nchunks, p.chunk_k, se);
+    else
+        hipLaunchKernelGGL((gemm_f32_kernel_rows<WM, WN, MI, NJ, AKM, BKM, EPI, 1>), dim3(grid), dim3(G::THREADS), G::LDS_BYTES, s, a, lda, b, ldb, I,
+                           J, K, c, ldc, p.tiles_i, p.tiles_j, p.nchunks, p.chunk_k, se, rl);
     return (int)hipGetLastError();
+}
+
+template <bool AKM, bool BKM, bool EPI, bool IDX>
+int launch_shape_as(const Plan &p, const float *a, long lda, const float *b, long ldb, long I, int J, long K, float *c, long ldc, hipStream_t s,
+                     const StoreEpi &se, const RowLists &rl) {
+    if constexpr (AKM && BKM) {
+        if (p.shape == S64x512) return launch<1, 4, 2, 4, AKM, BKM, EPI, IDX>(p, a, lda, b, ldb, I, J, K, c, ldc, s, se, rl);
+    }
+    switch (p.shape) {
+        case S256x128: return launch<4, 1, 2, 4, AKM, BKM, EPI, IDX>(p, a, lda, b, ldb, I, J, K, c, ldc, s, se, rl);
+        case S128: return launch<2, 2, 2, 2, AKM, BKM, EPI, IDX>(p, a, lda, b, ldb, I, J, K, c, ldc, s, se, rl);
+        case S64x128: return launch<2, 2, 1, 2, AKM, BKM, EPI, IDX>(p, a, lda, b, ldb, I, J, K, c, ldc, s, se, rl);
+        case S128x64: return launch<4, 1, 1, 2, AKM, BKM, EPI, IDX>(p, a, lda, b, ldb, I, J, K, c, ldc, s, se, rl);
+        case S64x64: return launch<2, 2, 1, 1, AKM, BKM, EPI, IDX>(p, a, lda, b, ldb, I, J, K, c, ldc, s, se, rl);
+        default: return launch<4, 2, 2, 4, AKM, BKM, EPI, IDX>(p, a, lda, b, ldb, I, J, K, c, ldc, s, se, rl);
+    }
 }
 
 template <bool AKM, bool BKM, bool EPI = false>
 int launch_shape(const Plan &p, const float *a, long lda, const float *b, long ldb, long I, int J, long K, float *c, long ldc, hipStream_t s,
-                 const StoreEpi &se = StoreEpi{}) {
-    if constexpr (AKM && BKM) {
-        if (p.shape == S64x512) return launch<1, 4, 2, 4, AKM, BKM, EPI>(p, a, lda, b, ldb, I, J, K, c, ldc, s, se);
-    }
-    switch (p.shape) {
-        case S256x128: return launch<4, 1, 2, 4, AKM, BKM, EPI>(p, a, lda, b, ldb, I, J, K, c, ldc, s, se);
-        case S128: return launch<2, 2, 2, 2, AKM, BKM, EPI>(p, a, lda, b, ldb, I, J, K, c, ldc, s, se);
-        case S64x128: return launch<2, 2, 1, 2, AKM, BKM, EPI>(p, a, lda, b, ldb, I, J, K, c, ldc, s, se);
-        case S128x64: return launch<4, 1, 1, 2, AKM, BKM, EPI>(p, a, lda, b, ldb, I, J, K, c, ldc, s, se);
-        case S64x64: return launch<2, 2, 1, 1, AKM, BKM, EPI>(p, a, lda, b, ldb, I, J, K, c, ldc, s, se);
-        default: return launch<4, 2, 2, 4, AKM, BKM, EPI>(p, a, lda, b, ldb, I, J, K, c, ldc, s, se);
-    }
+                 const StoreEpi &se = StoreEpi{}, const RowLists &rl = RowLists{nullptr, nullptr}) {
+    if (rl.a_rows || rl.b_rows) return launch_shape_as<AKM, BKM, EPI, true>(p, a, lda, b, ldb, I, J, K, c, ldc, s, se, rl);
+    return launch_shape_as<AKM, BKM, EPI, false>(p, a, lda, b, ldb, I, J, K, c, ldc, s, se, rl);
 }
 
 }
@@ -365,8 +522,18 @@
 
 extern "C" int fitgnn_gemm_exact_f32(const float *a, int64_t lda, int32_t a_kmajor, const float *b, int64_t ldb, int32_t b_kmajor,
                                      int64_t I, int32_t J, int64_t K, float *c, int64_t ldc, void *workspace, void *stream) {
+    return fitgnn_gemm_exact_rows_f32(a, lda, a_kmajor, nullptr, b, ldb, b_kmajor, nullptr, I, J, K, c, ldc, workspace, stream);
+}
+
+extern "C" int fitgnn_gemm_exact_rows_f32(const float *a, int64_t lda, int32_t a_kmajor, const int64_t *a_rows, const float *b, int64_t ldb,
+                                          int32_t b_kmajor, const int64_t *b_rows, int64_t I, int32_t J, int64_t K, float *c, int64_t ldc,
+                                          void *workspace, void *stream) {
     if (I <= 0 || J <= 0 || K <= 0 || ldc < J) return FITGNN_E_BADARG;
     if (!a || !b || !c) return FITGNN_E_BADARG;
+    if ((a_rows && a_kmajor) || (b_rows && !b_kmajor)) return FITGNN_E_BADARG;
+    if ((((uintptr_t)a_rows | (uintptr_t)b_rows) % 8) != 0) return FITGNN_E_ALIGN;
+    const RowLists rl{a_rows, b_rows};
+    const StoreEpi none{};
     const int64_t a_inner = a_kmajor ? I : K, b_inner = b_kmajor ? (int64_t)J : K;
     if (a_inner < 4 || b_inner < 4 || (a_inner % 4) != 0 || (b_inner % 4) != 0 || lda < a_inner || ldb < b_inner || (lda % 4) != 0 ||
         (ldb % 4) != 0)
@@ -381,14 +548,15 @@
         pm.tiles_i = (int)(p.main_rows / kShape[p.shape].ti);
         pr.tiles_i = p.rem_tiles_i; pr.nchunks = p.rem_chunks; pr.chunk_k = p.rem_chunk_k;
         const long rem_rows = (long)I - p.main_rows;
-        const float *a_rem = a + p.main_rows * (long)lda;
+        const float *a_rem = a_rows ? a : a + p.main_rows * (long)lda;
+        const RowLists rl_rem{a_rows ? a_rows + p.main_rows : nullptr, b_rows};
         int rc;
         if (b_kmajor) {
-            rc = launch_shape<false, true>(pm, a, (long)lda, b, (long)ldb, p.main_rows, J, (long)K, c, (long)ldc, s);
-            if (!rc) rc = launch_shape<false, true>(pr, a_rem, (long)lda, b, (long)ldb, rem_rows, J, (long)K, (float *)workspace, (long)J, s);
+            rc = launch_shape<false, true>(pm, a, (long)lda, b, (long)ldb, p.main_rows, J, (long)K, c, (long)ldc, s, none, rl);
+            if (!rc) rc = launch_shape<false, true>(pr, a_rem, (long)lda, b, (long)ldb, rem_rows, J, (long)K, (float *)workspace, (long)J, s, none, rl_rem);
         } else {
-            rc = launch_shape<false, false>(pm, a, (long)lda, b, (long)ldb, p.main_rows, J, (long)K, c, (long)ldc, s);
-            if (!rc) rc = launch_shape<false, false>(pr, a_rem, (long)lda, b, (long)ldb, rem_rows, J, (long)K, (float *)workspace, (long)J, s);
+            rc = launch_shape<false, false>(pm, a, (long)lda, b, (long)ldb, p.main_rows, J, (long)K, c, (long)ldc, s, none, rl);
+            if (!rc) rc = launch_shape<false, false>(pr, a_rem, (long)lda, b, (long)ldb, rem_rows, J, (long)K, (float *)workspace, (long)J, s, none, rl_rem);
         }
         if (rc) return rc;
         const long IJ = rem_rows * J;
@@ -403,9 +571,9 @@
         dst = (float *)workspace;
     }
     int rc;
-    if (a_kmajor) rc = launch_shape<true, true>(p, a, (long)lda, b, (long)ldb, (long)I, J, (long)K, dst, ldd, s);
-    else if (b_kmajor) rc = launch_shape<false, true>(p, a, (long)lda, b, (long)ldb, (long)I, J, (long)K, dst, ldd, s);
-    else rc = launch_shape<false, false>(p, a, (long)lda, b, (long)ldb, (long)I, J, (long)K, dst, ldd, s);
+    if (a_kmajor) rc = launch_shape<true, true>(p, a, (long)lda, b, (long)ldb, (long)I, J, (long)K, dst, ldd, s, none, rl);
+    else if (b_kmajor) rc = launch_shape<false, true>(p, a, (long)lda, b, (long)ldb, (long)I, J, (long)K, dst, ldd, s, none, rl);
+    else rc = launch_shape<false, false>(p, a, (long)lda, b, (long)ldb, (long)I, J, (long)K, dst, ldd, s, none, rl);
     if (rc) return rc;
     if (p.nchunks > 1) {
         const long IJ = (long)I * J;
@@ -419,10 +587,17 @@
 extern "C" int fitgnn_gemm_exact_epi_f32(const float *a, int64_t lda, const float *b, int64_t ldb, int64_t I, int32_t J, int64_t K, float *c,
                                          int64_t ldc, const int64_t *rows, const float *bias, uint32_t epilogue, float p_drop, uint64_t seed,
                                          const uint8_t *mask, void *workspace, void *stream) {
+    return fitgnn_gemm_exact_epi_rows_f32(a, lda, nullptr, b, ldb, I, J, K, c, ldc, rows, bias, epilogue, p_drop, seed, mask, workspace, stream);
+}
+
+extern "C" int fitgnn_gemm_exact_epi_rows_f32(const float *a, int64_t lda, const int64_t *a_rows, const float *b, int64_t ldb, int64_t I,
+                                              int32_t J, int64_t K, float *c, int64_t ldc, const int64_t *rows, const float *bias,
+                                              uint32_t epilogue, float p_drop, uint64_t seed, const uint8_t *mask, void *workspace,
+                                              void *stream) {
     if (I <= 0 || J <= 0 || K <= 0 || ldc < J) return FITGNN_E_BADARG;
     if (!a || !b || !c) return FITGNN_E_BADARG;
     if (K < 4 || (K % 4) != 0 || lda < K || ldb < K || (lda % 4) != 0 || (ldb % 4) != 0) return FITGNN_E_BADARG;
-    if ((((uintptr_t)a | (uintptr_t)b) % 16) != 0) return FITGNN_E_ALIGN;
+    if ((((uintptr_t)a | (uintptr_t)b) % 16) != 0 || ((uintptr_t)a_rows % 8) != 0) return FITGNN_E_ALIGN;
     if (epilogue & ~(FITGNN_EPI_BIAS | FITGNN_EPI_ELU | FITGNN_EPI_DROPOUT | FITGNN_EPI_SEED_DEVICE)) return FITGNN_E_BADARG;
     if ((epilogue & (FITGNN_EPI_ELU | FITGNN_EPI_DROPOUT)) && (J % 4) != 0) return FITGNN_E_BADARG;
     if ((epilogue & FITGNN_EPI_BIAS) && !bias) return FITGNN_E_BADARG;
@@ -430,15 +605,18 @@
     const Plan p = make_plan((long)I, J, (long)K, false, false);
     if (p.nchunks > 1) return FITGNN_E_BADARG;
     hipStream_t s = (hipStream_t)stream;
-    StoreEpi se{rows, bias, mask, seed, 0, epilogue, p_drop};
-    if (p.main_rows == 0) return launch_shape<false, false, true>(p, a, (long)lda, b, (long)ldb, (long)I, J, (long)K, c, (long)ldc, s, se);
+    const int vec = (J % 4) == 0 && (ldc % 4) == 0 && ((uintptr_t)c % 16) == 0;
+    StoreEpi se{rows, bias, mask, seed, 0, epilogue, p_drop, vec};
+    const RowLists rl{a_rows, nullptr};
+    if (p.main_rows == 0) return launch_shape<false, false, true>(p, a, (long)lda, b, (long)ldb, (long)I, J, (long)K, c, (long)ldc, s, se, rl);
     if (!workspace || ((uintptr_t)workspace % 16) != 0) return FITGNN_E_BADARG;
     Plan pm = p, pr = p;
     pm.tiles_i = (int)(p.main_rows / kShape[p.shape].ti);
     pr.tiles_i = p.rem_tiles_i; pr.nchunks = p.rem_chunks; pr.chunk_k = p.rem_chunk_k;
     const long rem_rows = (long)I - p.main_rows;
-    int rc = launch_shape<false, false, true>(pm, a, (long)lda, b, (long)ldb, p.main_rows, J, (long)K, c, (long)ldc, s, se);
-    if (!rc) rc = launch_shape<false, false>(pr, a + p.main_rows * (long)lda, (long)lda, b, (long)ldb, rem_rows, J, (long)K, (float *)workspace, (long)J, s);
+    int rc = launch_shape<false, false, true>(pm, a, (long)lda, b, (long)ldb, p.main_rows, J, (long)K, c, (long)ldc, s, se, rl);
+    if (!rc) rc = launch_shape<false, false>(pr, a_rows ? a : a + p.main_rows * (long)lda, (long)lda, b, (long)ldb, rem_rows, J, (long)K,
+                                             (float *)workspace, (long)J, s, StoreEpi{}, RowLists{a_rows ? a_rows + p.main_rows : nullptr, nullptr});
     if (rc) return rc;
     if (rows) se.rows = rows + p.main_rows;
     se.row0 = p.main_rows;
diff --git a/fit-gnn_amd/csrc/spmm.hip b/fit-gnn_amd/csrc/spmm.hip
--- a/fit-gnn_amd/csrc/spmm.hip
+++ b/fit-gnn_amd/csrc/spmm.hip
@@ -340,7 +340,16 @@
 #endif
     SSTAMP(s_begin);
     const fitgnn_block_t blk = blocks[b];
-    if (blk.row_end <= blk.row_begin) return;
+    if (blk.row_end <= blk.row_begin) {
+        if ((BWD || TWO) && col_part && threadIdx.x < 64) {
+            const int c0 = slab * 256 + (int)threadIdx.x * 4;
+            if (c0 + 4 <= H) {
+#pragma unroll
+                for (int i = 0; i < 4; ++i) col_part[(int64_t)b * H + c0 + i] = 0.f;
+            }
+        }
+        return;
+    }
     const int lane = threadIdx.x & 63;
     const int wave = __builtin_amdgcn_readfirstlane(threadIdx.x >> 6);
     const int col0 = slab * 256 + lane * 4;
diff --git a/fit-gnn_amd/fitgnn_amd/_lib.py b/fit-gnn_amd/fitgnn_amd/_lib.py
--- a/fit-gnn_amd/fitgnn_amd/_lib.py
+++ b/fit-gnn_amd/fitgnn_amd/_lib.py
@@ -89,6 +89,9 @@
     "fitgnn_gemm_exact_plan": (ctypes.c_int, [c_i64, c_i32, c_i64, c_i32, c_i32, ptr, ptr, ptr]),
     "fitgnn_gemm_exact_epi_f32": (ctypes.c_int, [ptr, c_i64, ptr, c_i64, c_i64, c_i32, c_i64, ptr, c_i64, ptr, ptr, c_u32, c_f32, c_u64, ptr, ptr,
                                                  ptr]),
+    "fitgnn_gemm_exact_rows_f32": (ctypes.c_int, [ptr, c_i64, c_i32, ptr, ptr, c_i64, c_i32, ptr, c_i64, c_i32, c_i64, ptr, c_i64, ptr, ptr]),
+    "fitgnn_gemm_exact_epi_rows_f32": (ctypes.c_int, [ptr, c_i64, ptr, ptr, c_i64, c_i64, c_i32, c_i64, ptr, c_i64, ptr, ptr, c_u32, c_f32,
+                                                      c_u64, ptr, ptr, ptr]),
     "fitgnn_gemm_nt_presplit_bytes": (c_size, [c_i32, c_i32]),
     "fitgnn_gemm_nt_presplit_f32": (ctypes.c_int, [ptr, c_i64, c_i64, c_i32, c_i32, c_i32, ptr, ptr]),
     "fitgnn_gemm_nt_pre_f32": (ctypes.c_int, [ptr, c_i64, ptr, c_i64, c_i32, c_i32, ptr, c_i64, ptr]),
diff --git a/fit-gnn_amd/fitgnn_amd/ops.py b/fit-gnn_amd/fitgnn_amd/ops.py
--- a/fit-gnn_amd/fitgnn_amd/ops.py
+++ b/fit-gnn_amd/fitgnn_amd/ops.py
@@ -11,12 +11,12 @@
 class OpConfig:
     __slots__ = ("gemm_precision", "atb_kernel", "nt_kernel", "nt_presplit", "fuse_dx_epilogue", "fold_backward",
                  "dedup_gather", "pad_table_min_k", "split_large_blocks", "compact_head_backward", "last_layer_on_loss_rows",
-                 "compact_rows_kernel", "stream_kernel", "two_hop_backward", "narrow_input_first", "fused_pool_head", "fused_gemm_epilogue", "pooled_rows_last_layer", "rows_kernel_min_rows", "appnp_in_lds", "appnp_blocks", "appnp_sliced", "grad_sink", "profile", "profile_gemm",
+                 "compact_rows_kernel", "stream_kernel", "two_hop_backward", "narrow_input_first", "fused_pool_head", "fused_gemm_epilogue", "rows_in_gemm", "pooled_rows_last_layer", "rows_kernel_min_rows", "appnp_in_lds", "appnp_blocks", "appnp_sliced", "grad_sink", "profile", "profile_gemm",
                  "profile_fused", "seed_bank")
 
     def __init__(self, gemm_precision="exact", atb_kernel=True, nt_kernel=True, nt_presplit=True, fuse_dx_epilogue=True,
                  fold_backward=False, dedup_gather=True, pad_table_min_k=0, split_large_blocks=True, compact_head_backward=True,
-                 last_layer_on_loss_rows=True, compact_rows_kernel=True, stream_kernel=False, two_hop_backward=True, narrow_input_first=True, fused_pool_head=True, fused_gemm_epilogue=True, pooled_rows_last_layer=True, rows_kernel_min_rows=32768, appnp_in_lds=True, appnp_blocks=True, appnp_sliced=True, grad_sink=None,
+                 last_layer_on_loss_rows=True, compact_rows_kernel=True, stream_kernel=False, two_hop_backward=True, narrow_input_first=True, fused_pool_head=True, fused_gemm_epilogue=True, rows_in_gemm=True, pooled_rows_last_layer=True, rows_kernel_min_rows=32768, appnp_in_lds=True, appnp_blocks=True, appnp_sliced=True, grad_sink=None,
                  profile=None, profile_gemm=None, profile_fused=None, seed_bank=None):
         if gemm_precision not in ("exact", "high", "highest"):
             raise ValueError(f"gemm_precision {gemm_precision!r}: 'exact', 'high' or 'highest'")
@@ -26,7 +26,7 @@
         self.compact_head_backward, self.last_layer_on_loss_rows = compact_head_backward, last_layer_on_loss_rows
         self.compact_rows_kernel, self.stream_kernel, self.two_hop_backward = compact_rows_kernel, stream_kernel, two_hop_backward
         self.narrow_input_first, self.fused_pool_head, self.grad_sink = narrow_input_first, fused_pool_head, grad_sink
-        self.fused_gemm_epilogue = fused_gemm_epilogue
+        self.fused_gemm_epilogue, self.rows_in_gemm = fused_gemm_epilogue, rows_in_gemm
         self.pooled_rows_last_layer, self.rows_kernel_min_rows = pooled_rows_last_layer, int(rows_kernel_min_rows)
         self.appnp_in_lds, self.appnp_blocks, self.appnp_sliced = appnp_in_lds, appnp_blocks, appnp_sliced
         self.profile, self.profile_gemm, self.profile_fused, self.seed_bank = profile, profile_gemm, profile_fused, seed_bank
@@ -79,19 +79,32 @@
     return cfg.gemm_precision == "exact" and _rows_16b(a) and _rows_16b(b)
 
 
-def gemm_exact(a, b, form, cfg=DEFAULT, out=None):
+def _row_list(rows):
+    return (rows if rows.dtype == torch.int64 else rows.long()).contiguous()
+
+
+def gemm_exact(a, b, form, cfg=DEFAULT, out=None, a_rows=None, b_rows=None):
     L = _lib.lib()
+    if form not in ("nt", "nn", "tn"):
+        raise ValueError(form)
+    akm, bkm = (1 if form == "tn" else 0), (0 if form == "nt" else 1)
+    assert (a_rows is None or not akm) and (b_rows is None or bkm), "a row list names the rows of a k-minor a / a k-major b"
+    if a_rows is not None:
+        a_rows = _row_list(a_rows)
+    if b_rows is not None:
+        b_rows = _row_list(b_rows)
+    _lib.require_cuda(a, b, a_rows, b_rows)
+    a0 = a.shape[0] if a_rows is None else int(a_rows.numel())
+    b0 = b.shape[0] if b_rows is None else int(b_rows.numel())
     if form == "nt":
-        (I, K), J, akm, bkm = a.shape, b.shape[0], 0, 0
+        I, K, J = a0, a.shape[1], b0
         assert b.shape[1] == K
     elif form == "nn":
-        (I, K), J, akm, bkm = a.shape, b.shape[1], 0, 1
-        assert b.shape[0] == K
-    elif form == "tn":
-        (K, I), J, akm, bkm = a.shape, b.shape[1], 1, 1
-        assert b.shape[0] == K
+        I, K, J = a0, a.shape[1], b.shape[1]
+        assert b0 == K
     else:
-        raise ValueError(form)
+        K, I, J = a0, a.shape[1], b.shape[1]
+        assert b0 == K
     if out is None:
         out = torch.empty((I, J), dtype=torch.float32, device=a.device)
     else:
@@ -99,35 +112,39 @@
     wb = int(L.fitgnn_gemm_exact_workspace_bytes(I, J, K, akm, bkm))
     ws = torch.empty(wb // 4, dtype=torch.float32, device=a.device) if wb else None
     ev = _gemm_events(cfg, "gemm_f32_kernel[%s]" % form, 2.0 * I * J * K)
-    rc = L.fitgnn_gemm_exact_f32(_lib.dptr(a), a.stride(0), akm, _lib.dptr(b), b.stride(0), bkm, I, J, K, _lib.dptr(out), out.stride(0),
-                                 _lib.dptr(ws), _lib.stream_ptr(a.device))
+    rc = L.fitgnn_gemm_exact_rows_f32(_lib.dptr(a), a.stride(0), akm, _lib.dptr(a_rows), _lib.dptr(b), b.stride(0), bkm, _lib.dptr(b_rows),
+                                      I, J, K, _lib.dptr(out), out.stride(0), _lib.dptr(ws), _lib.stream_ptr(a.device))
     _gemm_done(cfg, ev)
-    _lib.check(rc, "fitgnn_gemm_exact_f32")
+    _lib.check(rc, "fitgnn_gemm_exact_rows_f32")
     return out
 
 
-def gemm_exact_epi(a, b, rows, bias, epilogue, p=0.0, seed=0, mask=None, cfg=DEFAULT):
+def gemm_exact_epi(a, b, rows, bias, epilogue, p=0.0, seed=0, mask=None, cfg=DEFAULT, a_rows=None):
     L = _lib.lib()
-    (I, K), J = a.shape, b.shape[0]
+    K, J = a.shape[1], b.shape[0]
+    I = a.shape[0] if a_rows is None else int(a_rows.numel())
     assert b.shape[1] == K
     shape, nchunks, main_rows = ctypes.c_int32(), ctypes.c_int32(), ctypes.c_int64()
     _lib.check(L.fitgnn_gemm_exact_plan(I, J, K, 0, 0, ctypes.byref(shape), ctypes.byref(nchunks), ctypes.byref(main_rows)),
                "fitgnn_gemm_exact_plan")
     if nchunks.value > 1:
         return None
-    _lib.require_cuda(a, b, rows, bias, mask)
     seed, epilogue = _seed_arg(seed, epilogue)
+    same = a_rows is rows
     if rows is not None:
-        rows = (rows if rows.dtype == torch.int64 else rows.long()).contiguous()
+        rows = _row_list(rows)
+    if a_rows is not None:
+        a_rows = rows if same else _row_list(a_rows)
+    _lib.require_cuda(a, b, rows, a_rows, bias, mask)
     out = torch.empty((I, J), dtype=torch.float32, device=a.device)
     wb = int(L.fitgnn_gemm_exact_workspace_bytes(I, J, K, 0, 0))
     ws = torch.empty(wb // 4, dtype=torch.float32, device=a.device) if wb else None
     ev = _gemm_events(cfg, "gemm_f32_kernel[nt+epi]", 2.0 * I * J * K)
-    rc = L.fitgnn_gemm_exact_epi_f32(_lib.dptr(a), a.stride(0), _lib.dptr(b), b.stride(0), I, J, K, _lib.dptr(out), out.stride(0),
-                                     _lib.dptr(rows), _lib.dptr(None if bias is None else _f32c(bias)), epilogue, float(p), seed,
-                                     _lib.dptr(mask), _lib.dptr(ws), _lib.stream_ptr(a.device))
+    rc = L.fitgnn_gemm_exact_epi_rows_f32(_lib.dptr(a), a.stride(0), _lib.dptr(a_rows), _lib.dptr(b), b.stride(0), I, J, K, _lib.dptr(out),
+                                          out.stride(0), _lib.dptr(rows), _lib.dptr(None if bias is None else _f32c(bias)), epilogue,
+                                          float(p), seed, _lib.dptr(mask), _lib.dptr(ws), _lib.stream_ptr(a.device))
     _gemm_done(cfg, ev)
-    _lib.check(rc, "fitgnn_gemm_exact_epi_f32")
+    _lib.check(rc, "fitgnn_gemm_exact_epi_rows_f32")
     return out
 
 
@@ -325,7 +342,11 @@
     return mm_at_b(dy_c, out_c, cfg)
 
 
-def mm_at_b(a, b, cfg=DEFAULT, out=None):
+def mm_at_b(a, b, cfg=DEFAULT, out=None, b_rows=None):
+    if b_rows is not None:
+        if _exact(cfg, a, b):
+            return gemm_exact(a, b, "tn", cfg, out=out, b_rows=b_rows)
+        b = b.index_select(0, b_rows)
     R = a.shape[0]
     if out is not None:
         if _exact(cfg, a, b):
@@ -809,7 +830,7 @@
     if side.small_tiles.shape[0]:
         spmm_raw(side.rowptr, side.col, side.val, side.small_tiles, ZT, g.n, window_rows=g.window_rows, out=Y, cfg=quiet, xrow=ix["zrow"])
     n_blocks = int(side.blocks.shape[0])
-    part = torch.zeros((n_blocks + 1, H), dtype=torch.float32, device=dev) if link.want_db else None
+    part = _scratch((n_blocks + 1, H), dev) if link.want_db else None
     _lib.check(L.fitgnn_spmm_two_hop_blocks_f32(_lib.dptr(side.rowptr), _lib.dptr(side.col), _lib.dptr(side.val), _lib.dptr(ZT), ZT.stride(0),
                                                 _lib.dptr(Y), Y.stride(0), g.n, H, _lib.dptr(side.blocks), n_blocks, _lib.dptr(side.long_rows),
                                                 _lib.dptr(ix["zrow"]), _lib.dptr(ix["zcol"]), _lib.dptr(prev), _lib.dptr(Xc), Xc.stride(0), n_sel,
@@ -819,6 +840,8 @@
     if link.want_db:
         if ix["tile_zt"].numel():
             torch.sum(ZT.index_select(0, ix["tile_zt"]), 0, out=part[n_blocks])
+        else:
+            part[n_blocks].zero_()
         db = _fold_partials(part, dev, st)
     if ev is not None:
         ev[1].record()
@@ -860,7 +883,7 @@
     n_tiles = int(tiles.shape[0])
     n_blocks = int(side.blocks.shape[0]) if split else 0
     Y = torch.empty((g.n, H), dtype=torch.float32, device=dev)
-    part = (_scratch((n_tiles, H), dev) if n_blocks == 0 else torch.zeros((n_tiles + n_blocks, H), dtype=torch.float32, device=dev)) if want_db else None
+    part = _scratch((n_tiles + n_blocks, H), dev) if want_db else None
     st = _lib.stream_ptr(dev)
     ev = None
     if cfg.profile is not None:
@@ -1710,6 +1733,15 @@
     return epilogue_fwd_rows_(outc, rows, b, ep.fwd, p=ep.p, seed=ep.seed, mask=ep.mask)
 
 
+def _dense_rows_of(AH, W, b, rows, ep, cfg):
+    if cfg.rows_in_gemm and cfg.fused_gemm_epilogue and _exact(cfg, AH, W) and W.shape[0] % 4 == 0:
+        outc = gemm_exact_epi(AH, W, rows, b, ep.fwd, p=ep.p, seed=ep.seed, mask=ep.mask, cfg=cfg, a_rows=rows)
+        if outc is not None:
+            return outc, AH, True
+    AHc = AH.index_select(0, rows)
+    return _dense_rows(AHc, W, b, rows, ep, cfg), AHc, False
+
+
 def _head_rows_fwd(outc, Wl, bl, rows, n_total, compact_out, g, cfg):
     if _exact(cfg, outc, Wl) and Wl.shape[0] >= 16:
         y = gemm_exact_epi(outc, Wl, None, bl, EPI_BIAS, cfg=cfg) if (cfg.fused_gemm_epilogue and bl is not None) else None
@@ -1763,19 +1795,19 @@
         X = _f32c(X)
         rows = rows if rows.dtype == torch.int64 else rows.long()
         ctx.link_in, ctx.compact_out = link_in, bool(compact_out)
+        ep = _Epilogue(b is not None, p, training, seed, mask)
         if fwd_sub is not None:
             f = fwd_sub.f
             AHc = spmm_raw(f.rowptr, f.col, f.val, f.tiles, X, fwd_sub.m, window_rows=fwd_sub.window_rows, cfg=cfg, profile_kind="rows_fwd")
+            outc, through = _dense_rows(AHc, W, b, rows, ep, cfg), False
         else:
             AH = spmm_graph(g, X, cfg=cfg)
-            AHc = AH.index_select(0, rows)
+            outc, AHc, through = _dense_rows_of(AH, W, b, rows, ep, cfg)
             del AH
-        ep = _Epilogue(b is not None, p, training, seed, mask)
-        outc = _dense_rows(AHc, W, b, rows, ep, cfg)
         y = _head_rows_fwd(outc, Wl, bl, rows, g.n, compact_out, g, cfg)
         keep_x = link_in is not None and cfg.fuse_dx_epilogue and X.shape[1] % 4 == 0
         ctx.save_for_backward(W, Wl, AHc, outc, rows, ep.mask, X if keep_x else None)
-        ctx.g, ctx.ep, ctx.has_bias, ctx.has_bl, ctx.cfg = g, ep, b is not None, bl is not None, cfg
+        ctx.g, ctx.ep, ctx.has_bias, ctx.has_bl, ctx.cfg, ctx.through = g, ep, b is not None, bl is not None, cfg, through
         ctx.ptrs = _addresses(W, b, Wl, bl)
         return y
 
@@ -1787,7 +1819,7 @@
         dZc, db, dWl, dbl = _head_rows_bwd(dy, rows, ctx.compact_out, outc, Wl, ctx.ep, mask, ctx.has_bias, ctx.needs_input_grad[3],
                                            ctx.has_bl and ctx.needs_input_grad[4], cfg, sink, pb=pb if ctx.needs_input_grad[2] else None,
                                            pWl=pWl, pbl=pbl)
-        dW = sink.result(mm_at_b(dZc, AHc, cfg, out=sink.slice(pW))) if ctx.needs_input_grad[1] else None
+        dW = sink.result(mm_at_b(dZc, AHc, cfg, out=sink.slice(pW), b_rows=rows if ctx.through else None)) if ctx.needs_input_grad[1] else None
         dX = _rows_adjoint(ctx.g, dZc, W, rows, ctx.link_in, Xprev, cfg, zero_tail=True, two_hop=True) if ctx.needs_input_grad[0] else None
         return dX, dW, (db if ctx.has_bias else None), dWl, dbl, None, None, None, None, None, None, None, None, None, None
 
@@ -1798,9 +1830,8 @@
     def forward(ctx, X, W, b, g, p, training, seed, mask, rows, cfg, link_in=None):
         X = _f32c(X)
         rows = rows if rows.dtype == torch.int64 else rows.long()
-        AHc = spmm_graph(g, X, cfg=cfg).index_select(0, rows)
         ep = _Epilogue(b is not None, p, training, seed, mask)
-        outc = _dense_rows(AHc, W, b, rows, ep, cfg)
+        outc, AHc, ctx.through = _dense_rows_of(spmm_graph(g, X, cfg=cfg), W, b, rows, ep, cfg)
         keep_x = link_in is not None and cfg.fuse_dx_epilogue and X.shape[1] % 4 == 0
         ctx.save_for_backward(W, AHc, outc, rows, ep.mask, X if keep_x else None)
         ctx.g, ctx.ep, ctx.has_bias, ctx.cfg, ctx.link_in = g, ep, b is not None, cfg, link_in
@@ -1814,7 +1845,7 @@
         sink, (pW, pb) = _GradSink(cfg.grad_sink), ctx.ptrs
         sb = sink.slice(pb) if (ctx.has_bias and ctx.needs_input_grad[2]) else None
         dZc, db = epilogue_bwd_rows_raw(dOutc, outc, rows, ep.bwd, p=ep.p, seed=ep.seed, mask=mask, want_db=ctx.has_bias, db_out=sb)
-        dW = sink.result(mm_at_b(dZc, AHc, cfg, out=sink.slice(pW))) if ctx.needs_input_grad[1] else None
+        dW = sink.result(mm_at_b(dZc, AHc, cfg, out=sink.slice(pW), b_rows=rows if ctx.through else None)) if ctx.needs_input_grad[1] else None
         dX = _rows_adjoint(ctx.g, dZc, W, rows, ctx.link_in, Xprev, cfg, zero_tail=False) if ctx.needs_input_grad[0] else None
         return dX, dW, (sink.result(db) if ctx.has_bias else None), None, None, None, None, None, None, None, None
 
diff --git a/include/fitgnn_hip.h b/include/fitgnn_hip.h
--- a/include/fitgnn_hip.h
+++ b/include/fitgnn_hip.h
@@ -150,6 +150,12 @@
 int fitgnn_gemm_exact_epi_f32(const float *a, int64_t lda, const float *b, int64_t ldb, int64_t I, int32_t J, int64_t K, float *c,
                               int64_t ldc, const int64_t *rows, const float *bias, uint32_t epilogue, float p_drop, uint64_t seed,
                               const uint8_t *mask, void *workspace, void *stream);
+int fitgnn_gemm_exact_rows_f32(const float *a, int64_t lda, int32_t a_kmajor, const int64_t *a_rows, const float *b, int64_t ldb,
+                               int32_t b_kmajor, const int64_t *b_rows, int64_t I, int32_t J, int64_t K, float *c, int64_t ldc,
+                               void *workspace, void *stream);
+int fitgnn_gemm_exact_epi_rows_f32(const float *a, int64_t lda, const int64_t *a_rows, const float *b, int64_t ldb, int64_t I, int32_t J,
+                                   int64_t K, float *c, int64_t ldc, const int64_t *rows, const float *bias, uint32_t epilogue,
+                                   float p_drop, uint64_t seed, const uint8_t *mask, void *workspace, void *stream);
 
 size_t fitgnn_gemm_nt_presplit_bytes(int32_t N, int32_t K);
 int fitgnn_gemm_nt_presplit_f32(const float *b, int64_t stride_n, int64_t stride_k, int32_t N, int32_t K, int32_t K_valid,
```

Measured after the change: 3.669 billion (median of 6 runs). 1.01x the previous value.
